# mfouda/epsilon

Hardware: AMD Instinct MI355X
Metric: ADMM iters/sec, dense Lasso 1e4x5e4 (higher is better)
Workload: dtype f32

## Files before the change

### epsilon_amd/csrc/admm.cc

```cpp
#include "admm.h"

#include <algorithm>
#include <chrono>
#include <cmath>
#include <cstdio>
#include <cstdlib>
#include <map>

#include "comm.h"
#include "fused_route.h"
#include "options.h"

namespace eps {

double Now() {
  using clock = std::chrono::steady_clock;
  return std::chrono::duration<double>(clock::now().time_since_epoch()).count();
}

namespace {

std::set<std::string> InferShardedArgs(const BlockMatrix& H) {
  std::set<std::string> out;
  const ShardSpec& sh = ShardSpec::Get();
// ... 44 lines not shown
}

}

Solver::Solver(pb::Problem problem, std::shared_ptr<DataMap> data, pb::SolverParams params)
    : problem_(std::move(problem)), data_(std::move(data)), params_(params) {}
Solver::~Solver() {}

FusedRoute* Solver::batch_route() const { return initialized_ && !finished_ && iter_ == 0 ? route_.get() : nullptr; }
void Solver::BatchLaunchCheck(int iter) {
  iter_ = iter;
  if (route_->HasCheck()) route_->LaunchNorms();
}
bool Solver::BatchFinishCheck() {
  if (route_->HasCheck()) FinishRouteCheck();
  else ComputeResiduals();
  finished_ = status_.state == pb::SolverStatus::OPTIMAL;
  return finished_;
}
void Solver::BatchFinishMaxIterations(int iter) {
  iter_ = iter;
  ComputeResiduals();
  status_.state = pb::SolverStatus::MAX_ITERATIONS_REACHED;
  finished_ = true;
}
void Solver::BatchAddLoopTime(double seconds) {
  loop_seconds_ += seconds;
  status_.init_time = init_seconds_;
  status_.total_time = init_seconds_ + loop_seconds_;
}

void Solver::LogStatus() {
  if (!params_.verbose || !log_) return;
  char buf[256];
  std::snprintf(buf, sizeof(buf), "iter=%d residuals primal=%.2e [%.2e] dual=%.2e [%.2e]",
                status_.num_iterations, status_.r_norm, status_.epsilon_primal, status_.s_norm,
                status_.epsilon_dual);
  log_(buf);
}

void Solver::FinishResiduals(double r, double s, double eps_pri, double eps_dual) {
  status_.r_norm = r;
  status_.s_norm = s;
  status_.epsilon_primal = eps_pri;
  status_.epsilon_dual = eps_dual;
  if (r <= eps_pri && s <= eps_dual && !params_.ignore_stopping_criteria)
    status_.state = pb::SolverStatus::OPTIMAL;
  else
    status_.state = pb::SolverStatus::RUNNING;
  status_.num_iterations = iter_;
}

int Solver::Run(int max_sweeps) {
  EPS_CHECK_MSG(initialized_, "Solver::Run before Init");
  SetCurrentDType(data_->dtype());
  const double t0 = Now();
  int done = 0;
  const int epoch = params_.epoch_iterations > 0 ? params_.epoch_iterations : 1;
  const int log_every = params_.log_iterations > 0 ? params_.log_iterations : 1;
  auto batch_size = [&](int it, int done_so_far) {
    if (it >= params_.max_iterations || (max_sweeps >= 0 && done_so_far >= max_sweeps)) return 0;
    int batch = 1;
    while ((it + batch - 1) % epoch != 0 && !(params_.verbose && (it + batch - 1) % log_every == 0))
      ++batch;
    if (batch > params_.max_iterations - it) batch = params_.max_iterations - it;
    if (max_sweeps >= 0 && batch > max_sweeps - done_so_far) batch = max_sweeps - done_so_far;
    return batch;
  };
  int speculated = 0;
  auto far_from_optimal = [&] {
    if (status_.epsilon_primal <= 0 || status_.epsilon_dual <= 0) return true;
    return status_.r_norm > 4 * status_.epsilon_primal || status_.s_norm > 4 * status_.epsilon_dual;
  };
  while (!finished_ && iter_ < params_.max_iterations && (max_sweeps < 0 || done < max_sweeps)) {
    int batch = speculated;
    if (batch == 0) {
      batch = batch_size(iter_, done);
      SweepBatch(batch);
    }
    speculated = 0;
    done += batch;
    iter_ += batch - 1;
    if (iter_ % epoch == 0) {
      const int next = (PipelinedChecks() && (params_.ignore_stopping_criteria || far_from_optimal()))
                           ? batch_size(iter_ + 1, done)
                           : 0;
      if (next > 0) {
        BeginResiduals();
        SaveSnapshot();
        SweepBatch(next);
        speculated = next;
        EndResiduals();
        if (status_.state == pb::SolverStatus::OPTIMAL) {
          RestoreSnapshot();
          finished_ = true;
          break;
        }
      } else {
        ComputeResiduals();
        if (status_.state == pb::SolverStatus::OPTIMAL) {
          finished_ = true;
          break;
        }
      }
    }
    if (iter_ % log_every == 0) LogStatus();
    ++iter_;
  }
  if (!finished_ && iter_ == params_.max_iterations) {
    ComputeResiduals();
    status_.state = pb::SolverStatus::MAX_ITERATIONS_REACHED;
    finished_ = true;
  }
  Runtime::Get().Sync();
  if (Runtime::Get().peer()) Runtime::Get().peer()->CheckError();
  loop_seconds_ += Now() - t0;
  if (finished_) LogStatus();
  status_.init_time = init_seconds_;
  status_.total_time = init_seconds_ + loop_seconds_;
  return done;
}

void Solver::Solve() {
  const double t0 = Now();
  Init();
  Runtime::Get().Sync();
  init_seconds_ = Now() - t0;
  Run(-1);
}


class ProxADMMSolver final : public Solver {
 public:
  using Solver::Solver;
  ~ProxADMMSolver() override { ResetGraph(); }

  void Init() override {
    SetCurrentDType(data_->dtype());
    const double t0 = Now();
    if (op_cache_.size() > 64) op_cache_.Clear();
    OpCacheScope cache_scope(InitCache());
    static const bool trace = opt::IsSet(opt::kInitTrace);
    auto mark = [&](const char* what) {
      if (!trace) return;
      const double th = Now();
      Runtime::Get().Sync();
      std::fprintf(stderr, "[init] %-16s host %.2f ms  drained %.2f ms\n", what, 1e3 * (th - t0),
                   1e3 * (Now() - t0));
    };
    InitConstraints();
    mark("constraints");
    InitProxOperators();
    mark("prox operators");
    if (!params_.warm_start || !vars_initialized_) {
      InitVariables();
      vars_initialized_ = true;
    }
    iter_ = 0;
    finished_ = false;
    status_ = pb::SolverStatus();
    initialized_ = true;
    ResetGraph();
    route_.reset();
    route_ = RecogniseMultiBlockRoute({static_cast<int>(problem_.constraint.size()), A_, b_, prox_, data_.get(),
                                       shared_cache_, u_, x_, y_, y_prev_});
    mark("fused state");
    if (params_.verbose && log_) {
      char buf[128];
      std::snprintf(buf, sizeof(buf), "constraints, m = %lld, variables, n = %lld",
                    static_cast<long long>(m_), static_cast<long long>(n_));
      log_(buf);
    }
    Runtime::Get().Sync();
    init_seconds_ = Now() - t0;
  }

  BlockVector GetSolution() override {
    BlockVector r;
    for (int i = 0; i < N_; ++i) r += x_[i];
    return r;
  }

 protected:
  void InitConstraints() {
    A_ = BlockMatrix();
    b_ = BlockVector();
    for (size_t i = 0; i < problem_.constraint.size(); ++i) {
      const pb::Expression& constr = problem_.constraint[i];
      EPS_CHECK_MSG(constr.expression_type == pb::Expression::INDICATOR, "constraint is not an indicator");
      EPS_CHECK_MSG(constr.cone_type == 1, "constraint cone is not ZERO");
      EPS_CHECK(constr.arg.size() == 1);
      affine::BuildAffineOperator(constr.arg[0], data_.get(), affine::constraint_key(i), &A_, &b_);
    }
    AT_ = A_.Transpose();
    GlobalDims(A_, &m_, &n_);
  }

  void InitProxOperators() {
    EPS_CHECK_MSG(problem_.objective.expression_type == pb::Expression::ADD, "objective is not ADD");
    N_ = static_cast<int>(problem_.objective.arg.size());
    EPS_CHECK_MSG(params_.rho == 1, "rho != 1 is not supported (reference prox_admm.cc:50)");
    const double sqrt_rho = std::sqrt(params_.rho);
    prox_.clear();
    AiT_.clear();
    arg_shards_.clear();
    term_per_rank_.clear();
    std::set<std::string> constr_vars = A_.col_keys();
    for (int i = 0; i < N_; ++i) {
      const pb::Expression& f_expr = problem_.objective.arg[i];
      EPS_CHECK_MSG(f_expr.expression_type == pb::Expression::PROX_FUNCTION,
                    "objective term " << i << " is not a PROX_FUNCTION");
      AffineOperator H;
      for (size_t k = 0; k < f_expr.arg.size(); ++k)
        affine::BuildAffineOperator(f_expr.arg[k], data_.get(), affine::arg_key(k), &H.A, &H.b);
      AffineOperator A;
      std::map<std::string, const pb::Expression*> vars;
      GetVariables(f_expr, &vars);
      for (const auto& var : vars) {
        if (constr_vars.find(var.first) == constr_vars.end()) continue;
        for (const auto& it : A_.col(var.first)) A.A(it.first, var.first) = sqrt_rho * it.second;
      }
      prox_.emplace_back(CreateProxOperator(f_expr.prox_function.prox_function_type,
                                            f_expr.prox_function.epigraph));
      arg_shards_.push_back(InferShardedArgs(H.A));
      {
        const ShardSpec& sh = ShardSpec::Get();
        bool own = sh.active() && sh.consensus_terms() && !vars.empty();
        for (const auto& var : vars) own = own && sh.IsSharded(var.first);
        term_per_rank_.push_back(own);
      }
      {
        LocalShardScope scope(arg_shards_.back());
        prox_.back()->Init(ProxOperatorArg(f_expr.prox_function, data_.get(), H, A));
      }
      AiT_.push_back(A.A.Transpose());
    }
  }

  void InitVariables() {
    x_.assign(N_, BlockVector());
    y_.assign(N_, BlockVector());
    u_ = BlockVector();
    for (size_t i = 0; i < problem_.constraint.size(); ++i) {
      u_.Set(affine::constraint_key(i),
             DVec::Zeros(GetDimension(problem_.constraint[i].arg[0]), data_->dtype()));
    }
  }

  void ResetGraph() {
    if (graph_exec_) (void)hipGraphExecDestroy(graph_exec_);
    if (graph_) (void)hipGraphDestroy(graph_);
    graph_exec_ = nullptr;
    graph_ = nullptr;
    graph_len_ = 0;
  }

  void SweepBatch(int count) override {
    static const int mode = opt::Int(opt::kGraph, -1);
    Runtime& rt = Runtime::Get();
    const bool want = route_ && route_->Capturable() && (mode == 1 || (mode != 0 && route_->CaptureByDefault()));
    if (!want || count < 2 || rt.profiling()) {
      for (int i = 0; i < count; ++i) Sweep();
      return;
    }
    if (graph_exec_ == nullptr || graph_len_ != count) {
      ResetGraph();
      hipStream_t s = rt.stream();
      EPS_HIP(hipStreamBeginCapture(s, hipStreamCaptureModeThreadLocal));
      rt.set_capturing(true);
      try {
        for (int i = 0; i < count; ++i) route_->Sweep();
      } catch (...) {
        rt.set_capturing(false);
        hipGraph_t dead = nullptr;
        (void)hipStreamEndCapture(s, &dead);
        if (dead) (void)hipGraphDestroy(dead);
        throw;
      }
      rt.set_capturing(false);
      EPS_HIP(hipStreamEndCapture(s, &graph_));
      EPS_HIP(hipGraphInstantiate(&graph_exec_, graph_, nullptr, nullptr, 0));
      graph_len_ = count;
    }
    EPS_HIP(hipGraphLaunch(graph_exec_, rt.stream()));
  }

  void Sweep() override {
    if (route_) {
      route_->Sweep();
      return;
    }
    y_prev_ = y_;
    u_ -= b_;
    for (int i = 0; i < N_; ++i) u_ -= y_[i];
    for (int i = 0; i < N_; ++i) {
      u_ += y_[i];
      {
        LocalShardScope scope(arg_shards_[i]);
        x_[i] = prox_[i]->Apply(u_);
      }
      y_[i] = A_ * x_[i];
      u_ -= y_[i];
    }
  }

  bool PipelinedChecks() const override { return route_ && route_->PipelineChecks(); }
  void BeginResiduals() override {
    Runtime& rt = Runtime::Get();
    rt.ResetSlots();
    route_->LaunchNorms();
    rt.FetchSlotsAsync();
  }
  void EndResiduals() override {
    Runtime::Get().WaitSlots();
    FinishRouteCheck();
  }
  void FinishRouteCheck() override {
    const FusedRoute::Check c = route_->FinishCheck();
// ... 227 lines not shown
```

### epsilon_amd/csrc/capi.cc

```cpp
#include "../../include/epsilon_hip.h"

#include <algorithm>
#include <cmath>
#include <cstdio>
#include <cstdlib>
#include <cstring>
#include <map>
#include <memory>
#include <set>
#include <string>
#include <vector>

#include "admm.h"
#include "block.h"
#include "comm.h"
#include "kernels.h"
#include "linear_map.h"
#include "options.h"
#include "wire.h"

using namespace eps;

struct eps_result {
  std::string status;
// ... 1162 lines not shown
            PutValues(r.get(), "trace\t" + std::to_string(s) + "\t" + f.first, {FillValue(f.second)});
          PutValues(r.get(), "pivot\t" + std::to_string(s) + "\t" + trace[s].pivot, {static_cast<double>(s)});
        }
        for (size_t i = 0; i < chol.order().size(); ++i)
          PutValues(r.get(), "order\t" + std::to_string(i) + "\t" + chol.order()[i], {static_cast<double>(i)});
        if (args.mode == BlockSolveArgs::FACTOR) {
          PutBlocks(r.get(), "L", chol.L());
          PutBlocks(r.get(), "D_inv", chol.D_inv());
        }
        PutValues(r.get(), "condition_estimate", {chol.condition_estimate()});
        PutValues(r.get(), "refine_steps", {static_cast<double>(chol.refine_steps())});
        if (nrhs > 0) {
          PutVector(r.get(), "x", chol.Solve(b));
          PutVector(r.get(), "x_again", chol.Solve(b));
        }
        break;
      }
    }
    *out = r.release();
  });
}

int eps_test_dense_op(const eps_dense_op* g, double* out, double* out2) {
  return Guard([&] {
    const DenseOpArgs args = CheckDenseOpArgs(g, out, out2);
    const DType dt = ConfiguredDType();
    constexpr int64_t G = EPS_DENSE_OP_GUARD;
    const int64_t n = g->rows;
    DVec a_all, x_all, y_all, add_all, a, x, y, add, work;
    if (args.use_a) a = PlaceOperand(g->a, g->a_len, g->a_off, 0, dt, &a_all);
    if (args.use_x) x = PlaceOperand(g->x, g->x_len, g->x_off, 0, dt, &x_all);
    if (args.use_add) add = PlaceOperand(g->add, g->add_len, g->add_off, 0, dt, &add_all);
    if (args.reduction) {
      if (args.use_y) y = PlaceOperand(g->y, g->y_len, g->y_off, 0, dt, &y_all);
      Runtime& rt = Runtime::Get();
      rt.ResetSlots();
      const int slot = rt.NewSlot();
      EPS_HIP(hipMemcpyAsync(rt.SlotPtr(slot), &g->preset, sizeof(double), hipMemcpyHostToDevice, rt.stream()));
      rt.Sync();
      const bool acc = g->accumulate != 0;
      if (args.op == DenseOpArgs::SUMSQ) k::SumSq(x, rt.SlotPtr(slot), acc);
      else if (args.op == DenseOpArgs::SUMSQ_DIFF) k::SumSqDiff(x, y, rt.SlotPtr(slot), acc);
      else k::Dot(x, y, rt.SlotPtr(slot), acc);
      EPS_HIP(hipGetLastError());
      rt.FetchSlots();
      out[0] = rt.SlotValue(slot);
      rt.ResetSlots();
      return;
    }
    static_assert(EPS_DENSE_OP_GUARD % 4 == 0, "the guard keeps offset 0 aligned");
    auto place_y = [&] { y = PlaceOperand(g->y, g->y_len, g->y_off, G, dt, &y_all); };
    auto fetch_y = [&](double* dst) { y_all.Slice(g->y_off, g->y_len + 2 * G).ToHost(dst); };
    place_y();
    const bool symv = args.op == DenseOpArgs::SYMV || args.op == DenseOpArgs::SYMV_PACKED;
    if (symv && g->use_work) work = DVec::Empty(k::SymvWorkspace(n), dt);
    const DVec* wp = (symv && g->use_work) ? &work : nullptr;
    switch (args.op) {
      case DenseOpArgs::GEMV_N:
      case DenseOpArgs::GEMV_T:
        k::Gemv(args.op == DenseOpArgs::GEMV_T, n, g->cols, g->alpha, a, g->lda, x, g->beta, y);
        break;
      case DenseOpArgs::SYMV:
        k::Symv(n, g->alpha, a, g->lda, x, g->beta, y, wp);
        break;
      case DenseOpArgs::SYMV_PACKED: {
        const DVec P = k::SymvPack(n, a, g->lda);
        k::SymvPacked(n, g->alpha, P, x, g->beta, y, wp);
        EPS_HIP(hipGetLastError());
        fetch_y(out);
        place_y();
        k::Symv(n, g->alpha, a, g->lda, x, g->beta, y, wp);
        EPS_HIP(hipGetLastError());
        fetch_y(out2);
        return;
      }
      case DenseOpArgs::REDUCE_PARTIALS:
        k::ReducePartials(n, g->nparts, a, g->alpha, g->beta, y, args.use_add ? &add : nullptr);
        break;
      case DenseOpArgs::AXPBY:
        k::Axpby(y, g->alpha, g->alias_xy ? y : x, g->beta);
        break;
      case DenseOpArgs::DIAG_MUL:
        k::DiagMul(y, g->alpha, a, x, g->beta);
        break;
      default:
        EPS_FATAL("eps_test_dense_op: unreachable");
    }
    EPS_HIP(hipGetLastError());
    fetch_y(out);
  });
}

int eps_test_gemm_op(const eps_gemm_op* g, double* out, char* route, size_t route_cap) {
  return Guard([&] {
    const GemmOpArgs args = CheckGemmOpArgs(g, out, route, route_cap);
    route[0] = '\0';
    const DType dt = ConfiguredDType();
    constexpr int64_t G = EPS_DENSE_OP_GUARD;
    const int64_t M = g->M, N = g->N, K = g->K;
    DVec a_all, b_all, c_all, d_all, a, b, c, d;
    if (args.use_a) a = PlaceOperand(g->a, g->a_len, g->a_off, G, dt, &a_all);
    if (args.use_b) b = PlaceOperand(g->b, g->b_len, g->b_off, G, dt, &b_all);
    if (args.use_c) c = PlaceOperand(g->c, g->c_len, g->c_off, G, dt, &c_all);
    if (args.use_d) d = PlaceOperand(g->d, g->d_len, 0, G, dt, &d_all);
    k::GemmClearRoute();
    switch (args.op) {
      case GemmOpArgs::GEMM:
        k::Gemm(g->trans_a != 0, g->trans_b != 0, M, N, K, g->alpha, a, g->lda, b, g->ldb, g->beta, c, g->ldc,
                g->lower_only != 0);
        break;
      case GemmOpArgs::GEMM_BATCHED:
        k::GemmBatched(g->trans_a != 0, g->trans_b != 0, M, N, K, g->alpha, a, g->lda, g->sA, b, g->ldb, g->sB,
                       g->beta, c, g->ldc, g->sC, g->batch, g->lower_only != 0, g->outer, g->sA2, g->sB2);
        break;
      case GemmOpArgs::MAT_COPY:
        k::MatCopy(g->trans_a != 0, M, N, g->alpha, a, g->lda, c);
        break;
      case GemmOpArgs::ADD_DIAG:
        k::AddDiag(c, M, g->ldc, g->alpha, args.use_d ? &d : nullptr);
        break;
      case GemmOpArgs::SYMMETRIZE:
        k::SymmetrizeFromLower(c, M, g->ldc);
        break;
      case GemmOpArgs::COL_ABS_SUMS: {
        std::vector<double> h(static_cast<size_t>(N + 2 * G), EPS_DENSE_OP_SENTINEL);
        c_all = DVec::FromHost(h.data(), N + 2 * G, F64);
        k::ColAbsSums(a, M, N, g->lda, c_all.as<double>() + G);
        EPS_HIP(hipGetLastError());
        c_all.ToHost(out);
        return;
      }
      case GemmOpArgs::KRON:
        k::KronDense(c, a, M, N, b, K, g->batch);
        break;
    }
    EPS_HIP(hipGetLastError());
    std::snprintf(route, route_cap, "%s", k::GemmLastRoute());
    c_all.Slice(g->c_off, g->c_len + 2 * G).ToHost(out);
  });
}

int eps_test_factor_op(const eps_factor_op* g, double* out, double* out2) {
  return Guard([&] {
    const FactorOpArgs args = CheckFactorOpArgs(g, out);
    const DType dt = ConfiguredDType();
    constexpr int64_t G = EPS_DENSE_OP_GUARD;
    const int64_t n = g->n;
    DVec w_all;
    DVec W = PlaceOperand(g->a, g->a_len, g->a_off, G, dt, &w_all);
    struct Restore { ~Restore() { k::SetPotrfForm(-1); } } restore;
    k::SetPotrfForm(g->form);
    if (args.op == FactorOpArgs::SPD_INVERSE) {
      DVec X;
      k::SpdInverseInPlace(W, n, out2 != nullptr ? &X : nullptr);
      EPS_HIP(hipGetLastError());
      w_all.Slice(g->a_off, n * n + 2 * G).ToHost(out);
      if (out2 != nullptr && n > 0) X.Slice(0, n * n).ToHost(out2);
      return;
    }
    const int64_t len = n * g->out_cols;
    std::vector<double> h(static_cast<size_t>(g->a_off + 2 * G + len), EPS_DENSE_OP_SENTINEL);
    DVec o_all = DVec::FromHost(h.data(), static_cast<int64_t>(h.size()), dt);
    k::SpdInverseColumns(W, n, g->lo, g->cnt, o_all.Slice(g->a_off + G, len));
    EPS_HIP(hipGetLastError());
    o_all.Slice(g->a_off, len + 2 * G).ToHost(out);
    if (out2 != nullptr && n > 0) W.ToHost(out2);
  });
}

int eps_bench_spd_inverse_columns(int64_t n, int64_t cnt, int iters, double* ms_avg) {
  return Guard([&] {
    const DType dt = ConfiguredDType();
    DVec G = Synthetic(n * n, dt, 1.0);
    DVec W0 = DVec::Zeros(n * n, dt);
    k::Gemm(false, true, n, n, n, 1.0 / n, G, n, G, n, 0.0, W0, n, false);
    k::AddDiag(W0, n, n, 1.0, nullptr);
    DVec W = DVec::Empty(n * n, dt);
    DVec Out = DVec::Empty(n * cnt, dt);
    Runtime& rt = Runtime::Get();
    double total = 0;
    for (int i = 0; i < iters + 1; ++i) {
      k::Copy(W, W0);
      rt.Sync();
      hipEvent_t a, b;
      EPS_HIP(hipEventCreate(&a));
      EPS_HIP(hipEventCreate(&b));
      EPS_HIP(hipEventRecord(a, rt.stream()));
      k::SpdInverseColumns(W, n, 0, cnt, Out);
      EPS_HIP(hipEventRecord(b, rt.stream()));
      EPS_HIP(hipEventSynchronize(b));
      float e = 0;
      EPS_HIP(hipEventElapsedTime(&e, a, b));
      (void)hipEventDestroy(a);
      (void)hipEventDestroy(b);
      if (i > 0) total += e;
    }
    *ms_avg = total / iters;
  });
}

int eps_bench_prox(int kind, int64_t n, int iters, double* ms_avg) {
  return Guard([&] {
    EPS_CHECK(n > 0 && iters > 0 && ms_avg != nullptr);
    const DType dt = ConfiguredDType();
    DVec v = Synthetic(n, dt, 4.0);
    DVec x = DVec::Empty(n, dt);
    k::ScaledZoneArgs a;
    a.lam = 0.7;
    DVec lamv;
    if (kind == 1) {
      lamv = Synthetic(n, dt, 1.0);
      k::Axpby(lamv, 0.0, lamv, 1.0);
      k::Fill(lamv, 0.7);
      a.lam_vec = &lamv;
    }
    *ms_avg = TimeLaunches(iters, [&] {
      if (kind == 2) k::MaxZero(x, v);
      else k::ScaledZone(x, v, a);
    });
  });
}

int eps_bench_svd(int64_t m, int64_t n, int rank, int max_sweeps, double perturb, double* ms_cold,
                  int* sweeps_cold, double* ms_warm, int* sweeps_warm, double* defects) {
  return Guard([&] {
    EPS_CHECK(m > 0 && n > 0 && ms_cold != nullptr);
    const DType dt = ConfiguredDType();
    Runtime& rt = Runtime::Get();
    uint64_t st = 0x9E3779B97F4A7C15ull;
    auto uni = [&] {
      st ^= st << 13;
      st ^= st >> 7;
      st ^= st << 17;
      return static_cast<double>(st >> 11) * (1.0 / 9007199254740992.0);
    };
    auto gauss = [&] { return (uni() + uni() + uni() + uni() - 2.0) * 1.7320508075688772; };
    std::vector<double> h(static_cast<size_t>(m) * std::max<int64_t>(rank, 1));
    for (auto& v : h) v = gauss();
    DVec A = DVec::FromHost(h.data(), m * std::max<int64_t>(rank, 1), dt);
    h.resize(static_cast<size_t>(n) * std::max<int64_t>(rank, 1));
    for (auto& v : h) v = gauss();
    DVec B = DVec::FromHost(h.data(), n * std::max<int64_t>(rank, 1), dt);
    DVec Y = DVec::Empty(m * n, dt);
    {
      std::vector<float> sp(static_cast<size_t>(m) * n);
      for (auto& v : sp) v = uni() < 0.1 ? static_cast<float>(10.0 * gauss()) : 0.0f;
      std::vector<double> col(m);
      std::vector<double> all(sp.begin(), sp.end());
      sp.clear();
      sp.shrink_to_fit();
      Y = DVec::FromHost(all.data(), m * n, dt);
    }
    if (rank > 0) k::Gemm(false, true, m, n, rank, 1.0, A, m, B, n, 1.0, Y, m);
    auto timed = [&](const DVec& W, const DVec& V, bool warm, double* ms, int* sweeps) {
      rt.Sync();
      hipEvent_t a, b;
      EPS_HIP(hipEventCreate(&a));
      EPS_HIP(hipEventCreate(&b));
      EPS_HIP(hipEventRecord(a, rt.stream()));
      const int sw = k::JacobiSvd(W, m, n, V, max_sweeps, warm, false);
      EPS_HIP(hipEventRecord(b, rt.stream()));
      EPS_HIP(hipEventSynchronize(b));
      float e = 0;
      EPS_HIP(hipEventElapsedTime(&e, a, b));
      (void)hipEventDestroy(a);
      (void)hipEventDestroy(b);
      *ms = e;
      if (sweeps) *sweeps = sw;
    };
    auto measure = [&](const DVec& Y0, const DVec& W, const DVec& V, double* out) {
      DVec T = DVec::Empty(n * n, dt);
      k::Gemm(true, false, n, n, n, 1.0, V, n, V, n, 0.0, T, n);
      k::AddDiag(T, n, n, -1.0, nullptr);
      rt.ResetSlots();
      const int s0 = rt.NewSlot(), s1 = rt.NewSlot(), s2 = rt.NewSlot(), s3 = rt.NewSlot(), s4 = rt.NewSlot();
      k::SumSq(T, rt.SlotPtr(s0), false);
      DVec R = Y0.Clone();
      k::Gemm(false, true, m, n, n, 1.0, W, m, V, n, -1.0, R, m);
      k::SumSq(R, rt.SlotPtr(s1), false);
      k::SumSq(Y0, rt.SlotPtr(s2), false);
      k::Gemm(true, false, n, n, m, 1.0, W, m, W, m, 0.0, T, n);
      k::SumSq(T, rt.SlotPtr(s3), false);
      DVec sig = DVec::Empty(n, dt);
      k::ColNorms(W, m, n, sig, false);
      DVec sq = DVec::Empty(n, dt);
      k::DiagMul(sq, 1.0, sig, sig, 0.0);
      k::SumSq(sq, rt.SlotPtr(s4), false);
      rt.FetchSlots();
      out[0] = std::sqrt(rt.SlotValue(s0) / static_cast<double>(n));
      out[1] = std::sqrt(rt.SlotValue(s1) / rt.SlotValue(s2));
      const double all = rt.SlotValue(s3), diag = rt.SlotValue(s4);
      out[2] = std::sqrt(std::max(0.0, all - diag) / diag);
    };
    DVec W = Y.Clone();
    DVec V = DVec::Empty(n * n, dt);
    timed(W, V, false, ms_cold, sweeps_cold);
    if (defects) measure(Y, W, V, defects);
    if (ms_warm != nullptr && perturb >= 0) {
      DVec Y2 = Y.Clone();
      DVec N = Synthetic(m * n, dt, 1.0);
      k::Axpby(Y2, perturb, N, 1.0);
      DVec W2 = DVec::Empty(m * n, dt);
      k::Gemm(false, false, m, n, n, 1.0, Y2, m, V, n, 0.0, W2, m);
      timed(W2, V, true, ms_warm, sweeps_warm);
      if (defects) measure(Y2, W2, V, defects + 3);
    }
  });
// ... 60 lines not shown
```

### epsilon_amd/csrc/fused_route.cc

```cpp
#include "fused_route.h"

#include <algorithm>
#include <cmath>
#include <cstring>
#include <map>

#include "admm.h"
#include "comm.h"
#include "kernels.h"
#include "options.h"

namespace eps {
namespace {


k::ZoneParams ZoneOf(const ScaledZoneDesc& z, double a1) {
  k::ZoneParams s;
  s.alpha_vec = z.alpha_vec;
  s.beta_vec = z.beta_vec;
  s.Bs = z.Bs;
  s.Cs = z.Cs;
  s.a1 = a1;
  s.lam = z.lam;
  s.alpha = z.alpha;
// ... 33 lines not shown
    if (shared != nullptr) {
      key = HashCombine(HashCombine(reinterpret_cast<uintptr_t>(D->data().data()), 0x9ac4ed), m);
      if (auto hit = shared->Find(key)) {
        packed = hit->data();
        return;
      }
    }
    packed = k::SymvPack(m, D->data(), m);
    if (key) shared->Put(key, std::make_shared<DenseMatrixImpl>(packed, packed.n, 1, false, 1.0, key));
  }
  InverseApply Column(int64_t c) const {
    InverseApply a = *this;
    a.p = p.Slice(c * m, m);
    a.w = w.Slice(c * m, m);
    if (work.n > 0) a.work = work.Slice(c * k::SymvWorkspace(m), k::SymvWorkspace(m));
    return a;
  }
  void Apply() const {
    if (packed.n > 0) k::SymvPacked(m, D->scale(), packed, p, 0.0, w, &work);
    else if (work.n > 0) k::Symv(m, D->scale(), D->data(), m, p, 0.0, w, &work);
    else D->Apply(1.0, p, 0.0, w);
  }
};

struct StateSlice {
  BlockVector* home;
  std::string key;
  DVec v;
  bool take = true;
};
void AdoptState(const std::vector<StateSlice>& table, const std::vector<BlockVector*>& homes) {
  for (const StateSlice& s : table) {
    if (!s.take || !s.home->has_key(s.key)) continue;
    EPS_CHECK((*s.home)(s.key).n == s.v.n);
    k::Copy(s.v, (*s.home)(s.key));
  }
  for (BlockVector* h : homes) *h = BlockVector();
  for (const StateSlice& s : table) s.home->Set(s.key, s.v);
}
std::vector<BlockVector*> Homes(const MultiBlockParts& a) {
  std::vector<BlockVector*> h = {&a.u};
  for (auto* c : {&a.x, &a.y, &a.y_prev})
    for (BlockVector& v : *c) h.push_back(&v);
  return h;
}

int BatchWideMin();

enum ZeroTallMode { kZeroTallOff, kZeroTallOn, kZeroTallAuto };
enum MatrixRoute { kMatrixOff, kMatrixPass, kMatrixWide, kMatrixAuto };

constexpr int64_t kResidentLimitBytes = int64_t(224) << 20;

k::FusedResidency ResidentShare(int64_t m, int64_t n, DType dt, int64_t touched, bool auto_on,
                                k::LassoFusedArgs* pass = nullptr) {
  int64_t budget = opt::FusedResident();
  if (budget < 0) budget = auto_on ? std::max<int64_t>(0, kResidentLimitBytes - touched * (dt == F32 ? 4 : 8)) : 0;
  const k::FusedResidency res = k::LassoFusedResidency(m, n, dt, budget);
  if (pass != nullptr) {
    pass->qfull = res.qfull;
    pass->jcut = res.jcut;
  }
  return res;
}

constexpr int64_t kMatrixFusedMinRows = 256;

constexpr int64_t kZeroFusedMinRows = 256;

constexpr int64_t kZeroTallMinCols = 256;
constexpr int64_t kZeroTallAutoMinCols = 256;
constexpr int64_t kZeroTallSmoothAutoMinCols = 512;

uint64_t Bits(double v) {
  uint64_t b;
  std::memcpy(&b, &v, 8);
  return b;
}

bool RhsAligned(const std::vector<const k::LassoInstance*>& members) {
  bool aligned = true;
  for (const k::LassoInstance* s : members)
    if (s->rhs.n > 0) aligned = aligned && reinterpret_cast<uintptr_t>(s->rhs.data()) % 16 == 0;
  return aligned;
}

struct WideSweep {
  static constexpr int PW = k::kLassoWidePanel;
  int64_t m = 0, n = 0, lda = 0, ldv = 0, panel_len = 0;
  DVec A;
  bool whiten = false;
  const DenseMatrixImpl* D = nullptr;
  DVec V, T, apart;
  int64_t akc = 0, afull = 0, arem = 0, aparts = 0;

  void Init(int64_t m_, int64_t n_, const DVec& A_, int64_t lda_, bool whiten_, const DenseMatrixImpl* D_) {
    m = m_;
    n = n_;
    A = A_;
    lda = lda_;
    whiten = whiten_;
    D = D_;
    ldv = (n + 63) / 64 * 64;
    panel_len = static_cast<int64_t>(PW) * m;
    V = DVec::Zeros(static_cast<int64_t>(PW) * ldv, F32);
    T = DVec::Empty(static_cast<int64_t>(k::LassoWideSlabs(m, n)) * panel_len, F32);
    akc = std::max<int64_t>(32, ((m + 63) / 64 + 31) / 32 * 32);
    afull = m / akc;
    arem = m - afull * akc;
    aparts = afull + (arem > 0 ? 1 : 0);
    apart = whiten ? DVec() : DVec::Empty(aparts * panel_len, F32);
  }

  void ApplyInverse(const DVec& Pp, const DVec& Wp) const {
    const int64_t sA = D->trans() ? akc : akc * D->rows();
    k::GemmBatched(D->trans(), false, m, PW, akc, D->scale(), D->data(), D->rows(), sA, Pp, m, akc, 0.0, apart, m,
                   panel_len, afull);
    if (arem > 0) {
      const int64_t oA = afull * sA, oB = afull * akc;
      k::GemmBatched(D->trans(), false, m, PW, arem, D->scale(), D->data().Slice(oA, D->data().n - oA), D->rows(),
                     0, Pp.Slice(oB, Pp.n - oB), m, 0, 0.0, apart.Slice(afull * panel_len, panel_len), m, 0, 1);
    }
    k::ReducePartials(panel_len, static_cast<int>(aparts), apart, 1.0, 0.0, Wp);
  }

  void Run(const DVec& table, int first, int nk, uint64_t live, const DVec& Wp, const DVec& Pp,
           const double* group_lam = nullptr) const {
    k::LassoWideBack(m, n, lda, A, table, first, nk, live, Wp, m, V, ldv, group_lam);
    k::LassoWideForward(m, n, lda, A, nk, V, ldv, T, m);
    k::LassoWideReduce(m, n, table, first, nk, live, T, m);
    if (!whiten) ApplyInverse(Pp, Wp);
  }
};

struct BatchRoute : FusedRoute {
  DType dt = F32;
  int64_t m = 0, n = 0;
  int grid = 0;
  DVec w, p, tpart;
  InverseApply inv;
  bool whiten = false;
  k::LassoFusedArgs pass;
  k::FusedResidency res;

  virtual bool BatchKey(const pb::SolverParams& params, bool tall_groups, std::vector<uint64_t>* key) const = 0;
  virtual const k::ZeroRowsArgs* Rows() const { return nullptr; }
  virtual const k::ZeroTallSamplesArgs* Samples() const { return nullptr; }
  virtual k::FusedResidency Residency(int64_t count) const { return res; }

  std::vector<uint64_t> KeyHead(const DenseMatrixImpl& L, const DenseMatrixImpl& D,
                                const pb::SolverParams& params) const {
    return {static_cast<uint64_t>(pass.chain), reinterpret_cast<uintptr_t>(L.data().data()),
            static_cast<uint64_t>(L.rows()), static_cast<uint64_t>(m), static_cast<uint64_t>(n),
            static_cast<uint64_t>(dt), Bits(L.scale()), reinterpret_cast<uintptr_t>(D.data().data()),
            Bits(D.scale()), reinterpret_cast<uintptr_t>(inv.packed.data()), inv.work.n > 0 ? 1u : 0u,
            static_cast<uint64_t>(params.max_iterations), static_cast<uint64_t>(params.epoch_iterations)};
  }

  template <class Applies>
  void BatchSweep(const DVec& table, const DVec& row_table, const DVec& sample_table, int count,
                  const double* group_lam, const k::FusedResidency& share, bool rhs_aligned, const DVec& work,
                  Applies own_applies) const {
    const int64_t pm = pass.m, pn = pass.n;
    auto passes = [&](int chain) {
      const int width = k::LassoBatchWidth(pm, pn, dt, chain);
      for (int first = 0; first < count; first += width)
        k::LassoBatchPass(pm, pn, pass.lda, pass.A, table, first, std::min(width, count - first), group_lam, share,
                          chain);
    };
    passes(pass.chain);
    if (Samples() != nullptr) {
      k::ZeroTallSamplesBatch(pn, dt, sample_table, count);
      passes(5);
    }
    if (Rows() != nullptr) k::ZeroFusedRowsBatch(pm, grid, Rows()->smooth, dt, row_table, count, Rows()->tall);
    else k::ReducePartialsBatch(pm, grid, table, count, dt, rhs_aligned);
    if (whiten) return;
    if (inv.packed.n > 0) k::SymvPackedBatch(pm, inv.D->scale(), inv.packed, table, count, work);
    else own_applies();
  }
};

struct LassoRoute final : BatchRoute {
  LeastSquaresDesc ls;
  ScaledZoneDesc sz;
  double a1 = 0;
  int64_t slab = 0;
  bool sharded = false;
  bool use_peer = false;
  bool peer_slab = false;
  bool replicated_apply = false;
  DVec wpad, wslice;
  DVec state_all, snapshot;
  DVec norm_work;
  int norm_slot = 0;
  double wscale = 1;
  DVec X, Ahat, rhat;
  int64_t cols = 1;
  bool group = false;
  int64_t group_rows = 0;
  bool wide = false;
  bool rhs_aligned = true;
  std::vector<k::LassoInstance> members;
  DVec table;
  WideSweep ws;

  k::FusedResidency Residency(int64_t count, k::LassoFusedArgs* into) const {
    if (sharded || use_peer || wide || ShardSpec::Get().active()) return k::FusedResidency();
    return ResidentShare(m, n, dt, count * (static_cast<int64_t>(grid) * m + 6 * n + 2 * m) + (whiten ? 0 : m * m),
                         count == 1 && cols == 1, into);
  }
  k::FusedResidency Residency(int64_t count) const override { return Residency(count, nullptr); }

  bool Enable(const MultiBlockParts& a) {
    if (opt::Is0(opt::kFused) || a.prox.size() != 2 || a.num_constraints != 1 || !a.b.data().empty()) return false;
    const ShardSpec& sh = ShardSpec::Get();
    if (sh.active() && sh.consensus_terms()) return false;
    if (!a.prox[0]->DescribeLeastSquares(&ls)) return false;
    cols = ls.cols;
    const int matrix_mode = cols > 1 ? opt::Word(opt::kFusedMatrix) : kMatrixAuto;
    if (cols > 1 && (matrix_mode == kMatrixOff || sh.active())) return false;
    if (!a.prox[1]->DescribeScaledZone(&sz)) {
      GroupNorm2Desc gn;
      if (cols == 1 || !a.prox[1]->DescribeGroupNorm2(&gn) || gn.cols != cols) return false;
      group = true;
      group_rows = gn.rows;
      sz = ScaledZoneDesc();
      sz.var_key = gn.var_key;
      sz.constraint_key = gn.constraint_key;
      sz.Bs = gn.Bs;
      sz.Cs = gn.Cs;
      sz.lam = gn.lam;
    }
    dt = a.data->dtype();
    if ((sz.alpha_vec.n > 0 && sz.alpha_vec.dt != dt) || (sz.beta_vec.n > 0 && sz.beta_vec.dt != dt)) return false;
    const std::string ck = affine::constraint_key(0);
    if (ls.constraint_key != ck || sz.constraint_key != ck || a.A.data().size() != 2) return false;
    const DenseMatrixImpl& L = *ls.L_arg_var;
    if (L.trans()) return false;
    m = L.rows();
    n = L.cols();
    const int64_t nx = n * cols;
    double a0 = 0;
    if (!ConsensusTie(a.A, ck, ls.var_key, sz.var_key, nx, &a0, &a1) || a0 != 1.0) return false;
    if (!k::LassoFusedSupported(m, n, L.data(), L.rows())) return false;
    if (ls.rhs_arg.n != 0 && ls.rhs_arg.n != m * cols) return false;
    if (cols > 1 && !ChooseMatrixRoute(matrix_mode)) return false;
    const int64_t npad = (nx + 63) / 64 * 64;
    state_all = DVec::Zeros(6 * npad, dt);
    snapshot = DVec::Empty(6 * npad, dt);
    norm_work = DVec::Zeros(64 * 5 + 1, F64);
    a.y_prev.resize(2);
    std::vector<StateSlice> views = {{&a.x[0], ls.var_key}, {&a.x[1], sz.var_key}, {&a.y[0], ck},
                                     {&a.y[1], ck},         {&a.u, ck},            {&a.y_prev[1], ck}};
    views[5].take = false;
    for (size_t q = 0; q < views.size(); ++q) views[q].v = state_all.Slice(static_cast<int64_t>(q) * npad, nx);
    k::ConsensusState& s = pass.inst.state;
    s.copy = views[0].v, s.var = views[1].v, s.y_zero = views[2].v, s.y_term = views[3].v, s.u = views[4].v;
    s.y_term_prev = views[5].v;
    grid = k::LassoFusedGrid(m, n, dt);
    const int64_t wlen = wide ? (cols + WideSweep::PW - 1) / WideSweep::PW * WideSweep::PW * m : cols * m;
    p = DVec::Zeros(wlen, dt);
    if (!wide) tpart = DVec::Empty(static_cast<int64_t>(grid) * m * cols, dt);
    if (cols > 1) {
      w = DVec::Zeros(wlen, dt);
    } else {
      Comm* comm = Runtime::Get().comm();
      PeerExchange* px = Runtime::Get().peer();
      sharded = sh.active() && sh.IsSharded(ls.var_key);
      use_peer = sharded && px != nullptr && m * (dt == F64 ? 2 : 1) <= px->slot() && ls.Dinv_arg != nullptr &&
                 !ls.Dinv_arg->trans() && ls.Dinv_arg->rows() == m;
      const int G = use_peer ? px->view().G : (comm ? comm->size() : 1);
      slab = ((m + G - 1) / G + 3) / 4 * 4;
      wpad = DVec::Zeros(slab * G, dt);
      wslice = DVec::Zeros(slab, dt);
      w = wpad.Slice(0, m);
      const char* e = opt::Raw(opt::kShardedApply);
      replicated_apply = e && e[0] == 'r';
      const bool want_slab = e ? !replicated_apply : G >= 3;
      peer_slab = use_peer && want_slab && k::PeerSlabApplySupported(px->view(), m, slab, ls.Dinv_arg->data(), m);
    }
    if (!use_peer && !sh.active() && EnableWhiten()) {
    } else if (wide) {
    } else {
      inv.Init(ls.Dinv_arg, m, p, w, a.shared_cache, cols);
    }
    if (wide) ws.Init(m, n, whiten ? Ahat : L.data(), whiten ? m : L.rows(), whiten, ls.Dinv_arg.get());
    BuildPass();
    AdoptState(views, Homes(a));
    ForwardFromState();
    return true;
  }

  bool ChooseMatrixRoute(int mode) {
    const DenseMatrixImpl& L = *ls.L_arg_var;
    const DenseMatrixImpl& D = *ls.Dinv_arg;
    if (m < kMatrixFusedMinRows || L.dtype() != dt || D.dtype() != dt) return false;
    if (group && group_rows != n) return false;
    if (sz.alpha_vec.n > 0 && sz.alpha_vec.n != n * cols) return false;
    if (sz.beta_vec.n > 0 && sz.beta_vec.n != n * cols) return false;
    if (D.rows() != m || D.cols() != m) return false;
    const int width = k::LassoBatchWidth(m, n, dt);
    const bool pass_ok = width > 0 && (!group || cols <= width);
    const bool wide_ok = dt == F32 && k::LassoWideSupported(m, n, L.data(), L.rows()) &&
                         (!group || cols <= WideSweep::PW);
    if (mode == kMatrixPass) wide = false;
    else if (mode == kMatrixWide) wide = true;
    else wide = wide_ok && (cols >= BatchWideMin() || !pass_ok);
    return wide ? wide_ok : pass_ok;
  }

  bool EnableWhiten() {
    const DenseMatrixImpl& L = *ls.L_arg_var;
    const DenseMatrixImpl& D = *ls.Dinv_arg;
    OpCache* cache = CurrentOpCache();
    if (!FusedWhitenEnabled() || cache == nullptr || dt != F32 || L.dtype() != F32 || m < kWhitenMinRows)
      return false;
    if (n < 2 * m) return false;
    if (D.id() == 0 || D.trans() || D.rows() != m || D.cols() != m || L.rows() != m) return false;
    const auto cached = cache->Find(D.id());
    const auto Xm = cache->Find(FactorInverseKey(D.id()));
    if (!cached || !Xm || cached->data().data() != D.data().data() || Xm->rows() != m || Xm->cols() != m)
      return false;
    const uint64_t key = HashCombine(HashCombine(HashCombine(HashCombine(Xm->id(), 0x3a7),
                                                             reinterpret_cast<uintptr_t>(L.data().data())),
                                                 L.id()),
                                     static_cast<uint64_t>(n));
    DVec Ah;
    if (auto hit = cache->Find(key)) {
      Ah = hit->data();
    } else {
      Ah = DVec::Empty(m * n, F32);
      if (!k::GemmSplitF16KRange(4, m, n, m, 1.0, Xm->data(), m, L.data(), m, Ah, m))
        k::Gemm(false, false, m, n, m, 1.0, Xm->data(), m, L.data(), m, 0.0, Ah, m);
      cache->Put(key, std::make_shared<DenseMatrixImpl>(Ah, m, n, false, 1.0, key));
    }
    if (!k::LassoFusedSupported(m, n, Ah, m)) return false;
    if (ls.rhs_arg.n != 0 && cols > 1) {
      rhat = DVec::Empty(m * cols, F32);
      k::Gemm(false, false, m, cols, m, 1.0, Xm->data(), m, ls.rhs_arg, m, 0.0, rhat, m);
    } else if (ls.rhs_arg.n != 0) {
      rhat = DVec::Empty(m, F32);
      k::Gemv(false, m, m, 1.0, Xm->data(), m, ls.rhs_arg, 0.0, rhat);
    }
    X = Xm->data();
    Ahat = Ah;
    wscale = D.scale();
    whiten = true;
    return true;
  }

  void ForwardFromState() {
    const DenseMatrixImpl& L = *ls.L_arg_var;
    const k::ConsensusState& s = pass.inst.state;
    DVec v0 = s.u.Clone();
    k::Axpby(v0, -1.0, s.y_zero, 1.0);
    k::Axpby(v0, -1.0, s.y_term, 1.0);
    k::Axpby(v0, 1.0, s.y_zero, 1.0);
    if (cols == 1 && !whiten) {
      L.Apply(-1.0, v0, 0.0, p);
      ForwardTail(false);
      return;
    }
    const int64_t mk = m * cols;
    DVec pp = whiten && cols > 1 ? DVec::Empty(mk, v0.dt) : p.Slice(0, mk);
    for (int64_t c = 0; c < cols; ++c) L.Apply(-1.0, v0.Slice(c * n, n), 0.0, pp.Slice(c * m, m));
    if (ls.rhs_arg.n != 0) k::Axpby(pp, 1.0, ls.rhs_arg, 1.0);
    for (int64_t c = 0; whiten && c < cols; ++c)
      k::Gemv(false, m, m, 1.0, X, m, pp.Slice(c * m, m), 0.0, w.Slice(c * m, m));
    if (!whiten) ApplyInverseFixed();
  }

  void ForwardTail(bool reduced) {
    const DenseMatrixImpl& L = *ls.L_arg_var;
    if (whiten) {
      k::ReducePartials(m, grid, tpart, -L.scale(), 0.0, w, rhat.n != 0 ? &rhat : nullptr);
      return;
    }
    bool rhs_added = false;
    if (reduced) {
      const bool have_rhs = ls.rhs_arg.n != 0;
      const bool fold = have_rhs && (!sharded || Runtime::Get().comm()->rank() == 0);
      k::ReducePartials(m, grid, tpart, -L.scale(), 0.0, p, fold ? &ls.rhs_arg : nullptr);
      rhs_added = have_rhs;
    }
    if (sharded) Runtime::Get().comm()->AllReduceSum(p);
    if (ls.rhs_arg.n != 0 && !rhs_added) k::Axpby(p, 1.0, ls.rhs_arg, 1.0);
    const DenseMatrixImpl& D = *ls.Dinv_arg;
    Comm* comm = Runtime::Get().comm();
    if (sharded && comm->size() > 1 && !D.trans() && D.rows() == m && !replicated_apply) {
      const int64_t per = slab;
      const int64_t lo = std::min<int64_t>(m, comm->rank() * per);
      const int64_t cnt = std::min<int64_t>(m, lo + per) - lo;
      DVec mine = wslice;
      if (cnt < per) k::Fill(mine, 0.0);
      if (cnt > 0) {
        DVec rows = D.data().Slice(lo * m, cnt * m);
        k::Gemv(true, m, cnt, D.scale(), rows, m, p, 0.0, mine.Slice(0, cnt));
      }
      comm->AllGather(mine.data(), wpad.data(), static_cast<size_t>(per), wpad.dt);
    } else {
      ApplyInverseFixed();
    }
  }

  void ForwardTailPeer() {
    const DenseMatrixImpl& L = *ls.L_arg_var;
    const DenseMatrixImpl& D = *ls.Dinv_arg;
    const PeerView& pv = Runtime::Get().peer()->view();
    k::PeerReduceExchange(pv, m, grid, tpart, -L.scale(), ls.rhs_arg.n != 0 ? &ls.rhs_arg : nullptr, p);
    if (peer_slab) {
      const int64_t lo = std::min<int64_t>(m, static_cast<int64_t>(pv.rank) * slab);
      k::PeerSlabApplyExchange(pv, m, slab, lo, D.data(), m, D.scale(), p, wpad);
    } else {
      ApplyInverseFixed();
    }
  }

  void ApplyInverseFixed() {
    if (wide) {
      for (int64_t q = 0; q * ws.panel_len < w.n; ++q)
        ws.ApplyInverse(p.Slice(q * ws.panel_len, ws.panel_len), w.Slice(q * ws.panel_len, ws.panel_len));
    } else if (cols == 1) {
      inv.Apply();
    } else if (inv.packed.n > 0) {
      k::SymvPackedBatch(m, inv.D->scale(), inv.packed, table, static_cast<int>(cols), inv.work);
    } else {
      for (int64_t c = 0; c < cols; ++c) inv.Column(c).Apply();
    }
  }

  void BuildPass() {
    const DenseMatrixImpl& L = *ls.L_arg_var;
    pass.m = m;
    pass.n = n;
    pass.lda = whiten ? m : L.rows();
    pass.A = whiten ? Ahat : L.data();
    res = Residency(cols, &pass);
    k::LassoInstance& s = pass.inst;
    s.w = w;
    s.tpart = tpart;
    s.p = whiten ? w : p;
    s.rhs = whiten ? rhat : ls.rhs_arg;
    s.kappa = -L.scale() * (whiten ? wscale : 1.0);
    s.pkappa = -L.scale();
    s.zone = ZoneOf(sz, a1);
    if (cols == 1) return;
    members.assign(static_cast<size_t>(cols), s);
    for (int64_t c = 0; c < cols; ++c) {
      k::LassoInstance& mb = members[static_cast<size_t>(c)];
      auto col = [&](const DVec& v, int64_t len) { return v.n > 0 ? v.Slice(c * len, len) : v; };
      mb.w = col(s.w, m);
      mb.p = col(s.p, m);
      mb.rhs = col(s.rhs, m);
      if (!wide) mb.tpart = col(s.tpart, static_cast<int64_t>(grid) * m);
      else mb.tpart = mb.w;
      k::ConsensusState& ms = mb.state;
      for (DVec* v : {&ms.u, &ms.var, &ms.copy, &ms.y_term, &ms.y_zero, &ms.y_term_prev, &mb.zone.alpha_vec,
                      &mb.zone.beta_vec})
        *v = col(*v, n);
    }
    std::vector<const k::LassoInstance*> v;
    for (const auto& mb : members) v.push_back(&mb);
    rhs_aligned = RhsAligned(v);
    k::LassoBatchUpload(v, dt, &table);
  }

  void MatrixSweep() {
    const int K = static_cast<int>(cols);
    const double* group_lam = group ? &sz.lam : nullptr;
    if (wide) {
      constexpr int PW = WideSweep::PW;
      for (int first = 0; first < K; first += PW) {
        const int nk = std::min(PW, K - first);
        const uint64_t live = nk == 64 ? ~uint64_t(0) : (uint64_t(1) << nk) - 1;
        const int64_t off = static_cast<int64_t>(first) * m;
        ws.Run(table, first, nk, live, w.Slice(off, ws.panel_len), whiten ? DVec() : p.Slice(off, ws.panel_len),
               group_lam);
      }
      return;
    }
    BatchSweep(table, DVec(), DVec(), K, group_lam, res, rhs_aligned, inv.work, [&] {
      for (int64_t c = 0; c < cols; ++c) inv.Column(c).Apply();
    });
  }

  void Sweep() override {
    if (cols > 1) {
      MatrixSweep();
    } else if (use_peer) {
      pass.epoch = Runtime::Get().peer()->view().epoch;
      k::LassoFusedPass(pass);
      ForwardTailPeer();
    } else {
      k::LassoFusedPass(pass);
      ForwardTail(true);
    }
  }

  bool HasCheck() const override { return true; }
  bool PipelineChecks() const override {
    static const bool off = opt::Is0(opt::kPipelineChecks);
    return !off;
  }
  void LaunchNorms() override {
    Runtime& rt = Runtime::Get();
    norm_slot = rt.NewSlot();
// ... 598 lines not shown
```

### epsilon_amd/csrc/fused_route.h

```cpp
#pragma once

#include <memory>
#include <vector>

#include "block.h"
#include "prox.h"

namespace eps {

class FusedRoute {
 public:
  virtual ~FusedRoute() {}
  virtual void Sweep() = 0;

  virtual bool HasCheck() const { return false; }
  virtual bool PipelineChecks() const { return false; }
  virtual void LaunchNorms() {}
  struct Check {
    double r = 0, s = 0;
    double max_norm = 0;
    double atu = 0;
  };
  virtual Check FinishCheck() { return Check(); }
  virtual void SaveSnapshot() {}
  virtual void RestoreSnapshot() {}

  virtual bool Capturable() const { return false; }
  virtual bool CaptureByDefault() const { return false; }
};

struct MultiBlockParts {
  int num_constraints;
  const BlockMatrix& A;
  const BlockVector& b;
  const std::vector<std::unique_ptr<ProxOperator>>& prox;
  DataMap* data;
  OpCache* shared_cache;
  BlockVector& u;
  std::vector<BlockVector>&x, &y, &y_prev;
};
struct TwoBlockParts {
  int num_constraints;
  const AffineOperator& constr_H;
  const std::vector<std::unique_ptr<ProxOperator>>& prox;
  DataMap* data;
  BlockVector &x, &z, &u, &z_prev;
};

std::unique_ptr<FusedRoute> RecogniseMultiBlockRoute(const MultiBlockParts& parts);
std::unique_ptr<FusedRoute> RecogniseTwoBlockRoute(const TwoBlockParts& parts);

}
```

### epsilon_amd/csrc/kernels.h

```cpp
#pragma once

#include "device.h"

namespace eps {
struct PeerView;
namespace k {

void Fill(const DVec& y, double v);
void Copy(const DVec& dst, const DVec& src);
void FillHash(const DVec& y, uint64_t seed);
void Axpby(const DVec& y, double a, const DVec& x, double b);
void DiagMul(const DVec& y, double a, const DVec& d, const DVec& x, double b);
void ConvertFromF64(const DVec& dst, const double* src_dev);
void ConvertToF64(double* dst_dev, const DVec& src);
void ConvertFromF32(const DVec& dst, const float* src_dev);

void SumSq(const DVec& x, double* slot, bool accumulate);
void SumSqDiff(const DVec& x, const DVec& y, double* slot, bool accumulate);
void Dot(const DVec& x, const DVec& y, double* slot, bool accumulate);

void Gemv(bool trans, int64_t rows, int64_t cols, double alpha, const DVec& A, int64_t lda,
          const DVec& x, double beta, const DVec& y);

void Symv(int64_t n, double alpha, const DVec& S, int64_t lds, const DVec& x, double beta,
// ... 17 lines not shown
  double Bs = 0, Cs = 0, a1 = 0, lam = 0, alpha = 1, beta = 1, M = 0;
};
struct LassoInstance {
  DVec w;
  DVec tpart;
  ConsensusState state;
  ZoneParams zone;
  DVec p, rhs;
  double kappa = 0;
  double pkappa = 0;
  DVec zg, zrhs;
  DVec zd, zfarg;
  double ke = 0, dinv = 0;
};
struct LassoFusedArgs {
  int64_t m = 0, n = 0, lda = 0;
  DVec A;
  LassoInstance inst;
  unsigned* epoch = nullptr;
  int chain = 0;
  double a0 = 1;
  DVec e1;
  int qfull = 0;
  int64_t jcut = 0;
};

enum SmoothFn { SMOOTH_EXP, SMOOTH_LOGISTIC, SMOOTH_NEG_ENTR, SMOOTH_INV_POS, SMOOTH_NEG_LOG };

struct ZeroRowsArgs {
  int64_t m = 0;
  int nparts = 0;
  DVec w, tpart, r, rhs, g;
  ConsensusState state;
  ZoneParams zone;
  double e = 0, pkappa = 0;
  bool smooth = false;
  SmoothFn fn = SMOOTH_LOGISTIC;
  DVec hs, hys, hv;
  bool tall = false;
};
struct ZeroTallSamplesArgs {
  int64_t m = 0;
  DVec d, farg;
  DVec rhs, g;
  ConsensusState state;
  ZoneParams zone;
  DVec hs, hys, hv;
  double kappa = 0, ke = 0, dinv = 0;
  SmoothFn fn = SMOOTH_LOGISTIC;
};
void ZeroTallSamples(const ZeroTallSamplesArgs& args);
void ZeroTallSamplesHead(const ZeroTallSamplesArgs& args);
void ZeroFusedRows(const ZeroRowsArgs& args);
void ZeroSmoothHead(const ZeroRowsArgs& args);
void ZeroRowsBatchUpload(const std::vector<const ZeroRowsArgs*>& members, DVec* table);
void ZeroFusedRowsBatch(int64_t m, int nparts, bool smooth, DType dt, const DVec& table, int count,
                        bool tall = false);
void ZeroTallSamplesBatchUpload(const std::vector<const ZeroTallSamplesArgs*>& members, DVec* table);
void ZeroTallSamplesBatch(int64_t m, DType dt, const DVec& table, int count);
bool LassoFusedSupported(int64_t m, int64_t n, const DVec& A, int64_t lda);
int LassoFusedGrid(int64_t m, int64_t n, DType dt = F32);
int LassoFusedBlock(int64_t m, int64_t n, DType dt);
struct FusedResidency {
  int qfull = 0;
  int64_t jcut = 0;
  int64_t bytes = 0;
};
FusedResidency LassoFusedResidency(int64_t m, int64_t n, DType dt, int64_t budget);
FusedResidency LastFusedResidency();
void NoteFusedResidency(int qfull, int64_t jcut);
void LassoFusedPass(const LassoFusedArgs& args);
void LassoFusedNorms(const DVec& u, const DVec& y0, const DVec& y1, const DVec& y1prev, double* out6,
                     const DVec& work, const unsigned* peer_err = nullptr);

template <class T> struct LassoBatchInst {
  const T* w;
  T* tpart;
  T* u; T* x0; T* x1; T* y0; T* y1; T* y1prev;
  const T* alpha_v;
  const T* beta_v;
  T* p;
  const T* rhs;
  T kappa, Bs, Cs, a1, lam, alpha, beta, M;
  T pkappa;
  T* e0;
  const T* zg;
  const T* zrhs;
  T* zd;
  const T* zfarg;
  T ke, dinv;
};
int LassoBatchWidth(int64_t m, int64_t n, DType dt, int chain = 0);
void LassoBatchUpload(const std::vector<const LassoInstance*>& members, DType dt, DVec* table);
void LassoBatchPass(int64_t m, int64_t n, int64_t lda, const DVec& A, const DVec& table, int first,
                    int count, const double* group_lam = nullptr, const FusedResidency& res = FusedResidency(),
                    int chain = 0);
void ReducePartialsBatch(int64_t m, int nparts, const DVec& table, int count, DType dt,
                         bool rhs_aligned);
void SymvPackedBatch(int64_t m, double alpha, const DVec& P, const DVec& table, int count,
                     const DVec& work);

constexpr int kLassoWidePanel = 64;
bool LassoWideSupported(int64_t m, int64_t n, const DVec& A, int64_t lda);
int LassoWideSlabs(int64_t m, int64_t n);
void LassoWideBack(int64_t m, int64_t n, int64_t lda, const DVec& A, const DVec& table, int first, int nk,
                   uint64_t active, const DVec& W, int64_t ldw, const DVec& V, int64_t ldv,
                   const double* group_lam = nullptr);
void LassoWideForward(int64_t m, int64_t n, int64_t lda, const DVec& A, int nk, const DVec& V, int64_t ldv,
                      const DVec& T, int64_t ldt);
void LassoWideReduce(int64_t m, int64_t n, const DVec& table, int first, int nk, uint64_t active, const DVec& T,
                     int64_t ldt);

void PeerBumpEpoch(const PeerView& pv);
void PeerReduceExchange(const PeerView& pv, int64_t rows, int nparts, const DVec& partial,
                        double alpha, const DVec* add, const DVec& y);
bool PeerSlabApplySupported(const PeerView& pv, int64_t m, int64_t slab, const DVec& D, int64_t ldd);
void PeerSlabApplyExchange(const PeerView& pv, int64_t m, int64_t slab, int64_t lo, const DVec& D,
                           int64_t ldd, double scale, const DVec& p, const DVec& wpad);

void Gemm(bool transA, bool transB, int64_t M, int64_t N, int64_t K, double alpha,
          const DVec& A, int64_t lda, const DVec& B, int64_t ldb, double beta, const DVec& C,
          int64_t ldc, bool lower_only = false);
void GemmBatched(bool transA, bool transB, int64_t M, int64_t N, int64_t K, double alpha,
                 const DVec& A, int64_t lda, int64_t sA, const DVec& B, int64_t ldb, int64_t sB,
                 double beta, const DVec& C, int64_t ldc, int64_t sC, int64_t batch,
                 bool lower_only = false, int64_t outer = 1, int64_t sA2 = 0, int64_t sB2 = 0);
void SymmetrizeFromLower(const DVec& C, int64_t n, int64_t ldc);
const char* GemmLastRoute();
void GemmClearRoute();
bool GemmSplitF16(bool transA, bool transB, int64_t M, int64_t N, int64_t K, double alpha, const DVec& A,
                  int64_t lda, const DVec& B, int64_t ldb, double beta, const DVec& C, int64_t ldc,
                  bool lower_only);
bool GemmF64Pipe(bool transA, bool transB, int64_t M, int64_t N, int64_t K, double alpha, const DVec& A,
                 int64_t lda, int64_t sA, const DVec& B, int64_t ldb, int64_t sB, double beta,
                 const DVec& C, int64_t ldc, int64_t sC, int64_t n1, int64_t batch, bool lower_only,
                 int64_t sA2, int64_t sB2);
bool GemmSplitF16KRange(int kmode, int64_t M, int64_t N, int64_t K, double alpha, const DVec& A, int64_t lda,
                        const DVec& B, int64_t ldb, const DVec& C, int64_t ldc);
bool SyrkSplitF16LowerTriangular(int64_t n, const DVec& X, int64_t ldx, const DVec& C, int64_t ldc);
bool MultiGemv(bool transA, int64_t M, int64_t N, int64_t K, double alpha, const DVec& A, int64_t lda,
               const DVec& B, int64_t ldb, double beta, const DVec& C, int64_t ldc);
void StreamProbe(int mode, const void* src, void* dst, int64_t bytes, float* scratch, int grid);
void StreamResidentProbe(const void* src, int64_t bytes, int64_t resident_per_column, float* scratch, int grid);

void MatCopy(bool trans, int64_t rows, int64_t cols, double alpha, const DVec& src,
             int64_t lds, const DVec& dst);
void AddDiag(const DVec& W, int64_t n, int64_t ld, double alpha, const DVec* d);
void ColAbsSums(const DVec& A, int64_t rows, int64_t cols, int64_t lda, double* colsum_dev);
void ScaleByInvNorm(const DVec& y, const DVec& x, const double* normsq_dev);
void KronDense(const DVec& dst, const DVec& A, int64_t mA, int64_t nA, const DVec& B,
               int64_t mB, int64_t nB);

void SpdInverseInPlace(const DVec& W, int64_t n, DVec* factor_inverse = nullptr);
void SetPotrfForm(int form);
void SpdInverseColumns(const DVec& W, int64_t n, int64_t lo, int64_t cnt, const DVec& Out);

struct ScaledZoneArgs {
  double lam = 0, alpha = 1, beta = 1, M = 0, C = 0;
  const DVec* lam_vec = nullptr;
  const DVec* alpha_vec = nullptr;
  const DVec* beta_vec = nullptr;
  int64_t period = 0;
};
void ScaledZone(const DVec& x, const DVec& v, const ScaledZoneArgs& args);
void MaxZero(const DVec& x, const DVec& v);
void Norm2Shrink(const DVec& x, const DVec& v, double lam, const double* normsq);

void SumSquareEpigraph(const DVec& x, const DVec& t, const DVec& u, const DVec& s,
                       const double* normsq, double* lam_scratch);
void ZoneEpigraphKeys(const DVec& v, double alpha, double beta, const DVec* alpha_vec,
                      const DVec* beta_vec, double M, double C, double* key, double* w2,
                      double* fval);
void ZoneEpigraphSums(int64_t n, const double* key, const double* w2, double lam, double* sums);

int JacobiSvd(const DVec& W, int64_t m, int64_t n, const DVec& V, int max_sweeps = 40,
              bool warm = false, bool row_sharded = false);
int BlockJacobiSvd(const DVec& W, int64_t m, int64_t n, const DVec& V, int max_sweeps = 40,
                   bool warm = false, bool row_sharded = false);
bool JacobiSvdCanSkipV(int64_t m, int64_t n, DType dt);
int JacobiSvdNoV(const DVec& W, int64_t m, int64_t n, int max_sweeps = 40);
void ColNorms(const DVec& W, int64_t m, int64_t n, const DVec& sigma, bool row_sharded = false);
void ColScaleByRatio(const DVec& W, int64_t m, int64_t n, const DVec& sigma, const DVec& xt);

struct Segs {
  int64_t count = 1, len = 0, seg_stride = 0, elem_stride = 1;
};
void SegNorm2Shrink(const DVec& x, const DVec& v, double lam, const Segs& S);
void SegMaxProx(const DVec& x, const DVec& v, double lam, const Segs& S);
void SegMaxEpigraph(const DVec& x, const DVec& t, const DVec& v, const DVec& s, const Segs& S);
void SegSumLargestProx(const DVec& x, const DVec& v, double lam, int k, const Segs& S);
void SegSumLargestEpigraph(const DVec& x, const DVec& t, const DVec& v, const DVec& s, int k,
                           const Segs& S);
void SegZoneEpigraph(const DVec& x, const DVec& t, const DVec& v, const DVec& s, double alpha,
                     double beta, const DVec* alpha_vec, const DVec* beta_vec, double M,
                     const Segs& S);
void SegSocProject(const DVec& x, const DVec& t, const DVec& v, const DVec& tin, double beta,
                   const Segs& S);
void SegLogSumExpProx(const DVec& x, const DVec& v, double lam, const Segs& S);
void SegLogSumExpEpigraph(const DVec& x, const DVec& t, const DVec& v, const DVec& s,
                          const Segs& S);
void SmoothProx(SmoothFn fn, const DVec& x, const DVec& v, double lam, const DVec* lam_vec);
void SegSmoothEpigraph(SmoothFn fn, const DVec& x, const DVec& t, const DVec& v, const DVec& s,
                       const Segs& S);
void KlDivProx(const DVec& x, const DVec& y, const DVec& u, const DVec& v, double lam,
               const DVec* lam_vec);
void SegKlDivEpigraph(const DVec& x, const DVec& y, const DVec& t, const DVec& u, const DVec& v,
                      const DVec& s, const Segs& S);
void ExpEpigraph(const DVec& x, const DVec& t, const DVec& v, const DVec& s);

int Tv1dSeg(const DVec& x, const DVec& v, double lam, const Segs& S);

}
}
```

### epsilon_amd/csrc/kernels_factor.hip

```cpp
#include <hip/hip_runtime.h>

#include <algorithm>
#include <cstdlib>
#include <type_traits>

#include "kernels.h"
#include "options.h"

namespace eps {
namespace k {

namespace {

constexpr int NB = 64;

template <int L> __device__ inline float ReadLane(float v) {
  return __builtin_bit_cast(float, __builtin_amdgcn_readlane(__builtin_bit_cast(int, v), L));
}
template <int L> __device__ inline double ReadLane(double v) {
  const long long b = __builtin_bit_cast(long long, v);
  const int lo = __builtin_amdgcn_readlane(static_cast<int>(b), L);
  const int hi = __builtin_amdgcn_readlane(static_cast<int>(b >> 32), L);
  return __builtin_bit_cast(double, (static_cast<long long>(hi) << 32) |
                                        static_cast<unsigned int>(lo));
// ... 230 lines not shown
      if (col < kb) W[row + (k0 + col) * ld] = Tt[col][r];
    }
  }
}

__global__ __launch_bounds__(256) void PotrfFusedStepKernel(float* W, int64_t ld, int64_t n, int64_t K0,
                                                            int64_t k0, int kb, int* flag,
                                                            float* __restrict__ dfac) {
  using T = float;
  __shared__ T Tt[NB][NB];
  __shared__ T Dd[NB][NB];
  __shared__ T buf[2 * KC * NB];
  T* Lr = buf;
  T* Pc = buf + KC * NB;
  const int t = threadIdx.x, r = t & 63, q = t >> 6;
  const int64_t row0 = k0 + kb + static_cast<int64_t>(blockIdx.x) * NB;
  const int64_t row = row0 + r;
  const bool live = row < n;
  T acc[16], dac[16];
#pragma unroll
  for (int c = 0; c < 16; ++c) {
    const int col = q * 16 + c;
    acc[c] = (live && col < kb) ? W[row + (k0 + col) * ld] : T(0);
    T v = (r == col) ? T(1) : T(0);
    if (r < kb && col < kb && r >= col) v = W[(k0 + r) + (k0 + col) * ld];
    dac[c] = v;
  }
  constexpr int PF = KC * NB / 256;
  T pfl[PF], pfp[PF];
  auto fetch = [&](int64_t kk) {
#pragma unroll
    for (int i = 0; i < PF; ++i) {
      const int idx = t + i * 256, rr = idx & 63, k = idx >> 6;
      pfl[i] = (row0 + rr < n) ? W[(row0 + rr) + (kk + k) * ld] : T(0);
      pfp[i] = rr < kb ? W[(k0 + rr) + (kk + k) * ld] : T(0);
    }
  };
  if (K0 < k0) fetch(K0);
  for (int64_t kk = K0; kk < k0; kk += KC) {
    __syncthreads();
#pragma unroll
    for (int i = 0; i < PF; ++i) {
      const int idx = t + i * 256;
      Lr[idx] = pfl[i];
      Pc[idx] = pfp[i];
    }
    __syncthreads();
    if (kk + KC < k0) fetch(kk + KC);
#pragma unroll 4
    for (int k = 0; k < KC; ++k) {
      const T a = Lr[k * NB + r], d = Pc[k * NB + r];
#pragma unroll
      for (int c = 0; c < 16; ++c) {
        const T pc = Pc[k * NB + q * 16 + c];
        acc[c] -= a * pc;
        dac[c] -= d * pc;
      }
    }
  }
  __syncthreads();
#pragma unroll
  for (int c = 0; c < 16; ++c) {
    Tt[q * 16 + c][r] = acc[c];
    Dd[q * 16 + c][r] = dac[c];
  }
  __syncthreads();
  if (q == 0) {
    T rowv[NB], tv[NB];
    StaticFor<0, NB>::Run([&](auto cc) {
      constexpr int c = decltype(cc)::value;
      rowv[c] = r >= c ? Dd[c][r] : T(0);
      tv[c] = Tt[c][r];
    });
    const bool bad = CholRowsSolve(rowv, tv, r);
    if (bad && r == 0) *flag = 1;
    StaticFor<0, NB>::Run([&](auto cc) {
      constexpr int c = decltype(cc)::value;
      Tt[c][r] = tv[c];
      if (blockIdx.x == 0) dfac[c * NB + r] = rowv[c];
    });
  }
  __syncthreads();
  if (live) {
#pragma unroll
    for (int c = 0; c < 16; ++c) {
      const int col = q * 16 + c;
      if (col < kb) W[row + (k0 + col) * ld] = Tt[col][r];
    }
  }
}

template <class T>
__global__ __launch_bounds__(64) void TrtriDiagBlocksKernel(const T* W, int64_t ld, int64_t n, T* Dinv) {
  const int lane = threadIdx.x;
  const int64_t k0 = static_cast<int64_t>(blockIdx.x) * NB;
  const int kb = static_cast<int>(n - k0 < NB ? n - k0 : NB);
  T r[NB];
  StaticFor<0, NB>::Run([&](auto cc) {
    constexpr int c = decltype(cc)::value;
    T v = (lane == c) ? T(1) : T(0);
    if (lane < kb && c < kb && lane >= c) v = W[(k0 + lane) + (k0 + c) * ld];
    r[c] = v;
  });
  T x[NB];
  StaticFor<0, NB>::Run([&](auto ii) {
    constexpr int j = NB - 1 - decltype(ii)::value;
    const T ajj = T(1) / ReadLane<j>(r[j]);
    T acc = T(0);
    StaticFor<0, (NB - 1 - j + 3) / 4>::Run([&](auto gg) {
      constexpr int c0 = j + 1 + 4 * decltype(gg)::value;
      T b[4];
      StaticFor<0, 4>::Run([&](auto ii) {
        constexpr int kk = c0 + decltype(ii)::value;
        if constexpr (kk < NB) b[decltype(ii)::value] = ReadLane<kk>(r[j]);
      });
      StaticFor<0, 4>::Run([&](auto ii) {
        constexpr int kk = c0 + decltype(ii)::value;
        if constexpr (kk < NB) acc += x[kk] * b[decltype(ii)::value];
      });
      Pin(acc);
    });
    x[j] = lane > j ? -acc * ajj : (lane == j ? ajj : T(0));
  });
  T* out = Dinv + static_cast<int64_t>(blockIdx.x) * NB * NB;
  StaticFor<0, NB>::Run([&](auto cc) {
    constexpr int c = decltype(cc)::value;
    out[lane + c * NB] = (lane < kb && c < kb && lane >= c) ? x[c] : T(0);
  });
}

template <class T>
__global__ __launch_bounds__(256) void ScatterDiagBlocksKernel(const T* Dinv, T* X, int64_t ld, int64_t n) {
  const int64_t k0 = static_cast<int64_t>(blockIdx.x) * NB;
  const T* src = Dinv + static_cast<int64_t>(blockIdx.x) * NB * NB;
  for (int idx = threadIdx.x; idx < NB * NB; idx += 256) {
    const int r = idx & 63, c = idx >> 6;
    if (k0 + r < n && k0 + c < n) X[(k0 + r) + (k0 + c) * ld] = src[idx];
  }
}

DVec Sub(const DVec& W, int64_t i, int64_t j, int64_t ld) {
  const int64_t off = i + j * ld;
  return W.Slice(off, W.n - off);
}

}

namespace {
void PotrfBlocked(const DVec& W, int64_t n, const DVec& dinv, int* flag);
void CheckFlag(int* flag);
void DoublingInverse(const DVec& W, const DVec& X, int64_t n, const DVec& dinv, int64_t cap);
}

void SpdInverseInPlace(const DVec& W, int64_t n, DVec* factor_inverse) {
  EPS_CHECK(W.n >= n * n);
  if (n == 0) return;
  Runtime& rt = Runtime::Get();
  hipStream_t s = rt.stream();
  ProfScope prof("spd_inverse", n);
  const DType dt = W.dt;
  const int64_t ld = n;
  const int64_t nb = (n + NB - 1) / NB;

  DVec dinv = DVec::Empty(nb * NB * NB, dt);
  auto flag_buf = rt.Alloc(sizeof(int));
  int* flag = static_cast<int*>(flag_buf->p);
  EPS_HIP(hipMemsetAsync(flag, 0, sizeof(int), s));
  {
    ProfScope p1("potrf", n);
    PotrfBlocked(W, n, dinv, flag);
  }

  DVec X = DVec::Zeros(n * n, dt);
  {
    ProfScope p2("trtri", n);
    DoublingInverse(W, X, n, dinv, n);
  }
  ProfScope p3("lauum", n);

  if (!SyrkSplitF16LowerTriangular(n, X, ld, W, ld)) {
    const int64_t B = 1024;
    Fill(W.Slice(0, n * n), 0.0);
    for (int64_t p0 = 0; p0 < n; p0 += B) {
      const int64_t pb = std::min<int64_t>(B, n - p0);
      const int64_t cp = p0 + pb;
      DVec Xp = Sub(X, p0, 0, ld);
      Gemm(true, false, cp, cp, pb, 1.0, Xp, ld, Xp, ld, 1.0, W, ld, true);
    }
  }
  SymmetrizeFromLower(W, n, ld);

  CheckFlag(flag);
  if (factor_inverse) *factor_inverse = X;
}

namespace {

void CheckFlag(int* flag) {
  hipStream_t s = Runtime::Get().stream();
  int host_flag = 0;
  EPS_HIP(hipMemcpyAsync(&host_flag, flag, sizeof(int), hipMemcpyDeviceToHost, s));
  EPS_HIP(hipStreamSynchronize(s));
  EPS_CHECK_MSG(host_flag == 0, "dense inverse: matrix is not positive definite");
}

void DoublingInverse(const DVec& W, const DVec& X, int64_t n, const DVec& dinv, int64_t cap) {
  hipStream_t s = Runtime::Get().stream();
  const DType dt = W.dt;
  const int64_t ld = n;
  const int64_t nb = (n + NB - 1) / NB;
  if (dt == F32)
    hipLaunchKernelGGL(ScatterDiagBlocksKernel<float>, dim3(static_cast<unsigned>(nb)), dim3(256), 0, s,
                       dinv.as<float>(), X.as<float>(), ld, n);
  else
    hipLaunchKernelGGL(ScatterDiagBlocksKernel<double>, dim3(static_cast<unsigned>(nb)), dim3(256), 0, s,
                       dinv.as<double>(), X.as<double>(), ld, n);
  const int64_t half = std::min<int64_t>(cap, n) / 2 + NB;
  const int64_t kBatchBelow = 4096;
  DVec tmp2 = DVec::Empty(std::max<int64_t>({1, half * half, n * std::min(cap, kBatchBelow) / 4}), dt);
  for (int64_t sz = NB; sz < cap; sz *= 2) {
    int64_t r_first = 0;
    if (sz < kBatchBelow) {
      const int64_t P = n / (2 * sz);
      if (P > 0) {
        const int64_t stride = 2 * sz * (ld + 1);
        EPS_CHECK(tmp2.n >= P * sz * sz);
        GemmBatched(false, false, sz, sz, sz, 1.0, Sub(W, sz, 0, ld), ld, stride, X, ld, stride, 0.0,
                    tmp2, sz, sz * sz, P);
        GemmBatched(false, false, sz, sz, sz, -1.0, Sub(X, sz, sz, ld), ld, stride, tmp2, sz, sz * sz,
                    0.0, Sub(X, sz, 0, ld), ld, stride, P);
      }
      r_first = P * 2 * sz;
    }
    for (int64_t r0 = r_first; r0 + sz < n; r0 += 2 * sz) {
      const int64_t s1 = sz;
      const int64_t s2 = std::min<int64_t>(sz, n - (r0 + sz));
      DVec L21 = Sub(W, r0 + s1, r0, ld);
      DVec X11 = Sub(X, r0, r0, ld);
      DVec X22 = Sub(X, r0 + s1, r0 + s1, ld);
      DVec X21 = Sub(X, r0 + s1, r0, ld);
      EPS_CHECK(tmp2.n >= s2 * s1);
      DVec T = tmp2.Slice(0, s2 * s1);
      const int64_t tiles = ((s1 + 127) / 128) * ((s2 + 127) / 128);
      const int64_t nsplit = std::max<int64_t>(1, std::min<int64_t>(4, tiles / 400));
      const int64_t cb = (s1 + nsplit - 1) / nsplit;
      const bool t_done = GemmSplitF16KRange(3, s2, s1, s1, 1.0, L21, ld, X11, ld, T, s2);
      for (int64_t c0 = 0; c0 < s1 && !t_done; c0 += cb) {
        const int64_t cw = std::min<int64_t>(cb, s1 - c0);
        Gemm(false, false, s2, cw, s1 - c0, 1.0, Sub(L21, 0, c0, ld), ld, Sub(X11, c0, c0, ld), ld,
             0.0, T.Slice(c0 * s2, cw * s2), s2);
      }
      const int64_t rb = (s2 + nsplit - 1) / nsplit;
      const bool x_done = GemmSplitF16KRange(4, s2, s1, s2, -1.0, X22, ld, T, s2, X21, ld);
      for (int64_t r1 = 0; r1 < s2 && !x_done; r1 += rb) {
        const int64_t rw = std::min<int64_t>(rb, s2 - r1);
        Gemm(false, false, rw, s1, r1 + rw, -1.0, Sub(X22, r1, 0, ld), ld, T, s2, 0.0,
             Sub(X21, r1, 0, ld), ld);
      }
    }
  }

}

int g_potrf_form = -1;

void PotrfBlocked(const DVec& W, int64_t n, const DVec& dinv, int* flag) {
  Runtime& rt = Runtime::Get();
  hipStream_t s = rt.stream();
  const DType dt = W.dt;
  const int64_t ld = n;
  const int64_t OB = 4 * NB;
  {
    const bool two_kernels = g_potrf_form == 1 ||
                             (g_potrf_form < 0 && opt::IsSet(opt::kPotrfTwoKernels));
    const unsigned nblk = static_cast<unsigned>((n + NB - 1) / NB);
    const bool fused = dt == F32 && !two_kernels;
    std::shared_ptr<Buffer> dfac_buf;
    if (fused) dfac_buf = rt.Alloc(static_cast<size_t>(nblk) * NB * NB * sizeof(float));
    float* dfac = fused ? static_cast<float*>(dfac_buf->p) : nullptr;
    for (int64_t K0 = 0; K0 < n; K0 += OB) {
      const int64_t KB = std::min<int64_t>(OB, n - K0);
      for (int64_t k0 = K0; k0 < K0 + KB; k0 += NB) {
        const int kb = static_cast<int>(std::min<int64_t>(NB, n - k0));
        const int64_t rem = n - (k0 + kb);
        const unsigned blocks = static_cast<unsigned>((rem + NB - 1) / NB);
        if (dt == F32) {
          if (fused) {
            hipLaunchKernelGGL(PotrfFusedStepKernel, dim3(blocks ? blocks : 1), dim3(256), 0, s,
                               W.as<float>(), ld, n, K0, k0, kb, flag, dfac + (k0 / NB) * NB * NB);
          } else {
            hipLaunchKernelGGL(PotrfDiagStepKernel<float>, dim3(1), dim3(256), 0, s, W.as<float>(), ld,
                               K0, k0, kb, flag);
            if (blocks)
              hipLaunchKernelGGL(PotrfPanelStepKernel<float>, dim3(blocks), dim3(256), 0, s,
                                 W.as<float>(), ld, n, K0, k0, kb);
          }
        } else {
          hipLaunchKernelGGL(PotrfDiagStepKernel<double>, dim3(1), dim3(256), 0, s, W.as<double>(),
                             ld, K0, k0, kb, flag);
          if (blocks)
            hipLaunchKernelGGL(PotrfPanelStepKernel<double>, dim3(blocks), dim3(256), 0, s,
                               W.as<double>(), ld, n, K0, k0, kb);
        }
      }
      const int64_t rem2 = n - (K0 + KB);
      if (rem2 > 0) {
        DVec L21 = Sub(W, K0 + KB, K0, ld);
        DVec W22 = Sub(W, K0 + KB, K0 + KB, ld);
        Gemm(false, true, rem2, rem2, KB, -1.0, L21, ld, L21, ld, 1.0, W22, ld, true);
      }
    }
    if (fused)
      hipLaunchKernelGGL(ScatterDiagBlocksKernel<float>, dim3(nblk), dim3(256), 0, s, dfac, W.as<float>(), ld, n);
    if (dt == F32)
      hipLaunchKernelGGL(TrtriDiagBlocksKernel<float>, dim3(nblk), dim3(64), 0, s, W.as<float>(), ld, n,
                         dinv.as<float>());
    else
      hipLaunchKernelGGL(TrtriDiagBlocksKernel<double>, dim3(nblk), dim3(64), 0, s, W.as<double>(), ld,
                         n, dinv.as<double>());
  }
}

}

void SetPotrfForm(int form) { g_potrf_form = form; }

void SpdInverseColumns(const DVec& W, int64_t n, int64_t lo, int64_t cnt, const DVec& Out) {
  EPS_CHECK(W.n >= n * n && Out.n >= n * cnt && Out.dt == W.dt && lo >= 0 && lo + cnt <= n);
  if (n == 0) return;
  Runtime& rt = Runtime::Get();
  hipStream_t s = rt.stream();
  ProfScope prof("spd_inverse_columns", n, cnt);
  const DType dt = W.dt;
  const int64_t ld = n;
  const int64_t nb = (n + NB - 1) / NB;
  DVec dinv = DVec::Empty(nb * NB * NB, dt);
  auto flag_buf = rt.Alloc(sizeof(int));
  int* flag = static_cast<int*>(flag_buf->p);
  EPS_HIP(hipMemsetAsync(flag, 0, sizeof(int), s));
  PotrfBlocked(W, n, dinv, flag);
  if (cnt == 0) {
    CheckFlag(flag);
    return;
  }
  Fill(Out.Slice(0, n * cnt), 0.0);
// ... 37 lines not shown
```

### epsilon_amd/csrc/kernels_vec.hip

```cpp
#include <hip/hip_runtime.h>

#include "kernels.h"

namespace eps {
namespace k {

namespace {

constexpr int kBlock = 256;
constexpr int kMaxGrid = 2048;

template <class T> struct Pack;
template <> struct Pack<float> { using type = float4; static constexpr int V = 4; };
template <> struct Pack<double> { using type = double2; static constexpr int V = 2; };

inline bool Aligned16(const void* p) { return (reinterpret_cast<uintptr_t>(p) & 15) == 0; }

inline int GridFor(int64_t work_items) {
  int64_t g = (work_items + kBlock - 1) / kBlock;
  if (g < 1) g = 1;
  if (g > kMaxGrid) g = kMaxGrid;
  return static_cast<int>(g);
}

// ... 94 lines not shown
#pragma unroll
  for (int off = 32; off > 0; off >>= 1) v += __shfl_down(v, off, 64);
  return v;
}

__device__ inline double BlockSum(double v) {
  __shared__ double wsum[kBlock / 64];
  v = WaveSum(v);
  const int lane = threadIdx.x & 63, wave = threadIdx.x >> 6;
  if (lane == 0) wsum[wave] = v;
  __syncthreads();
  double total = 0;
  if (threadIdx.x == 0) {
#pragma unroll
    for (int w = 0; w < kBlock / 64; ++w) total += wsum[w];
  }
  __syncthreads();
  return total;
}

enum RedOp { RED_SUMSQ = 0, RED_SUMSQ_DIFF = 1, RED_DOT = 2 };

template <class T, int OP>
__device__ inline double RedTerm(const T* x, const T* y, int64_t i) {
  if (OP == RED_SUMSQ) {
    double a = static_cast<double>(x[i]);
    return a * a;
  } else if (OP == RED_SUMSQ_DIFF) {
    double a = static_cast<double>(x[i]) - static_cast<double>(y[i]);
    return a * a;
  } else {
    return static_cast<double>(x[i]) * static_cast<double>(y[i]);
  }
}

template <class T, int OP>
__global__ __launch_bounds__(kBlock) void RedKernel(const T* __restrict__ x,
                                                    const T* __restrict__ y, int64_t n,
                                                    double* partial, double* slot,
                                                    int accumulate) {
  const int64_t tid = blockIdx.x * static_cast<int64_t>(blockDim.x) + threadIdx.x;
  const int64_t stride = static_cast<int64_t>(gridDim.x) * blockDim.x;
  double a0 = 0, a1 = 0, a2 = 0, a3 = 0;
  int64_t i = tid;
  for (; i + 3 * stride < n; i += 4 * stride) {
    a0 += RedTerm<T, OP>(x, y, i);
    a1 += RedTerm<T, OP>(x, y, i + stride);
    a2 += RedTerm<T, OP>(x, y, i + 2 * stride);
    a3 += RedTerm<T, OP>(x, y, i + 3 * stride);
  }
  for (; i < n; i += stride) a0 += RedTerm<T, OP>(x, y, i);
  double total = BlockSum((a0 + a1) + (a2 + a3));
  if (threadIdx.x == 0) {
    if (gridDim.x == 1) {
      *slot = (accumulate ? *slot : 0.0) + total;
    } else {
      partial[blockIdx.x] = total;
    }
  }
}

__global__ __launch_bounds__(kBlock) void RedFinalKernel(const double* partial, int nparts,
                                                         double* slot, int accumulate) {
  double acc = 0;
  for (int i = threadIdx.x; i < nparts; i += kBlock) acc += partial[i];
  double total = BlockSum(acc);
  if (threadIdx.x == 0) *slot = (accumulate ? *slot : 0.0) + total;
}

template <class T, int OP>
void LaunchRed(const T* x, const T* y, int64_t n, double* slot, bool accumulate) {
  Runtime& rt = Runtime::Get();
  hipStream_t s = rt.stream();
  if (n <= (int64_t(1) << 13)) {
    hipLaunchKernelGGL((RedKernel<T, OP>), dim3(1), dim3(kBlock), 0, s, x, y, n,
                       static_cast<double*>(nullptr), slot, accumulate ? 1 : 0);
    return;
  }
  int grid = GridFor(n / 8);
  if (grid > 1024) grid = 1024;
  double* partial = static_cast<double*>(rt.Scratch(1024 * sizeof(double)));
  hipLaunchKernelGGL((RedKernel<T, OP>), dim3(grid), dim3(kBlock), 0, s, x, y, n, partial, slot,
                     0);
  hipLaunchKernelGGL(RedFinalKernel, dim3(1), dim3(kBlock), 0, s, partial, grid, slot,
                     accumulate ? 1 : 0);
}


template <class T>
__global__ __launch_bounds__(kBlock) void AddDiagKernel(T* W, int64_t n, int64_t ld, T alpha,
                                                        const T* d) {
  const int64_t i = blockIdx.x * static_cast<int64_t>(blockDim.x) + threadIdx.x;
  if (i < n) W[i + i * ld] += d ? alpha * d[i] : alpha;
}

template <class T>
__global__ __launch_bounds__(kBlock) void MatCopyKernel(int trans, int64_t rows, int64_t cols,
                                                        T alpha, const T* __restrict__ src,
                                                        int64_t lds, T* __restrict__ dst) {
  __shared__ T tile[32][33];
  const int tx = threadIdx.x & 31, ty = threadIdx.x >> 5;
  const int64_t i0 = static_cast<int64_t>(blockIdx.x) * 32, j0 = static_cast<int64_t>(blockIdx.y) * 32;
  if (!trans) {
    for (int r = ty; r < 32; r += 8) {
      int64_t i = i0 + tx, j = j0 + r;
      if (i < rows && j < cols) dst[i + j * rows] = alpha * src[i + j * lds];
    }
    return;
  }
  for (int r = ty; r < 32; r += 8) {
    int64_t j = j0 + tx, i = i0 + r;
    if (i < rows && j < cols) tile[r][tx] = src[j + i * lds];
  }
  __syncthreads();
  for (int r = ty; r < 32; r += 8) {
    int64_t i = i0 + tx, j = j0 + r;
    if (i < rows && j < cols) dst[i + j * rows] = alpha * tile[tx][r];
  }
}

template <class T>
__global__ __launch_bounds__(kBlock) void SymmetrizeKernel(T* C, int64_t n, int64_t ldc) {
  __shared__ T tile[32][33];
  const int tx = threadIdx.x & 31, ty = threadIdx.x >> 5;
  const int64_t bi = blockIdx.x, bj = blockIdx.y;
  if (bi > bj) return;
  for (int r = ty; r < 32; r += 8) {
    int64_t jj = bj * 32 + tx, ii = bi * 32 + r;
    if (jj < n && ii < n) tile[r][tx] = C[jj + ii * ldc];
  }
  __syncthreads();
  for (int r = ty; r < 32; r += 8) {
    int64_t ii = bi * 32 + tx, jj = bj * 32 + r;
    if (ii < n && jj < n && ii < jj) C[ii + jj * ldc] = tile[tx][r];
  }
}

template <class T>
__global__ __launch_bounds__(kBlock) void ColAbsSumKernel(const T* __restrict__ A, int64_t rows,
                                                          int64_t lda, double* __restrict__ colsum) {
  const T* col = A + static_cast<int64_t>(blockIdx.x) * lda;
  double a0 = 0, a1 = 0;
  int64_t i = threadIdx.x;
  for (; i + kBlock < rows; i += 2 * kBlock) {
    a0 += fabs(static_cast<double>(col[i]));
    a1 += fabs(static_cast<double>(col[i + kBlock]));
  }
  if (i < rows) a0 += fabs(static_cast<double>(col[i]));
  const double total = BlockSum(a0 + a1);
  if (threadIdx.x == 0) colsum[blockIdx.x] = total;
}

template <class T>
__global__ __launch_bounds__(kBlock) void ScaleByInvNormKernel(T* __restrict__ y, const T* __restrict__ x,
                                                               int64_t n, const double* normsq) {
  const double nn = *normsq;
  const T sc = nn > 0.0 ? static_cast<T>(1.0 / sqrt(nn)) : T(1);
  const int64_t stride = static_cast<int64_t>(gridDim.x) * blockDim.x;
  for (int64_t i = blockIdx.x * static_cast<int64_t>(blockDim.x) + threadIdx.x; i < n; i += stride) y[i] = sc * x[i];
}

template <class T>
__global__ __launch_bounds__(kBlock) void KronKernel(T* __restrict__ dst, const T* __restrict__ A,
                                                     int64_t mA, int64_t nA,
                                                     const T* __restrict__ B, int64_t mB,
                                                     int64_t nB) {
  const int64_t M = mA * mB, N = nA * nB;
  const int64_t total = M * N;
  const int64_t tid = blockIdx.x * static_cast<int64_t>(blockDim.x) + threadIdx.x;
  const int64_t stride = static_cast<int64_t>(gridDim.x) * blockDim.x;
  for (int64_t idx = tid; idx < total; idx += stride) {
    int64_t r = idx % M, c = idx / M;
    int64_t ia = r / mB, ib = r % mB, ja = c / nB, jb = c % nB;
    dst[idx] = A[ia + ja * mA] * B[ib + jb * mB];
  }
}

}

#define EPS_DISPATCH(dt, ...)                      \
  do {                                             \
    if ((dt) == F32) {                             \
      using T = float;                             \
      __VA_ARGS__;                                 \
    } else {                                       \
      using T = double;                            \
      __VA_ARGS__;                                 \
    }                                              \
  } while (0)

void Fill(const DVec& y, double v) {
  EPS_DISPATCH(y.dt, LaunchEw<T>(y.as<T>(), nullptr, nullptr, nullptr, y.n, FillF<T>{T(v)}));
}

namespace {
template <class T> __global__ __launch_bounds__(256) void FillHashKernel(T* y, int64_t n, uint64_t seed) {
  const int64_t i = blockIdx.x * static_cast<int64_t>(256) + threadIdx.x;
  if (i >= n) return;
  uint64_t z = seed + 0x9E3779B97F4A7C15ull * static_cast<uint64_t>(i + 1);
  z = (z ^ (z >> 30)) * 0xBF58476D1CE4E5B9ull;
  z = (z ^ (z >> 27)) * 0x94D049BB133111EBull;
  z ^= z >> 31;
  y[i] = static_cast<T>(static_cast<double>(z >> 11) * (2.0 / 9007199254740992.0) - 1.0);
}
}

void FillHash(const DVec& y, uint64_t seed) {
  if (y.n == 0) return;
  hipStream_t s = Runtime::Get().stream();
  const unsigned grid = static_cast<unsigned>((y.n + 255) / 256);
  if (y.dt == F32) hipLaunchKernelGGL(FillHashKernel<float>, dim3(grid), dim3(256), 0, s, y.as<float>(), y.n, seed);
  else hipLaunchKernelGGL(FillHashKernel<double>, dim3(grid), dim3(256), 0, s, y.as<double>(), y.n, seed);
}

void Copy(const DVec& dst, const DVec& src) {
  CheckSame(dst, src);
  if (dst.n == 0 || dst.data() == src.data()) return;
  EPS_HIP(hipMemcpyAsync(dst.data(), src.data(), dst.bytes(), hipMemcpyDeviceToDevice,
                         Runtime::Get().stream()));
}

void Axpby(const DVec& y, double a, const DVec& x, double b) {
  CheckSame(y, x);
  if (b == 0) {
    EPS_DISPATCH(y.dt, LaunchEw<T>(y.as<T>(), x.as<T>(), nullptr, nullptr, y.n, ScaleF<T>{T(a)}));
  } else if (b == 1 && (a == 1 || a == -1)) {
    EPS_DISPATCH(y.dt,
                 LaunchEw<T>(y.as<T>(), x.as<T>(), y.as<T>(), nullptr, y.n, AddF<T>{T(a)}));
  } else {
    EPS_DISPATCH(y.dt, LaunchEw<T>(y.as<T>(), x.as<T>(), y.as<T>(), nullptr, y.n,
                                   AxpbyF<T>{T(a), T(b)}));
  }
}

void DiagMul(const DVec& y, double a, const DVec& d, const DVec& x, double b) {
  CheckSame(y, x);
  CheckSame(y, d);
  if (b == 0) {
    EPS_DISPATCH(y.dt,
                 LaunchEw<T>(y.as<T>(), d.as<T>(), x.as<T>(), nullptr, y.n, DiagMul0F<T>{T(a)}));
  } else {
    EPS_DISPATCH(y.dt, LaunchEw<T>(y.as<T>(), d.as<T>(), x.as<T>(), y.as<T>(), y.n,
                                   DiagMulF<T>{T(a), T(b)}));
  }
}

void ConvertFromF64(const DVec& dst, const double* src_dev) {
  EPS_DISPATCH(dst.dt, LaunchCvt<T, double>(dst.as<T>(), src_dev, dst.n));
}

void ConvertFromF32(const DVec& dst, const float* src_dev) {
  EPS_DISPATCH(dst.dt, LaunchCvt<T, float>(dst.as<T>(), src_dev, dst.n));
}

void ConvertToF64(double* dst_dev, const DVec& src) {
  EPS_DISPATCH(src.dt, LaunchCvt<double, T>(dst_dev, src.as<T>(), src.n));
}

void SumSq(const DVec& x, double* slot, bool accumulate) {
  EPS_DISPATCH(x.dt, (LaunchRed<T, RED_SUMSQ>(x.as<T>(), nullptr, x.n, slot, accumulate)));
}

void SumSqDiff(const DVec& x, const DVec& y, double* slot, bool accumulate) {
  CheckSame(x, y);
  EPS_DISPATCH(x.dt, (LaunchRed<T, RED_SUMSQ_DIFF>(x.as<T>(), y.as<T>(), x.n, slot, accumulate)));
}

void Dot(const DVec& x, const DVec& y, double* slot, bool accumulate) {
  CheckSame(x, y);
  EPS_DISPATCH(x.dt, (LaunchRed<T, RED_DOT>(x.as<T>(), y.as<T>(), x.n, slot, accumulate)));
}

void AddDiag(const DVec& W, int64_t n, int64_t ld, double alpha, const DVec* d) {
  if (n <= 0) return;
  EPS_CHECK(W.n >= (n - 1) * ld + n);
  if (d) EPS_CHECK(d->n == n && d->dt == W.dt);
  int grid = static_cast<int>((n + kBlock - 1) / kBlock);
  EPS_DISPATCH(W.dt, hipLaunchKernelGGL(AddDiagKernel<T>, dim3(grid), dim3(kBlock), 0,
                                        Runtime::Get().stream(), W.as<T>(), n, ld, T(alpha),
                                        d ? d->as<T>() : static_cast<const T*>(nullptr)));
}

void MatCopy(bool trans, int64_t rows, int64_t cols, double alpha, const DVec& src,
             int64_t lds, const DVec& dst) {
  if (rows <= 0 || cols <= 0) return;
  EPS_CHECK(dst.n >= rows * cols && src.dt == dst.dt);
  dim3 grid(static_cast<unsigned>((rows + 31) / 32), static_cast<unsigned>((cols + 31) / 32));
  EPS_DISPATCH(dst.dt, hipLaunchKernelGGL(MatCopyKernel<T>, grid, dim3(kBlock), 0,
                                          Runtime::Get().stream(), trans ? 1 : 0, rows, cols,
                                          T(alpha), src.as<T>(), lds, dst.as<T>()));
}

void SymmetrizeFromLower(const DVec& C, int64_t n, int64_t ldc) {
  if (n <= 1) return;
  unsigned nb = static_cast<unsigned>((n + 31) / 32);
  EPS_DISPATCH(C.dt, hipLaunchKernelGGL(SymmetrizeKernel<T>, dim3(nb, nb), dim3(kBlock), 0,
                                        Runtime::Get().stream(), C.as<T>(), n, ldc));
}

void ColAbsSums(const DVec& A, int64_t rows, int64_t cols, int64_t lda, double* colsum_dev) {
  if (rows <= 0 || cols <= 0) return;
  EPS_CHECK(A.n >= (cols - 1) * lda + rows);
  EPS_DISPATCH(A.dt, hipLaunchKernelGGL(ColAbsSumKernel<T>, dim3(static_cast<unsigned>(cols)), dim3(kBlock), 0,
                                        Runtime::Get().stream(), A.as<T>(), rows, lda, colsum_dev));
}

void ScaleByInvNorm(const DVec& y, const DVec& x, const double* normsq_dev) {
  CheckSame(y, x);
  if (y.n == 0) return;
  EPS_DISPATCH(y.dt, hipLaunchKernelGGL(ScaleByInvNormKernel<T>, dim3(GridFor(y.n)), dim3(kBlock), 0,
                                        Runtime::Get().stream(), y.as<T>(), x.as<T>(), y.n, normsq_dev));
}

void KronDense(const DVec& dst, const DVec& A, int64_t mA, int64_t nA, const DVec& B,
               int64_t mB, int64_t nB) {
  int64_t total = mA * mB * nA * nB;
  EPS_CHECK(dst.n == total && A.n >= mA * nA && B.n >= mB * nB);
  EPS_CHECK(dst.dt == A.dt && dst.dt == B.dt);
  if (total == 0) return;
  EPS_DISPATCH(dst.dt, hipLaunchKernelGGL(KronKernel<T>, dim3(GridFor(total)), dim3(kBlock), 0,
                                          Runtime::Get().stream(), dst.as<T>(), A.as<T>(), mA,
                                          nA, B.as<T>(), mB, nB));
}


namespace {
typedef float f32x4_probe __attribute__((ext_vector_type(4)));

template <bool NT>
__global__ __launch_bounds__(256) void StreamReadKernel(const f32x4_probe* __restrict__ p, int64_t n4,
                                                        float* __restrict__ out) {
  const int64_t stride = static_cast<int64_t>(gridDim.x) * 256;
  int64_t i = static_cast<int64_t>(blockIdx.x) * 256 + threadIdx.x;
  float acc = 0.f;
  for (; i + 3 * stride < n4; i += 4 * stride) {
    f32x4_probe v0, v1, v2, v3;
    if (NT) {
      v0 = __builtin_nontemporal_load(p + i);
      v1 = __builtin_nontemporal_load(p + i + stride);
      v2 = __builtin_nontemporal_load(p + i + 2 * stride);
      v3 = __builtin_nontemporal_load(p + i + 3 * stride);
    } else {
      v0 = p[i];
      v1 = p[i + stride];
      v2 = p[i + 2 * stride];
      v3 = p[i + 3 * stride];
    }
    acc += (v0.x + v0.y + v0.z + v0.w) + (v1.x + v1.y + v1.z + v1.w) + (v2.x + v2.y + v2.z + v2.w) +
           (v3.x + v3.y + v3.z + v3.w);
  }
  for (; i < n4; i += stride) {
    const f32x4_probe v = p[i];
    acc += v.x + v.y + v.z + v.w;
  }
  __shared__ float red[256];
  red[threadIdx.x] = acc;
  __syncthreads();
  for (int off = 128; off > 0; off >>= 1) {
    if (static_cast<int>(threadIdx.x) < off) red[threadIdx.x] += red[threadIdx.x + off];
    __syncthreads();
  }
  if (threadIdx.x == 0) out[blockIdx.x] = red[0];
}

constexpr int kProbeColumn = 2500;

__global__ __launch_bounds__(256) void StreamResidentKernel(const f32x4_probe* __restrict__ p, int64_t ncols,
                                                            int rv, float* __restrict__ out) {
  typedef const f32x4_probe __attribute__((address_space(4))) * ConstV;
  constexpr int kPer = (kProbeColumn + 255) / 256;
  const int tid = threadIdx.x;
  float acc = 0.f;
  for (int64_t c = blockIdx.x; c < ncols; c += gridDim.x) {
    const f32x4_probe* cp = p + c * kProbeColumn;
    f32x4_probe v[kPer];
#pragma unroll
    for (int q = 0; q < kPer; ++q) {
      const int i = q * 256 + tid;
      if (i >= kProbeColumn) v[q] = 0.f;
      else if (i < rv) v[q] = *(ConstV)(cp + i);
      else v[q] = __builtin_nontemporal_load(cp + i);
    }
#pragma unroll
    for (int q = 0; q < kPer; ++q) acc += (v[q].x + v[q].y) + (v[q].z + v[q].w);
  }
  __shared__ float red[256];
  red[tid] = acc;
  __syncthreads();
  for (int off = 128; off > 0; off >>= 1) {
    if (tid < off) red[tid] += red[tid + off];
    __syncthreads();
  }
  if (tid == 0) out[blockIdx.x] = red[0];
}

__global__ __launch_bounds__(256) void StreamCopyKernel(const f32x4_probe* __restrict__ src,
                                                        f32x4_probe* __restrict__ dst, int64_t n4) {
  const int64_t stride = static_cast<int64_t>(gridDim.x) * 256;
  for (int64_t i = static_cast<int64_t>(blockIdx.x) * 256 + threadIdx.x; i < n4; i += stride)
    dst[i] = src[i];
}
}

void StreamProbe(int mode, const void* src, void* dst, int64_t bytes, float* scratch, int grid) {
  hipStream_t s = Runtime::Get().stream();
  const int64_t n4 = bytes / 16;
  const auto* p = static_cast<const f32x4_probe*>(src);
  if (mode == 0)
    hipLaunchKernelGGL(StreamReadKernel<true>, dim3(grid), dim3(256), 0, s, p, n4, scratch);
  else if (mode == 1)
    hipLaunchKernelGGL(StreamReadKernel<false>, dim3(grid), dim3(256), 0, s, p, n4, scratch);
  else
    hipLaunchKernelGGL(StreamCopyKernel, dim3(grid), dim3(256), 0, s, p, static_cast<f32x4_probe*>(dst), n4);
}

void StreamResidentProbe(const void* src, int64_t bytes, int64_t resident_per_column, float* scratch, int grid) {
  const int64_t ncols = bytes / (16 * kProbeColumn);
  int64_t rv = resident_per_column / 16;
  if (rv < 0) rv = 0;
  if (rv > kProbeColumn) rv = kProbeColumn;
  if (ncols < 1) return;
  hipLaunchKernelGGL(StreamResidentKernel, dim3(grid), dim3(256), 0, Runtime::Get().stream(),
                     static_cast<const f32x4_probe*>(src), ncols, static_cast<int>(rv), scratch);
}

}
}
```

### epsilon_amd/csrc/linear_map.cc

```cpp
#include "linear_map.h"

#include <chrono>
#include <cstdio>
#include <cstdlib>

#include <algorithm>
#include <cmath>
#include <cstdlib>
#include <cstring>
#include <limits>
#include <sstream>

#include "comm.h"
#include "kernels.h"
#include "options.h"
#include "sparse.h"

namespace eps {

const char* ImplTypeName(ImplType t) {
  switch (t) {
    case DENSE_MATRIX: return "DENSE_MATRIX";
    case SPARSE_MATRIX: return "SPARSE_MATRIX";
    case DIAGONAL_MATRIX: return "DIAGONAL_MATRIX";
// ... 87 lines not shown
                                  << " elements, expected " << count);
    DVec src = DVec::Borrow(const_cast<void*>(b.ptr), count, bdt);
    if (bdt == dtype_) {
      v = src;
    } else {
      v = DVec::Empty(count, dtype_);
      if (bdt == F32) k::ConvertFromF32(v, src.as<float>());
      else k::ConvertFromF64(v, src.as<double>());
    }
  }
  uploaded_[c.data_location] = v;
  return v;
}

uint64_t DataMap::DenseId(const pb::Constant& c_in) const {
  const pb::Constant& c = Resolve(c_in);
  if (c.data_location.empty()) return 0;
  const Blob& b = Get(c.data_location);
  uint64_t h = HashBytes(c.data_location.data(), c.data_location.size(), 0x5eed);
  if (b.kind != 0) h = HashCombine(h, reinterpret_cast<uintptr_t>(b.ptr));
  auto g = generation_.find(c.data_location);
  h = HashCombine(h, g == generation_.end() ? 0 : g->second);
  h = HashCombine(h, b.len);
  h = HashCombine(h, static_cast<uint64_t>(c.m) << 32 | static_cast<uint32_t>(c.n));
  return h ? h : 1;
}

std::vector<double> DataMap::DenseHost(const pb::Constant& c_in) {
  const pb::Constant& c = Resolve(c_in);
  EPS_CHECK_MSG(c.constant_type == pb::Constant::DENSE_MATRIX, "constant is not a dense matrix");
  const int64_t count = static_cast<int64_t>(c.m) * c.n;
  const Blob& b = Get(c.data_location);
  if (b.kind == 0 && b.ptr != nullptr) {
    EPS_CHECK(b.len == static_cast<size_t>(count) * sizeof(double));
    std::vector<double> out(count);
    std::memcpy(out.data(), b.ptr, b.len);
    return out;
  }
  return DenseDevice(c).ToHost();
}


LinearMap::LinearMap() : impl_(std::make_shared<ScalarMatrixImpl>(0, 0.0)) {}

LinearMap& LinearMap::operator+=(const LinearMap& rhs) {
  *this = *this + rhs;
  return *this;
}
LinearMap& LinearMap::operator*=(const LinearMap& rhs) {
  *this = *this * rhs;
  return *this;
}

LinearMap LinearMap::Identity(int64_t n) { return Scalar(1.0, n); }
LinearMap LinearMap::Scalar(double alpha, int64_t n) {
  return LinearMap(std::make_shared<ScalarMatrixImpl>(n, alpha));
}
LinearMap LinearMap::Diagonal(std::vector<double> d, DType dt) {
  return LinearMap(std::make_shared<DiagonalMatrixImpl>(std::move(d), dt));
}
LinearMap LinearMap::Dense(DVec data, int64_t rows, int64_t cols, uint64_t id) {
  EPS_CHECK(data.n == rows * cols);
  return LinearMap(std::make_shared<DenseMatrixImpl>(std::move(data), rows, cols, false, 1.0, id));
}
LinearMap LinearMap::Kronecker(LinearMap A, LinearMap B) {
  return LinearMap(std::make_shared<KroneckerProductImpl>(std::move(A), std::move(B)));
}

bool operator==(const LinearMap& lhs, const LinearMap& rhs) { return lhs.impl().Equals(rhs.impl()); }

LinearMap operator*(double alpha, const LinearMap& A) {
  return LinearMap::Scalar(alpha, A.impl().m()) * A;
}

DType MapDType(const LinearMapImpl& A, DType fallback) {
  switch (A.type()) {
    case DENSE_MATRIX: return static_cast<const DenseMatrixImpl&>(A).dtype();
    case DIAGONAL_MATRIX: return static_cast<const DiagonalMatrixImpl&>(A).dtype();
    case SPARSE_MATRIX: return static_cast<const SparseMatrixImpl&>(A).dtype();
    case KRONECKER_PRODUCT: {
      const auto& K = static_cast<const KroneckerProductImpl&>(A);
      return MapDType(K.A().impl(), MapDType(K.B().impl(), fallback));
    }
    default: return fallback;
  }
}


std::string ScalarMatrixImpl::DebugString() const {
  std::ostringstream os;
  os << "scalar matrix: n=" << n_ << " alpha=" << alpha_;
  return os.str();
}
std::shared_ptr<const LinearMapImpl> ScalarMatrixImpl::Transpose() const {
  return std::make_shared<ScalarMatrixImpl>(n_, alpha_);
}
std::shared_ptr<const LinearMapImpl> ScalarMatrixImpl::Inverse() const {
  return std::make_shared<ScalarMatrixImpl>(n_, 1 / alpha_);
}
bool ScalarMatrixImpl::Equals(const LinearMapImpl& o) const {
  if (o.type() != SCALAR_MATRIX || o.m() != m() || o.n() != n()) return false;
  return static_cast<const ScalarMatrixImpl&>(o).alpha() == alpha_;
}
void ScalarMatrixImpl::Apply(double alpha, const DVec& x, double beta, const DVec& y) const {
  EPS_CHECK_MSG(x.n == n_ && y.n == n_, "scalar map of size " << n_ << " applied to " << x.n);
  k::Axpby(y, alpha * alpha_, x, beta);
}
std::vector<double> ScalarMatrixImpl::AsDenseHost() const {
  std::vector<double> D(n_ * n_, 0.0);
  for (int64_t i = 0; i < n_; ++i) D[i + i * n_] = alpha_;
  return D;
}


DiagonalMatrixImpl::DiagonalMatrixImpl(std::vector<double> d, DType dt)
    : LinearMapImpl(DIAGONAL_MATRIX), d_(std::move(d)) {
  dev_ = DVec::FromHost(d_.data(), static_cast<int64_t>(d_.size()), dt);
}
std::string DiagonalMatrixImpl::DebugString() const {
  std::ostringstream os;
  os << "diagonal matrix: n=" << d_.size();
  return os.str();
}
std::shared_ptr<const LinearMapImpl> DiagonalMatrixImpl::Transpose() const {
  return std::make_shared<DiagonalMatrixImpl>(d_, dev_.dt);
}
std::shared_ptr<const LinearMapImpl> DiagonalMatrixImpl::Inverse() const {
  std::vector<double> inv(d_.size());
  for (size_t i = 0; i < d_.size(); ++i) inv[i] = d_[i] ? 1 / d_[i] : 0;
  return std::make_shared<DiagonalMatrixImpl>(std::move(inv), dev_.dt);
}
bool DiagonalMatrixImpl::Equals(const LinearMapImpl& o) const {
  if (o.type() != DIAGONAL_MATRIX || o.m() != m()) return false;
  return static_cast<const DiagonalMatrixImpl&>(o).d_ == d_;
}
void DiagonalMatrixImpl::Apply(double alpha, const DVec& x, double beta, const DVec& y) const {
  EPS_CHECK(x.n == n() && y.n == m());
  k::DiagMul(y, alpha, dev_, x, beta);
}
std::vector<double> DiagonalMatrixImpl::AsDenseHost() const {
  const int64_t n = m();
  std::vector<double> D(n * n, 0.0);
  for (int64_t i = 0; i < n; ++i) D[i + i * n] = d_[i];
  return D;
}


std::string DenseMatrixImpl::DebugString() const {
  std::ostringstream os;
  os << "dense matrix " << m() << " x " << n() << (trans_ ? " (T)" : "") << " scale=" << scale_;
  return os.str();
}
std::shared_ptr<const LinearMapImpl> DenseMatrixImpl::Transpose() const {
  return std::make_shared<DenseMatrixImpl>(data_, rows_, cols_, !trans_, scale_, id_, symmetric_);
}
DVec DenseMatrixImpl::Materialize(bool force_copy) const {
  if (!trans_ && scale_ == 1.0 && !force_copy) return data_;
  DVec out = DVec::Empty(m() * n(), data_.dt);
  k::MatCopy(trans_, m(), n(), scale_, data_, rows_, out);
  return out;
}
namespace {
DVec SymmetricInverseByEig(const DVec& S, int64_t n) {
  Runtime& rt = Runtime::Get();
  rt.ResetSlots();
  const int slot = rt.NewSlot();
  k::SumSq(S, rt.SlotPtr(slot), false);
  rt.FetchSlots();
  const double fro = std::sqrt(rt.SlotValue(slot));
  EPS_CHECK_MSG(fro > 0 && std::isfinite(fro), "dense inverse: the matrix is zero or not finite");
  const double shift = fro * 1.0625;
  DVec W = S.Clone();
  k::AddDiag(W, n, n, shift, nullptr);
  DVec V = DVec::Empty(n * n, S.dt);
  k::JacobiSvd(W, n, n, V, 60, false, false);
  DVec sigma = DVec::Empty(n, S.dt);
  k::ColNorms(W, n, n, sigma, false);
  std::vector<double> lam = sigma.ToHost();
  const double tiny = (S.dt == F32 ? 1e-5 : 1e-12) * fro;
  for (double& l : lam) {
    l -= shift;
    EPS_CHECK_MSG(std::fabs(l) > tiny, "dense inverse: the matrix is singular to working precision");
    l = 1.0 / l;
  }
  DVec linv = DVec::FromHost(lam.data(), n, S.dt);
  DVec ones = DVec::Full(n, 1.0, S.dt);
  DVec T = V.Clone();
  k::ColScaleByRatio(T, n, n, ones, linv);
  DVec out = DVec::Empty(n * n, S.dt);
  k::Gemm(false, true, n, n, n, 1.0, T, n, V, n, 0.0, out, n);
  k::SymmetrizeFromLower(out, n, n);
  return out;
}
}

std::shared_ptr<const LinearMapImpl> DenseMatrixImpl::Inverse() const {
  EPS_CHECK_MSG(m() == n(), "inverting non-square dense matrix");
  const int64_t nn = n();
  if (nn == 0) return std::make_shared<DenseMatrixImpl>(data_, 0, 0, false, 1.0);
  double d0;
  {
    DVec first = data_.Slice(0, 1);
    std::vector<double> h = first.ToHost();
    d0 = h[0] * scale_;
  }
  const double sign = d0 < 0 ? -1.0 : 1.0;
  uint64_t key = 0;
  OpCache* cache = CurrentOpCache();
  if (cache && id_) {
    key = HashDouble(HashCombine(HashCombine(id_, 0x1171), trans_ ? 2 : 1), scale_);
    if (auto hit = cache->Find(key)) {
      auto again = std::make_shared<DenseMatrixImpl>(hit->data(), nn, nn, false, sign, key, true);
      again->packed_ = hit->packed_;
      again->applies_ = hit->applies_;
      return again;
    }
  }
  DVec W = DVec::Empty(nn * nn, data_.dt);
  k::MatCopy(trans_, nn, nn, sign * scale_, data_, rows_, W);
  const bool keep_x = key != 0 && data_.dt == F32 && nn >= kWhitenMinRows && FusedWhitenEnabled();
  DVec X;
  try {
    k::SpdInverseInPlace(W, nn, keep_x ? &X : nullptr);
  } catch (const Error&) {
    (void)hipGetLastError();
    k::MatCopy(trans_, nn, nn, sign * scale_, data_, rows_, W);
    W = SymmetricInverseByEig(W, nn);
    X = DVec();
  }
  auto result = std::make_shared<DenseMatrixImpl>(W, nn, nn, false, sign, key, true);
  if (cache && key) cache->Put(key, result);
  if (cache && key && X.n > 0) {
    const uint64_t xkey = FactorInverseKey(key);
    cache->Put(xkey, std::make_shared<DenseMatrixImpl>(X, nn, nn, false, 1.0, xkey));
  }
  return result;
}

bool FusedWhitenEnabled() {
  static const bool on = !opt::Is0(opt::kFusedWhiten);
  return on;
}
std::shared_ptr<const LinearMapImpl> DenseMatrixImpl::InverseDistributed() const {
  Comm* comm = Runtime::Get().comm();
  const int64_t nn = n();
  const int min_ranks = opt::Int(opt::kDistInverse, 16);
  if (comm == nullptr || comm->size() < std::max(2, min_ranks) || m() != nn || nn < 1024)
    return Inverse();
  double d0;
  {
    std::vector<double> h = data_.Slice(0, 1).ToHost();
    d0 = h[0] * scale_;
  }
  const double sign = d0 < 0 ? -1.0 : 1.0;
  uint64_t key = 0;
  OpCache* cache = CurrentOpCache();
  if (cache && id_) {
    key = HashDouble(HashCombine(HashCombine(id_, 0x1171), trans_ ? 2 : 1), scale_);
    if (auto hit = cache->Find(key))
      return std::make_shared<DenseMatrixImpl>(hit->data(), nn, nn, false, sign, key, true);
  }
  const int G = comm->size();
  const int64_t per = (nn + G - 1) / G;
  const int64_t lo = std::min<int64_t>(nn, comm->rank() * per);
  const int64_t cnt = std::min<int64_t>(nn, lo + per) - lo;
  DVec W = DVec::Empty(nn * nn, data_.dt);
  k::MatCopy(trans_, nn, nn, sign * scale_, data_, rows_, W);
  DVec mine = DVec::Zeros(nn * per, data_.dt);
  k::SpdInverseColumns(W, nn, lo, cnt, mine);
  DVec full = DVec::Empty(nn * per * G, data_.dt);
  comm->AllGather(mine.data(), full.data(), static_cast<size_t>(nn * per), data_.dt);
  DVec inv = full.Slice(0, nn * nn);
  k::SymmetrizeFromLower(inv, nn, nn);
  auto result = std::make_shared<DenseMatrixImpl>(inv, nn, nn, false, sign, key, true);
  if (cache && key) cache->Put(key, result);
  return result;
}

bool DenseMatrixImpl::Equals(const LinearMapImpl& o) const {
  if (o.type() != DENSE_MATRIX || o.m() != m() || o.n() != n()) return false;
  const auto& A = static_cast<const DenseMatrixImpl&>(o);
  if (A.trans_ != trans_ || A.scale_ != scale_) return false;
  if (A.data_.data() == data_.data()) return true;
  if (A.data_.dt != data_.dt) return false;
  Runtime& rt = Runtime::Get();
  rt.ResetSlots();
  int s = rt.NewSlot();
  k::SumSqDiff(A.data_, data_, rt.SlotPtr(s), false);
  rt.FetchSlots();
  return rt.SlotValue(s) == 0.0;
}
void DenseMatrixImpl::Apply(double alpha, const DVec& x, double beta, const DVec& y) const {
  if (symmetric_ && rows_ >= 1024) {
    const opt::SymvPackedMode mode = opt::SymvPacked();
    const bool packed = mode != opt::kSymvPackedOff;
    const int first = mode == opt::kSymvPackedFirst ? 1 : 3;
    if (!packed) packed_ = DVec();
    if (packed && packed_.n == 0 && ++applies_ >= first && !Runtime::Get().capturing())
      packed_ = k::SymvPack(rows_, data_, rows_);
    if (packed_.n > 0) k::SymvPacked(rows_, alpha * scale_, packed_, x, beta, y);
    else k::Symv(rows_, alpha * scale_, data_, rows_, x, beta, y);
    return;
  }
  k::Gemv(trans_, rows_, cols_, alpha * scale_, data_, rows_, x, beta, y);
}
std::vector<double> DenseMatrixImpl::AsDenseHost() const { return Materialize(false).ToHost(); }


std::string KroneckerProductImpl::DebugString() const {
  return "kronecker product\nA: " + A_.impl().DebugString() + "\nB: " + B_.impl().DebugString();
}
std::shared_ptr<const LinearMapImpl> KroneckerProductImpl::Transpose() const {
  return std::make_shared<KroneckerProductImpl>(A_.Transpose(), B_.Transpose());
}
std::shared_ptr<const LinearMapImpl> KroneckerProductImpl::Inverse() const {
  return std::make_shared<KroneckerProductImpl>(A_.Inverse(), B_.Inverse());
}
bool KroneckerProductImpl::Equals(const LinearMapImpl& o) const {
  if (o.type() != KRONECKER_PRODUCT || o.m() != m() || o.n() != n()) return false;
  const auto& K = static_cast<const KroneckerProductImpl&>(o);
  return K.A() == A_ && K.B() == B_;
}

namespace {
void LeftMultiply(const LinearMapImpl& F, double alpha, const DVec& X, int64_t N, double beta,
                  const DVec& C) {
  const int64_t M = F.m(), K = F.n();
  if (F.type() == SCALAR_MATRIX) {
    k::Axpby(C, alpha * static_cast<const ScalarMatrixImpl&>(F).alpha(), X, beta);
  } else if (F.type() == DENSE_MATRIX) {
    const auto& D = static_cast<const DenseMatrixImpl&>(F);
    k::Gemm(D.trans(), false, M, N, K, alpha * D.scale(), D.data(), D.rows(), X, K, beta, C, M);
  } else {
    auto D = ToDense(F, X.dt);
    k::Gemm(false, false, M, N, K, alpha, D->data(), D->rows(), X, K, beta, C, M);
  }
}
void RightMultiplyT(const LinearMapImpl& F, double alpha, const DVec& X, int64_t M, double beta,
                    const DVec& C) {
  const int64_t N = F.m(), K = F.n();
  if (F.type() == SCALAR_MATRIX) {
    k::Axpby(C, alpha * static_cast<const ScalarMatrixImpl&>(F).alpha(), X, beta);
  } else if (F.type() == DENSE_MATRIX) {
    const auto& D = static_cast<const DenseMatrixImpl&>(F);
    k::Gemm(false, !D.trans(), M, N, K, alpha * D.scale(), X, M, D.data(), D.rows(), beta, C, M);
  } else {
    auto D = ToDense(F, X.dt);
    k::Gemm(false, true, M, N, K, alpha, X, M, D->data(), D->rows(), beta, C, M);
  }
}
}

void KroneckerProductImpl::Apply(double alpha, const DVec& x, double beta, const DVec& y) const {
  const LinearMapImpl& A = A_.impl();
  const LinearMapImpl& B = B_.impl();
  EPS_CHECK(x.n == n() && y.n == m());
  if (A.type() == SCALAR_MATRIX) {
    LeftMultiply(B, alpha * static_cast<const ScalarMatrixImpl&>(A).alpha(), x, A.n(), beta, y);
    return;
  }
  if (B.type() == SCALAR_MATRIX) {
    RightMultiplyT(A, alpha * static_cast<const ScalarMatrixImpl&>(B).alpha(), x, B.n(), beta, y);
    return;
  }
  DVec T = DVec::Empty(B.m() * A.n(), x.dt);
  LeftMultiply(B, 1.0, x, A.n(), 0.0, T);
  RightMultiplyT(A, alpha, T, B.m(), beta, y);
}

std::vector<double> KroneckerProductImpl::AsDenseHost() const {
  std::vector<double> A = A_.impl().AsDenseHost(), B = B_.impl().AsDenseHost();
  const int64_t mA = A_.impl().m(), nA = A_.impl().n(), mB = B_.impl().m(), nB = B_.impl().n();
  const int64_t M = mA * mB, N = nA * nB;
  std::vector<double> C(M * N);
  for (int64_t ja = 0; ja < nA; ++ja)
    for (int64_t jb = 0; jb < nB; ++jb)
      for (int64_t ia = 0; ia < mA; ++ia)
        for (int64_t ib = 0; ib < mB; ++ib)
          C[(ia * mB + ib) + (ja * nB + jb) * M] = A[ia + ja * mA] * B[ib + jb * mB];
  return C;
}


std::shared_ptr<const DenseMatrixImpl> ToDense(const LinearMapImpl& A, DType dt) {
  const int64_t m = A.m(), n = A.n();
  EPS_CHECK_MSG(m * n <= (int64_t(1) << 28), "refusing to densify a " << m << " x " << n << " "
                                                                     << ImplTypeName(A.type()));
  switch (A.type()) {
    case DENSE_MATRIX: {
      const auto& D = static_cast<const DenseMatrixImpl&>(A);
      return std::make_shared<DenseMatrixImpl>(D.Materialize(false), m, n, false, 1.0);
    }
    case SCALAR_MATRIX: {
      DVec W = DVec::Zeros(m * n, dt);
      k::AddDiag(W, n, n, static_cast<const ScalarMatrixImpl&>(A).alpha(), nullptr);
      return std::make_shared<DenseMatrixImpl>(W, m, n, false, 1.0);
    }
    case DIAGONAL_MATRIX: {
      const auto& D = static_cast<const DiagonalMatrixImpl&>(A);
      DVec W = DVec::Zeros(m * n, dt);
      k::AddDiag(W, n, n, 1.0, &D.device());
      return std::make_shared<DenseMatrixImpl>(W, m, n, false, 1.0);
    }
    case KRONECKER_PRODUCT: {
      const auto& K = static_cast<const KroneckerProductImpl&>(A);
      auto DA = ToDense(K.A().impl(), dt);
      auto DB = ToDense(K.B().impl(), dt);
      DVec W = DVec::Empty(m * n, dt);
      k::KronDense(W, DA->data(), DA->rows(), DA->cols(), DB->data(), DB->rows(), DB->cols());
      return std::make_shared<DenseMatrixImpl>(W, m, n, false, 1.0);
    }
    case SPARSE_MATRIX: {
      const auto& S = static_cast<const SparseMatrixImpl&>(A);
      DVec W = DVec::Zeros(m * n, S.dtype());
      k::ScatterAddCsc(S.csr_of_transpose(), S.scale(), W);
      return std::make_shared<DenseMatrixImpl>(W, m, n, false, 1.0);
    }
    default:
      EPS_FATAL("ToDense: unsupported type " << ImplTypeName(A.type()));
  }
}


namespace {

using ImplPtr = std::shared_ptr<const LinearMapImpl>;

DType PairDType(const LinearMapImpl& a, const LinearMapImpl& b) {
  return MapDType(a, MapDType(b, CurrentDType()));
}

ImplPtr MultiplyDenseDense(const DenseMatrixImpl& A, const DenseMatrixImpl& B) {
  const int64_t M = A.m(), K = A.n(), N = B.n();
  const double scale = A.scale() * B.scale();
  uint64_t key = 0;
  OpCache* cache = CurrentOpCache();
  if (cache && A.id() && B.id()) {
    key = HashCombine(HashCombine(HashCombine(A.id(), 0x6d756c), B.id()),
                      (A.trans() ? 2 : 0) + (B.trans() ? 1 : 0));
    if (auto hit = cache->Find(key))
      return std::make_shared<DenseMatrixImpl>(hit->data(), M, N, false, scale, key);
  }
  DVec C = DVec::Empty(M * N, A.dtype());
  const bool syrk = A.data().data() == B.data().data() && A.rows() == B.rows() &&
                    A.cols() == B.cols() && A.trans() != B.trans() && M == N;
  k::Gemm(A.trans(), B.trans(), M, N, K, 1.0, A.data(), A.rows(), B.data(), B.rows(), 0.0, C, M,
          syrk);
  if (syrk) k::SymmetrizeFromLower(C, M, M);
  auto unit = std::make_shared<DenseMatrixImpl>(C, M, N, false, 1.0, key);
  if (cache && key) cache->Put(key, unit);
  return std::make_shared<DenseMatrixImpl>(C, M, N, false, scale, key);
}

ImplPtr MultiplyViaDense(const LinearMapImpl& L, const LinearMapImpl& R) {
  DType dt = PairDType(L, R);
  return MultiplyDenseDense(*ToDense(L, dt), *ToDense(R, dt));
}

ImplPtr Multiply(const LinearMapImpl& L, const LinearMapImpl& R);

ImplPtr MultiplyScalarKron(const ScalarMatrixImpl& S, const KroneckerProductImpl& K) {
  ScalarMatrixImpl S1(K.A().impl().m(), S.alpha());
  ScalarMatrixImpl S2(K.B().impl().m(), 1);
  return std::make_shared<KroneckerProductImpl>(LinearMap(Multiply(S1, K.A().impl())),
                                                LinearMap(Multiply(S2, K.B().impl())));
}

ImplPtr MultiplyDenseSparse(const DenseMatrixImpl& A, const SparseMatrixImpl& S);

ImplPtr MultiplyViaSparse(const LinearMapImpl& L, const LinearMapImpl& R) {
  auto diag_of = [](const LinearMapImpl& D, std::vector<double>* d) {
    if (D.type() == SCALAR_MATRIX) {
      d->assign(1, static_cast<const ScalarMatrixImpl&>(D).alpha());
      return true;
    }
    if (D.type() == DIAGONAL_MATRIX) {
      *d = static_cast<const DiagonalMatrixImpl&>(D).diagonal();
      return true;
    }
    return false;
  };
  std::vector<double> d;
  if (R.type() == SPARSE_MATRIX && diag_of(L, &d)) {
    const auto& SR = static_cast<const SparseMatrixImpl&>(R);
    if (d.size() == 1) return SR.Scaled(d[0]);
    return std::make_shared<SparseMatrixImpl>(CscScaleRows(SR.csc(), d), SR.dtype());
  }
  if (L.type() == SPARSE_MATRIX && diag_of(R, &d)) {
    const auto& SL = static_cast<const SparseMatrixImpl&>(L);
    if (d.size() == 1) return SL.Scaled(d[0]);
    return std::make_shared<SparseMatrixImpl>(CscScaleCols(SL.csc(), d), SL.dtype());
  }
  if (L.type() == SPARSE_MATRIX && R.type() == SPARSE_MATRIX) {
    const auto& SL = static_cast<const SparseMatrixImpl&>(L);
    const auto& SR = static_cast<const SparseMatrixImpl&>(R);
    const HostCsc& A = SL.csc_unscaled();
    const HostCsc& B = SR.csc_unscaled();
    std::vector<int64_t> brow(static_cast<size_t>(B.m), 0);
    for (int32_t r : B.rowidx) ++brow[static_cast<size_t>(r)];
    double work = 0;
    for (int64_t k = 0; k < A.n; ++k)
      work += static_cast<double>(A.colptr[k + 1] - A.colptr[k]) * static_cast<double>(brow[k]);
    if (work > 5e7 && L.m() * L.n() <= (int64_t(1) << 28) && L.m() * R.n() <= (int64_t(1) << 25)) {
      const DType dt = PairDType(L, R);
      ImplPtr D = MultiplyDenseSparse(*ToDense(L, dt), SR);
      return std::make_shared<SparseMatrixImpl>(CscFromDense(D->AsDenseHost(), L.m(), R.n()), dt);
    }
  }
  return std::make_shared<SparseMatrixImpl>(CscMultiply(AsSparseHost(L), AsSparseHost(R)),
                                            PairDType(L, R));
}

ImplPtr MultiplyDenseSparse(const DenseMatrixImpl& A, const SparseMatrixImpl& S) {
  DVec Am = A.Materialize(false);
  DVec C = DVec::Empty(A.m() * S.n(), A.dtype());
  k::DenseSpmmCsc(S.csr_of_transpose(), S.scale(), Am, A.m(), A.m(), C);
  return std::make_shared<DenseMatrixImpl>(C, A.m(), S.n(), false, 1.0);
}

ImplPtr MultiplySparseDense(const SparseMatrixImpl& S, const DenseMatrixImpl& B) {
  DVec Bm = B.Materialize(false);
  DVec C = DVec::Empty(S.m() * B.n(), B.dtype());
  k::SpmmCsrDense(S.csr(), S.scale(), Bm, B.m(), B.n(), C);
  return std::make_shared<DenseMatrixImpl>(C, S.m(), B.n(), false, 1.0);
}

ImplPtr Multiply(const LinearMapImpl& L, const LinearMapImpl& R) {
  EPS_CHECK_MSG(L.n() == R.m(), "multiply: A: " << L.DebugString() << "\nB: " << R.DebugString());
  const ImplType a = L.type(), b = R.type();
  if (a == SPARSE_MATRIX || b == SPARSE_MATRIX) {
    if (a == DENSE_MATRIX)
      return MultiplyDenseSparse(static_cast<const DenseMatrixImpl&>(L),
                                 static_cast<const SparseMatrixImpl&>(R));
    if (b == DENSE_MATRIX)
      return MultiplySparseDense(static_cast<const SparseMatrixImpl&>(L),
                                 static_cast<const DenseMatrixImpl&>(R));
    return MultiplyViaSparse(L, R);
  }
  if (a == SCALAR_MATRIX) {
    const auto& S = static_cast<const ScalarMatrixImpl&>(L);
    switch (b) {
      case SCALAR_MATRIX:
        return std::make_shared<ScalarMatrixImpl>(
            S.n(), S.alpha() * static_cast<const ScalarMatrixImpl&>(R).alpha());
      case DIAGONAL_MATRIX: {
        const auto& D = static_cast<const DiagonalMatrixImpl&>(R);
        std::vector<double> d = D.diagonal();
        for (auto& v : d) v = S.alpha() * v;
        return std::make_shared<DiagonalMatrixImpl>(std::move(d), D.dtype());
      }
      case DENSE_MATRIX: {
        const auto& D = static_cast<const DenseMatrixImpl&>(R);
        return std::make_shared<DenseMatrixImpl>(D.data(), D.rows(), D.cols(), D.trans(),
                                                 S.alpha() * D.scale(), D.id(), D.symmetric());
      }
      case KRONECKER_PRODUCT:
        return MultiplyScalarKron(S, static_cast<const KroneckerProductImpl&>(R));
      default: break;
    }
  }
  if (b == SCALAR_MATRIX) {
    const auto& S = static_cast<const ScalarMatrixImpl&>(R);
    switch (a) {
      case DIAGONAL_MATRIX: {
        const auto& D = static_cast<const DiagonalMatrixImpl&>(L);
        std::vector<double> d = D.diagonal();
        for (auto& v : d) v = v * S.alpha();
        return std::make_shared<DiagonalMatrixImpl>(std::move(d), D.dtype());
      }
      case DENSE_MATRIX: {
        const auto& D = static_cast<const DenseMatrixImpl&>(L);
        return std::make_shared<DenseMatrixImpl>(D.data(), D.rows(), D.cols(), D.trans(),
                                                 D.scale() * S.alpha(), D.id(), D.symmetric());
      }
      case KRONECKER_PRODUCT:
        return MultiplyScalarKron(S, static_cast<const KroneckerProductImpl&>(L));
      default: break;
    }
  }
  if (a == DIAGONAL_MATRIX && b == DIAGONAL_MATRIX) {
    const auto& D = static_cast<const DiagonalMatrixImpl&>(L);
    const auto& E = static_cast<const DiagonalMatrixImpl&>(R);
    std::vector<double> d(D.diagonal().size());
    for (size_t i = 0; i < d.size(); ++i) d[i] = D.diagonal()[i] * E.diagonal()[i];
    return std::make_shared<DiagonalMatrixImpl>(std::move(d), D.dtype());
  }
  if (a == DENSE_MATRIX && b == DENSE_MATRIX)
    return MultiplyDenseDense(static_cast<const DenseMatrixImpl&>(L),
                              static_cast<const DenseMatrixImpl&>(R));
  if (a == KRONECKER_PRODUCT && b == KRONECKER_PRODUCT) {
    const auto& C = static_cast<const KroneckerProductImpl&>(L);
    const auto& D = static_cast<const KroneckerProductImpl&>(R);
    if (C.A().impl().n() == D.A().impl().m() && C.B().impl().n() == D.B().impl().m())
      return std::make_shared<KroneckerProductImpl>(C.A() * D.A(), C.B() * D.B());
  }
  if (a == DENSE_MATRIX || b == DENSE_MATRIX) return MultiplyViaDense(L, R);
  return MultiplyViaSparse(L, R);
}


ImplPtr Add(const LinearMapImpl& L, const LinearMapImpl& R);

ImplPtr AddViaDense(const LinearMapImpl& L, const LinearMapImpl& R) {
  DType dt = PairDType(L, R);
  auto A = ToDense(L, dt);
  auto B = ToDense(R, dt);
  DVec C = A->Materialize(true);
  k::Axpby(C, 1.0, B->Materialize(false), 1.0);
  return std::make_shared<DenseMatrixImpl>(C, L.m(), L.n(), false, 1.0);
}

ImplPtr AddViaSparse(const LinearMapImpl& L, const LinearMapImpl& R) {
  return std::make_shared<SparseMatrixImpl>(CscAdd(AsSparseHost(L), AsSparseHost(R)),
                                            PairDType(L, R));
}

ImplPtr AddScalarKron(const ScalarMatrixImpl& S, const KroneckerProductImpl& K) {
  if (K.A().impl().type() == SCALAR_MATRIX) {
    const auto& KS = static_cast<const ScalarMatrixImpl&>(K.A().impl());
    LinearMap S1 = LinearMap::Scalar(0, K.A().impl().n());
    LinearMap S2 = LinearMap::Scalar(S.alpha() / KS.alpha(), K.B().impl().n());
    return std::make_shared<KroneckerProductImpl>(S1 + K.A(), S2 + K.B());
  }
  if (K.B().impl().type() == SCALAR_MATRIX) {
    const auto& KS = static_cast<const ScalarMatrixImpl&>(K.B().impl());
    LinearMap S1 = LinearMap::Scalar(S.alpha() / KS.alpha(), K.A().impl().n());
    LinearMap S2 = LinearMap::Scalar(0, K.B().impl().n());
    return std::make_shared<KroneckerProductImpl>(S1 + K.A(), S2 + K.B());
  }
  return AddViaSparse(S, K);
}

ImplPtr Add(const LinearMapImpl& L, const LinearMapImpl& R) {
  EPS_CHECK_MSG(L.m() == R.m() && L.n() == R.n(),
                "add: A: " << L.DebugString() << "\nB: " << R.DebugString());
  const ImplType a = L.type(), b = R.type();
  if (a == SPARSE_MATRIX || b == SPARSE_MATRIX) {
    if (a == DENSE_MATRIX || b == DENSE_MATRIX) {
      const auto& D = static_cast<const DenseMatrixImpl&>(a == DENSE_MATRIX ? L : R);
      const auto& S = static_cast<const SparseMatrixImpl&>(a == DENSE_MATRIX ? R : L);
      DVec C = D.Materialize(true);
      k::ScatterAddCsc(S.csr_of_transpose(), S.scale(), C);
      return std::make_shared<DenseMatrixImpl>(C, D.m(), D.n(), false, 1.0);
    }
    return AddViaSparse(L, R);
  }
  if (a == SCALAR_MATRIX && b == SCALAR_MATRIX) {
    return std::make_shared<ScalarMatrixImpl>(
        L.n(), static_cast<const ScalarMatrixImpl&>(L).alpha() +
                   static_cast<const ScalarMatrixImpl&>(R).alpha());
  }
  if (a == DIAGONAL_MATRIX && b == DIAGONAL_MATRIX) {
    const auto& D = static_cast<const DiagonalMatrixImpl&>(L);
    const auto& E = static_cast<const DiagonalMatrixImpl&>(R);
    std::vector<double> d(D.diagonal().size());
    for (size_t i = 0; i < d.size(); ++i) d[i] = D.diagonal()[i] + E.diagonal()[i];
    return std::make_shared<DiagonalMatrixImpl>(std::move(d), D.dtype());
  }
  if ((a == DIAGONAL_MATRIX && b == SCALAR_MATRIX) || (a == SCALAR_MATRIX && b == DIAGONAL_MATRIX)) {
    const auto& D = static_cast<const DiagonalMatrixImpl&>(a == DIAGONAL_MATRIX ? L : R);
    const auto& S = static_cast<const ScalarMatrixImpl&>(a == DIAGONAL_MATRIX ? R : L);
    std::vector<double> d = D.diagonal();
    for (auto& v : d) v = v + S.alpha();
    return std::make_shared<DiagonalMatrixImpl>(std::move(d), D.dtype());
  }
  if (a == DENSE_MATRIX || b == DENSE_MATRIX) {
    const LinearMapImpl& Dm = (a == DENSE_MATRIX) ? L : R;
    const LinearMapImpl& O = (a == DENSE_MATRIX) ? R : L;
    const auto& D = static_cast<const DenseMatrixImpl&>(Dm);
    if (O.type() == DENSE_MATRIX) {
      const auto& E = static_cast<const DenseMatrixImpl&>(O);
      DVec C = static_cast<const DenseMatrixImpl&>(L).Materialize(true);
      k::Axpby(C, 1.0, static_cast<const DenseMatrixImpl&>(R).Materialize(false), 1.0);
      (void)E;
      return std::make_shared<DenseMatrixImpl>(C, L.m(), L.n(), false, 1.0);
    }
    if (O.type() == SCALAR_MATRIX) {
      const double a = static_cast<const ScalarMatrixImpl&>(O).alpha();
      uint64_t key = 0;
      OpCache* cache = CurrentOpCache();
      if (cache && D.id()) {
        key = HashDouble(HashDouble(HashCombine(HashCombine(D.id(), 0xadd5), D.trans() ? 2 : 1),
                                    D.scale()), a);
        if (auto hit = cache->Find(key)) return hit;
      }
      DVec C = D.Materialize(true);
      k::AddDiag(C, D.m(), D.m(), a, nullptr);
      auto result = std::make_shared<DenseMatrixImpl>(C, D.m(), D.n(), false, 1.0, key);
      if (cache && key) cache->Put(key, result);
      return result;
    }
    if (O.type() == DIAGONAL_MATRIX) {
      DVec C = D.Materialize(true);
      k::AddDiag(C, D.m(), D.m(), 1.0, &static_cast<const DiagonalMatrixImpl&>(O).device());
      return std::make_shared<DenseMatrixImpl>(C, D.m(), D.n(), false, 1.0);
    }
    return AddViaDense(L, R);
  }
  if (a == SCALAR_MATRIX && b == KRONECKER_PRODUCT)
    return AddScalarKron(static_cast<const ScalarMatrixImpl&>(L),
                         static_cast<const KroneckerProductImpl&>(R));
  if (a == KRONECKER_PRODUCT && b == SCALAR_MATRIX)
    return AddScalarKron(static_cast<const ScalarMatrixImpl&>(R),
                         static_cast<const KroneckerProductImpl&>(L));
  if (a == KRONECKER_PRODUCT && b == KRONECKER_PRODUCT) {
    const auto& K1 = static_cast<const KroneckerProductImpl&>(L);
    const auto& K2 = static_cast<const KroneckerProductImpl&>(R);
    if (K1.A() == K2.A()) return std::make_shared<KroneckerProductImpl>(K1.A(), K1.B() + K2.B());
    if (K1.B() == K2.B()) return std::make_shared<KroneckerProductImpl>(K1.A() + K2.A(), K1.B());
  }
  return AddViaSparse(L, R);
}

}

LinearMap operator*(const LinearMap& lhs, const LinearMap& rhs) {
  return LinearMap(Multiply(lhs.impl(), rhs.impl()));
}
LinearMap operator+(const LinearMap& lhs, const LinearMap& rhs) {
  return LinearMap(Add(lhs.impl(), rhs.impl()));
}


LinearMap BuildLinearMap(const pb::LinearMap& p, DataMap* data) {
  switch (p.linear_map_type) {
    case pb::LinearMap::DENSE_MATRIX: {
      const pb::Constant& c = data->Resolve(p.constant);
      return LinearMap::Dense(data->DenseDevice(c), c.m, c.n, data->DenseId(c));
    }
    case pb::LinearMap::DIAGONAL_MATRIX:
      return LinearMap::Diagonal(data->DenseHost(p.constant), data->dtype());
    case pb::LinearMap::SCALAR:
      return LinearMap::Scalar(p.scalar, p.n);
    case pb::LinearMap::KRONECKER_PRODUCT:
      EPS_CHECK(p.arg.size() == 2);
      return LinearMap::Kronecker(BuildLinearMap(p.arg[0], data), BuildLinearMap(p.arg[1], data));
    case pb::LinearMap::TRANSPOSE:
      EPS_CHECK(p.arg.size() == 1);
      return BuildLinearMap(p.arg[0], data).Transpose();
    case pb::LinearMap::SPARSE_MATRIX: {
      const pb::Constant& c = data->Resolve(p.constant);
      const Blob& b = data->Get(c.data_location);
      EPS_CHECK_MSG(b.kind == 0, "sparse constants must be host blobs");
      return LinearMap(std::make_shared<SparseMatrixImpl>(CscFromBlob(c, b.ptr, b.len),
                                                          data->dtype()));
    }
    default:
      EPS_FATAL("No linear map function for type " << p.linear_map_type);
  }
}

std::vector<double> GetDiagonal(const LinearMap& A) {
  const LinearMapImpl& impl = A.impl();
  if (impl.type() == SCALAR_MATRIX) {
    const auto& S = static_cast<const ScalarMatrixImpl&>(impl);
    return std::vector<double>(S.n(), S.alpha());
  }
  EPS_CHECK_MSG(impl.type() == DIAGONAL_MATRIX, "Non-diagonal linear map " << impl.DebugString());
  return static_cast<const DiagonalMatrixImpl&>(impl).diagonal();
}

double GetScalar(const LinearMap& A) {
  EPS_CHECK_MSG(A.impl().type() == SCALAR_MATRIX, "Non-scalar matrix " << A.impl().DebugString());
  return static_cast<const ScalarMatrixImpl&>(A.impl()).alpha();
}

double OneNorm(const LinearMapImpl& A) {
  switch (A.type()) {
    case SCALAR_MATRIX: return std::fabs(static_cast<const ScalarMatrixImpl&>(A).alpha());
    case DIAGONAL_MATRIX: {
      double mx = 0;
      for (double d : static_cast<const DiagonalMatrixImpl&>(A).diagonal()) mx = std::max(mx, std::fabs(d));
      return mx;
    }
    case DENSE_MATRIX: {
      const auto& D = static_cast<const DenseMatrixImpl&>(A);
      if (D.rows() == 0 || D.cols() == 0) return 0;
      auto buf = Runtime::Get().Alloc(static_cast<size_t>(D.cols()) * sizeof(double));
      k::ColAbsSums(D.data(), D.rows(), D.cols(), D.rows(), static_cast<double*>(buf->p));
      std::vector<double> h(static_cast<size_t>(D.cols()));
      EPS_HIP(hipMemcpyAsync(h.data(), buf->p, h.size() * sizeof(double), hipMemcpyDeviceToHost,
                             Runtime::Get().stream()));
      Runtime::Get().Sync();
      double mx = 0;
      for (double v : h) mx = std::max(mx, v);
      return mx * std::fabs(D.scale());
    }
    case SPARSE_MATRIX: {
      const auto& S = static_cast<const SparseMatrixImpl&>(A);
      const HostCsc& C = S.csc_unscaled();
      double mx = 0;
      for (int64_t j = 0; j < C.n; ++j) {
        double sum = 0;
        for (int32_t p = C.colptr[j]; p < C.colptr[j + 1]; ++p) sum += std::fabs(C.val[p]);
        mx = std::max(mx, sum);
      }
      return mx * std::fabs(S.scale());
    }
    case KRONECKER_PRODUCT: {
      const auto& K = static_cast<const KroneckerProductImpl&>(A);
      return OneNorm(K.A().impl()) * OneNorm(K.B().impl());
    }
    default: return 0;
  }
}

namespace {
double SpectralNormLowerBound(const LinearMapImpl& A, int steps) {
  const int64_t n = A.n();
  if (n == 0 || A.m() != n) return 0;
  const DType dt = MapDType(A, CurrentDType());
  Runtime& rt = Runtime::Get();
  DVec x = DVec::Empty(n, dt), y = DVec::Empty(n, dt);
  k::FillHash(x, 0x5eedu);
  rt.ResetSlots();
  int slot = rt.NewSlot();
  k::SumSq(x, rt.SlotPtr(slot), false);
  k::ScaleByInvNorm(x, x, rt.SlotPtr(slot));
  for (int it = 0; it < steps; ++it) {
    A.Apply(1.0, x, 0.0, y);
    slot = rt.NewSlot();
    k::SumSq(y, rt.SlotPtr(slot), false);
    k::ScaleByInvNorm(x, y, rt.SlotPtr(slot));
  }
  rt.FetchSlots();
  return std::sqrt(rt.SlotValue(slot));
}
}

double ConditionEstimate(const LinearMap& B, const LinearMap& Binv) {
  if (B.impl().type() == SCALAR_MATRIX) return 1.0;
  if (B.impl().type() == DIAGONAL_MATRIX) {
    double mx = 0, mn = std::numeric_limits<double>::infinity();
    for (double d : static_cast<const DiagonalMatrixImpl&>(B.impl()).diagonal()) {
      if (d == 0) continue;
      mx = std::max(mx, std::fabs(d));
      mn = std::min(mn, std::fabs(d));
    }
    return mx > 0 ? mx / mn : 1.0;
  }
  const double k1 = OneNorm(B.impl()) * OneNorm(Binv.impl());
  if (!(k1 > 1e3)) return k1;
  const double k2 = 1.5 * SpectralNormLowerBound(B.impl(), 6) * SpectralNormLowerBound(Binv.impl(), 6);
  return std::min(k1, k2);
}

ImplType ComputeType(ImplType A, ImplType B) {
  if (A <= SCALAR_MATRIX && B <= SCALAR_MATRIX) return A < B ? A : B;
  return DENSE_MATRIX;
}

uint64_t Nonzeros(ImplType type, uint64_t m, uint64_t n) {
  switch (type) {
    case DENSE_MATRIX:
    case SPARSE_MATRIX: return m * n;
    case DIAGONAL_MATRIX: EPS_CHECK(m == n); return n;
    case SCALAR_MATRIX: return 1;
    default: EPS_FATAL("Nonzeros: not implemented for " << ImplTypeName(type));
  }
}

}
```

### epsilon_amd/csrc/linear_map.h

```cpp
#pragma once

#include <map>
#include <memory>
#include <string>
#include <vector>

#include "device.h"
#include "wire.h"

namespace eps {

enum ImplType {
  DENSE_MATRIX = 0,
  SPARSE_MATRIX = 1,
  DIAGONAL_MATRIX = 2,
  SCALAR_MATRIX = 3,
  KRONECKER_PRODUCT = 4,
  NUM_IMPL_TYPES = 5,
};

const char* ImplTypeName(ImplType t);

class LinearMapImpl {
 public:
  explicit LinearMapImpl(ImplType type) : type_(type) {}
  virtual ~LinearMapImpl() {}
  ImplType type() const { return type_; }
  virtual int64_t m() const = 0;
  virtual int64_t n() const = 0;
  virtual std::string DebugString() const = 0;
  virtual std::shared_ptr<const LinearMapImpl> Transpose() const = 0;
  virtual std::shared_ptr<const LinearMapImpl> Inverse() const = 0;
  virtual bool Equals(const LinearMapImpl& other) const = 0;
  virtual void Apply(double alpha, const DVec& x, double beta, const DVec& y) const = 0;
  virtual std::vector<double> AsDenseHost() const = 0;

 private:
  ImplType type_;
};

struct Blob {
  const void* ptr = nullptr;
  size_t len = 0;
  int kind = 0;
  std::shared_ptr<char> owned;
};

class DataMap {
 public:
  explicit DataMap(DType dt) : dtype_(dt) {}
  DType dtype() const { return dtype_; }
  void Insert(const std::string& key, const Blob& b) {
    blobs_[key] = b;
    uploaded_.erase(key);
    ++generation_[key];
  }
  void InsertOwned(const std::string& key, Blob b);
  bool Has(const std::string& key) const { return blobs_.count(key) != 0; }
  const Blob& Get(const std::string& key) const;
  DVec DenseDevice(const pb::Constant& c);
  uint64_t DenseId(const pb::Constant& c) const;
  std::vector<double> DenseHost(const pb::Constant& c);
  void SetParameter(const std::string& id, const pb::Constant& c) { params_[id] = c; }
  void ClearParameters() { params_.clear(); }
  const pb::Constant& Resolve(const pb::Constant& c) const;

 private:
  DType dtype_;
  std::map<std::string, Blob> blobs_;
  std::map<std::string, DVec> uploaded_;
  std::map<std::string, uint64_t> generation_;
  std::map<std::string, pb::Constant> params_;
};

class LinearMap {
 public:
  LinearMap();
  explicit LinearMap(std::shared_ptr<const LinearMapImpl> impl) : impl_(std::move(impl)) {}
  const LinearMapImpl& impl() const { return *impl_; }
  const std::shared_ptr<const LinearMapImpl>& ptr() const { return impl_; }
  LinearMap Inverse() const { return LinearMap(impl_->Inverse()); }
  LinearMap Transpose() const { return LinearMap(impl_->Transpose()); }
  LinearMap& operator+=(const LinearMap& rhs);
  LinearMap& operator*=(const LinearMap& rhs);

  static LinearMap Identity(int64_t n);
  static LinearMap Scalar(double alpha, int64_t n);
  static LinearMap Diagonal(std::vector<double> d, DType dt);
  static LinearMap Dense(DVec data, int64_t rows, int64_t cols, uint64_t id = 0);
  static LinearMap Kronecker(LinearMap A, LinearMap B);

 private:
  std::shared_ptr<const LinearMapImpl> impl_;
};

LinearMap operator+(const LinearMap& lhs, const LinearMap& rhs);
LinearMap operator*(const LinearMap& lhs, const LinearMap& rhs);
LinearMap operator*(double alpha, const LinearMap& A);
bool operator==(const LinearMap& lhs, const LinearMap& rhs);

LinearMap BuildLinearMap(const pb::LinearMap& proto, DataMap* data);

std::vector<double> GetDiagonal(const LinearMap& A);
double GetScalar(const LinearMap& A);

double OneNorm(const LinearMapImpl& A);
double ConditionEstimate(const LinearMap& B, const LinearMap& Binv);

ImplType ComputeType(ImplType A, ImplType B);
uint64_t Nonzeros(ImplType type, uint64_t m, uint64_t n);


class ScalarMatrixImpl final : public LinearMapImpl {
 public:
  ScalarMatrixImpl(int64_t n, double alpha) : LinearMapImpl(SCALAR_MATRIX), n_(n), alpha_(alpha) {}
  int64_t m() const override { return n_; }
  int64_t n() const override { return n_; }
  std::string DebugString() const override;
  std::shared_ptr<const LinearMapImpl> Transpose() const override;
  std::shared_ptr<const LinearMapImpl> Inverse() const override;
  bool Equals(const LinearMapImpl& other) const override;
  void Apply(double alpha, const DVec& x, double beta, const DVec& y) const override;
  std::vector<double> AsDenseHost() const override;
  double alpha() const { return alpha_; }

 private:
  int64_t n_;
  double alpha_;
};

class DiagonalMatrixImpl final : public LinearMapImpl {
 public:
  DiagonalMatrixImpl(std::vector<double> d, DType dt);
  int64_t m() const override { return static_cast<int64_t>(d_.size()); }
  int64_t n() const override { return static_cast<int64_t>(d_.size()); }
  std::string DebugString() const override;
  std::shared_ptr<const LinearMapImpl> Transpose() const override;
  std::shared_ptr<const LinearMapImpl> Inverse() const override;
  bool Equals(const LinearMapImpl& other) const override;
  void Apply(double alpha, const DVec& x, double beta, const DVec& y) const override;
  std::vector<double> AsDenseHost() const override;
  const std::vector<double>& diagonal() const { return d_; }
  const DVec& device() const { return dev_; }
  DType dtype() const { return dev_.dt; }

 private:
  std::vector<double> d_;
  DVec dev_;
};

class DenseMatrixImpl final : public LinearMapImpl {
 public:
  DenseMatrixImpl(DVec data, int64_t rows, int64_t cols, bool trans, double scale,
                  uint64_t id = 0, bool symmetric = false)
      : LinearMapImpl(DENSE_MATRIX), data_(std::move(data)), rows_(rows), cols_(cols),
        trans_(trans), scale_(scale), id_(id), symmetric_(symmetric && rows == cols) {}
  int64_t m() const override { return trans_ ? cols_ : rows_; }
  int64_t n() const override { return trans_ ? rows_ : cols_; }
  std::string DebugString() const override;
  std::shared_ptr<const LinearMapImpl> Transpose() const override;
  std::shared_ptr<const LinearMapImpl> Inverse() const override;
  std::shared_ptr<const LinearMapImpl> InverseDistributed() const;
  bool Equals(const LinearMapImpl& other) const override;
  void Apply(double alpha, const DVec& x, double beta, const DVec& y) const override;
  std::vector<double> AsDenseHost() const override;

  const DVec& data() const { return data_; }
  int64_t rows() const { return rows_; }
  int64_t cols() const { return cols_; }
  bool trans() const { return trans_; }
  double scale() const { return scale_; }
  uint64_t id() const { return id_; }
  bool symmetric() const { return symmetric_; }
  DType dtype() const { return data_.dt; }
  DVec Materialize(bool force_copy) const;

 private:
  DVec data_;
  int64_t rows_, cols_;
  bool trans_;
  double scale_;
  uint64_t id_;
  bool symmetric_;
  mutable DVec packed_;
  mutable int applies_ = 0;
};

class OpCache {
 public:
  std::shared_ptr<const DenseMatrixImpl> Find(uint64_t key) const {
    auto it = map_.find(key);
    return it == map_.end() ? nullptr : it->second;
  }
  void Put(uint64_t key, std::shared_ptr<const DenseMatrixImpl> v) { map_[key] = std::move(v); }
  size_t size() const { return map_.size(); }
  void Clear() { map_.clear(); }

 private:
  std::map<uint64_t, std::shared_ptr<const DenseMatrixImpl>> map_;
};
OpCache* CurrentOpCache();
struct OpCacheScope {
  OpCache* saved;
  explicit OpCacheScope(OpCache* c);
  ~OpCacheScope();
};
uint64_t HashCombine(uint64_t h, uint64_t v);
uint64_t HashBytes(const void* p, size_t n, uint64_t seed);
inline uint64_t HashDouble(uint64_t h, double d) {
  uint64_t b;
  static_assert(sizeof(b) == sizeof(d), "");
  __builtin_memcpy(&b, &d, 8);
  return HashCombine(h, b);
}

constexpr int64_t kWhitenMinRows = 2048;
bool FusedWhitenEnabled();
inline uint64_t FactorInverseKey(uint64_t inverse_key) { return HashCombine(inverse_key, 0x77e1); }

class KroneckerProductImpl final : public LinearMapImpl {
 public:
  KroneckerProductImpl(LinearMap A, LinearMap B)
      : LinearMapImpl(KRONECKER_PRODUCT), A_(std::move(A)), B_(std::move(B)) {}
  int64_t m() const override { return A_.impl().m() * B_.impl().m(); }
  int64_t n() const override { return A_.impl().n() * B_.impl().n(); }
  std::string DebugString() const override;
  std::shared_ptr<const LinearMapImpl> Transpose() const override;
  std::shared_ptr<const LinearMapImpl> Inverse() const override;
  bool Equals(const LinearMapImpl& other) const override;
  void Apply(double alpha, const DVec& x, double beta, const DVec& y) const override;
  std::vector<double> AsDenseHost() const override;
  const LinearMap& A() const { return A_; }
  const LinearMap& B() const { return B_; }

 private:
  LinearMap A_, B_;
};

std::shared_ptr<const DenseMatrixImpl> ToDense(const LinearMapImpl& A, DType dt);
DType MapDType(const LinearMapImpl& A, DType fallback);

}
```

### epsilon_amd/csrc/options.cc

```cpp
#include "options.h"

#include <algorithm>
#include <cstdlib>
#include <cstring>
#include <string>

#include "common.h"

namespace eps {
namespace opt {
namespace {

const struct Option {
  Id id;
  const char *env, *key, *words[5], *unset;
} kOptions[] = {
    {kBatchWide, "EPSILON_HIP_BATCH_WIDE", "batch_wide", {"0", "1"}, "0"},
    {kBatchWideMin, "EPSILON_HIP_BATCH_WIDE_MIN"},
    {kBatchZeroTall, "EPSILON_HIP_BATCH_ZERO_TALL", "batch_zero_tall", {"0", "1"}, "0"},
    {kBenchRandom, "EPSILON_HIP_BENCH_RANDOM"},
    {kDevice, "EPSILON_HIP_DEVICE", "device"},
    {kDistInverse, "EPSILON_HIP_DIST_INVERSE"},
    {kDtype, "EPSILON_HIP_DTYPE"},
    {kForceSharded, "EPSILON_HIP_FORCE_SHARDED"},
    {kFused, "EPSILON_HIP_FUSED", "fused"},
    {kFusedBlock, "EPSILON_HIP_FUSED_BLOCK"},
    {kFusedGrid, "EPSILON_HIP_FUSED_GRID"},
    {kFusedMatrix, "EPSILON_HIP_FUSED_MATRIX", "fused_matrix", {"0", "pass", "wide", "auto"}, "auto"},
    {kFusedResident, "EPSILON_HIP_FUSED_RESIDENT_KB", "fused_resident"},
    {kFusedWhiten, "EPSILON_HIP_FUSED_WHITEN"},
    {kFusedZero, "EPSILON_HIP_FUSED_ZERO", "fused_zero", {"0", "auto"}, "auto"},
    {kFusedZeroTall, "EPSILON_HIP_FUSED_ZERO_TALL", "fused_zero_tall", {"0", "1", "auto"}, "auto"},
    {kFusedZeroTallSmooth, "EPSILON_HIP_FUSED_ZERO_TALL_SMOOTH", "fused_zero_tall_smooth", {"0", "1", "auto"}, "auto"},
    {kGemm, "EPSILON_HIP_GEMM", "gemm"},
    {kGemmOrder, "EPSILON_HIP_GEMM_ORDER"},
    {kGemmSmall, "EPSILON_HIP_GEMM_SMALL"},
    {kGemmStage, "EPSILON_HIP_GEMM_STAGE"},
    {kGramF16Split, "EPSILON_HIP_GRAM_F16SPLIT"},
    {kGraph, "EPSILON_HIP_GRAPH"},
    {kHostThreads, "EPSILON_HIP_HOST_THREADS"},
    {kInitTrace, "EPSILON_HIP_INIT_TRACE"},
    {kPeerWindowMemory, "EPSILON_HIP_PEER_WINDOW_MEMORY"},
    {kPinnedUpload, "EPSILON_HIP_PINNED_UPLOAD"},
    {kPipelineChecks, "EPSILON_HIP_PIPELINE_CHECKS"},
    {kPotrfTwoKernels, "EPSILON_HIP_POTRF_TWO_KERNELS"},
    {kRccl, "EPSILON_HIP_RCCL"},
    {kRefine, "EPSILON_HIP_REFINE", "refine"},
    {kSegGrid, "EPSILON_HIP_SEG_GRID"},
    {kShardedApply, "EPSILON_HIP_SHARDED_APPLY"},
    {kSvd, "EPSILON_HIP_SVD"},
    {kSvdConfirm, "EPSILON_HIP_SVD_CONFIRM"},
    {kSvdInner, "EPSILON_HIP_SVD_INNER"},
    {kSvdMfma, "EPSILON_HIP_SVD_MFMA"},
    {kSvdNoV, "EPSILON_HIP_SVD_NO_V"},
    {kSvdNsplit, "EPSILON_HIP_SVD_NSPLIT"},
    {kSvdPartial, "EPSILON_HIP_SVD_PARTIAL"},
    {kSvdPartialBackoff, "EPSILON_HIP_SVD_PARTIAL_BACKOFF"},
    {kSvdPolar, "EPSILON_HIP_SVD_POLAR"},
    {kSvdSmallFast, "EPSILON_HIP_SVD_SMALL_FAST"},
    {kSvdSort, "EPSILON_HIP_SVD_SORT"},
    {kSvdTrace, "EPSILON_HIP_SVD_TRACE"},
    {kSvdVerbose, "EPSILON_HIP_SVD_VERBOSE"},
    {kSvdWarm, "EPSILON_HIP_SVD_WARM"},
    {kSymvPacked, "EPSILON_HIP_SYMV_PACKED"},
    {kSyrk2d, "EPSILON_HIP_SYRK_2D"},
    {kSyrkTail, "EPSILON_HIP_SYRK_TAIL"},
};
static_assert(sizeof(kOptions) / sizeof(kOptions[0]) == kNumOptions, "one row per Id");

const Option& Row(Id id) {
  const Option& o = kOptions[id];
  EPS_CHECK(o.id == id);
  return o;
}

int WordIndex(const Option& o, const char* value) {
  std::string list;
  for (int i = 0; o.words[i] != nullptr; ++i) {
    if (std::strcmp(o.words[i], value) == 0) return i;
    if (i > 0) list += o.words[i + 1] != nullptr ? ", " : " or ";
    list += o.words[i];
  }
  EPS_FATAL(o.key << " must be " << list << ", got " << value);
}

int64_t ParseFusedResident(const char* value) {
  if (std::strcmp(value, "auto") == 0) return -1;
  const int64_t cap = int64_t(1) << 40;
  int64_t kb = 0;
  bool ok = value[0] != '\0';
  for (const char* c = value; ok && *c != '\0'; ++c) {
    ok = *c >= '0' && *c <= '9';
    if (ok) kb = std::min(cap, kb * 10 + (*c - '0'));
  }
  if (!ok) EPS_FATAL("fused_resident must be auto or a number of KiB, got " << value);
  return kb * 1024;
}

}

const char* Raw(Id id) { return std::getenv(Row(id).env); }

bool IsSet(Id id) { return Raw(id) != nullptr; }

bool Is0(Id id) {
  const char* e = Raw(id);
  return e != nullptr && e[0] == '0';
}

bool Is1(Id id) {
  const char* e = Raw(id);
  return e != nullptr && e[0] == '1';
}

int Int(Id id, int fallback) {
  const char* e = Raw(id);
  return e != nullptr ? std::atoi(e) : fallback;
}

int Word(Id id) {
  const Option& o = Row(id);
  EPS_CHECK(o.words[0] != nullptr);
  const char* e = std::getenv(o.env);
  return WordIndex(o, e != nullptr ? e : o.unset);
}

void Set(const char* key, const char* value) {
  for (const Option& o : kOptions) {
    if (o.key == nullptr || std::strcmp(o.key, key) != 0) continue;
    if (o.words[0] != nullptr) (void)WordIndex(o, value);
    if (o.id == kFusedResident) (void)ParseFusedResident(value);
    if (o.id == kRefine && std::strcmp(value, "auto") == 0) unsetenv(o.env);
    else setenv(o.env, value, 1);
    return;
  }
  EPS_FATAL("unknown option " << key);
}

int64_t FusedResident() {
  const char* e = Raw(kFusedResident);
  return e == nullptr ? -1 : ParseFusedResident(e);
}

int InitTraceLevel() { return Int(kInitTrace, 0); }

SymvPackedMode SymvPacked() {
  const char* e = Raw(kSymvPacked);
  if (e != nullptr && e[0] == '0') return kSymvPackedOff;
  if (e != nullptr && e[0] == '2') return kSymvPackedFirst;
  return kSymvPackedDefault;
}

int DeviceOrdinal(int fallback) {
  const char* e = Raw(kDevice);
  if (e == nullptr) e = std::getenv("LOCAL_RANK");
  return e != nullptr ? std::atoi(e) : fallback;
}

}
}
```

### epsilon_amd/csrc/options.h

```cpp
#pragma once

#include <cstdint>

namespace eps {
namespace opt {

enum Id {
  kBatchWide,
  kBatchWideMin,
  kBatchZeroTall,
  kBenchRandom,
  kDevice,
  kDistInverse,
  kDtype,
  kForceSharded,
  kFused,
  kFusedBlock,
  kFusedGrid,
  kFusedMatrix,
  kFusedResident,
  kFusedWhiten,
  kFusedZero,
  kFusedZeroTall,
  kFusedZeroTallSmooth,
  kGemm,
  kGemmOrder,
  kGemmSmall,
  kGemmStage,
  kGramF16Split,
  kGraph,
  kHostThreads,
  kInitTrace,
  kPeerWindowMemory,
  kPinnedUpload,
  kPipelineChecks,
  kPotrfTwoKernels,
  kRccl,
  kRefine,
  kSegGrid,
  kShardedApply,
  kSvd,
  kSvdConfirm,
  kSvdInner,
  kSvdMfma,
  kSvdNoV,
  kSvdNsplit,
  kSvdPartial,
  kSvdPartialBackoff,
  kSvdPolar,
  kSvdSmallFast,
  kSvdSort,
  kSvdTrace,
  kSvdVerbose,
  kSvdWarm,
  kSymvPacked,
  kSyrk2d,
  kSyrkTail,
  kNumOptions
};

const char* Raw(Id id);
bool IsSet(Id id);
bool Is0(Id id);
bool Is1(Id id);
int Int(Id id, int fallback);
int Word(Id id);

void Set(const char* key, const char* value);

int64_t FusedResident();
int InitTraceLevel();
enum SymvPackedMode { kSymvPackedOff, kSymvPackedFirst, kSymvPackedDefault };
SymvPackedMode SymvPacked();
int DeviceOrdinal(int fallback);

}
}
```

### epsilon_amd/csrc/prox.cc

```cpp
#include "prox.h"

#include <cmath>
#include <map>

#include "kernels.h"

namespace eps {


namespace {
using Factory = std::function<std::unique_ptr<ProxOperator>()>;
std::map<std::pair<int, bool>, Factory>* g_registry = nullptr;
}

bool RegisterProxOperatorFactory(int type, bool epigraph, Factory factory) {
  if (g_registry == nullptr) g_registry = new std::map<std::pair<int, bool>, Factory>();
  (*g_registry)[std::make_pair(type, epigraph)] = std::move(factory);
  return true;
}

std::unique_ptr<ProxOperator> CreateProxOperator(int type, bool epigraph) {
  EPS_CHECK_MSG(g_registry != nullptr, "No registered operators");
  auto it = g_registry->find(std::make_pair(type, epigraph));
  if (it == g_registry->end()) {
// ... 354 lines not shown
REGISTER_EPIGRAPH_OPERATOR(SUM_HINGE, ScaledZoneEpigraph);
REGISTER_EPIGRAPH_OPERATOR(SUM_QUANTILE, ScaledZoneEpigraph);


class Norm2Prox final : public VectorProx {
 public:

  void Init(const ProxOperatorArg& arg) override {
    VectorProx::Init(arg);
    const pb::ProxFunction& f = arg.prox_function();
    has_axis_ = f.has_axis;
    axis_ = f.axis;
    rows_ = cols_ = 0;
    if (!f.arg_size.empty() && f.arg_size[0].dim.size() == 2) {
      rows_ = f.arg_size[0].dim[0];
      cols_ = f.arg_size[0].dim[1];
    }
  }

  bool DescribeGroupNorm2(GroupNorm2Desc* d) const override {
    if (!has_axis_ || axis_ != 1 || rows_ < 1 || cols_ < 1) return false;
    if (!ScalarForm(&d->var_key, &d->constraint_key, &d->Bs, &d->Cs, &d->lam)) return false;
    d->rows = rows_;
    d->cols = cols_;
    return true;
  }

 protected:
  void ApplyVector(const VectorProxInput& input, VectorProxOutput* output) override {
    const DVec& v = input.value_vec(0);
    if (input.prox_function().has_axis) {
      DVec x = DVec::Empty(v.n, v.dt);
      k::SegNorm2Shrink(x, v, input.lambda(), SegsOf(input.prox_function(), 0, v.n));
      output->set_value(0, x);
      return;
    }
    if (!normsq_) normsq_ = Runtime::Get().Alloc(sizeof(double));
    double* slot = static_cast<double*>(normsq_->p);
    k::SumSq(v, slot, false);
    DVec x = DVec::Empty(v.n, v.dt);
    k::Norm2Shrink(x, v, input.lambda(), slot);
    output->set_value(0, x);
  }

 private:
  std::shared_ptr<Buffer> normsq_;
  bool has_axis_ = false;
  int axis_ = 0;
  int64_t rows_ = 0, cols_ = 0;
};
REGISTER_PROX_OPERATOR(NORM_2, Norm2Prox);


class NonNegativeProx final : public VectorProx {
 public:

 protected:
  void ApplyVector(const VectorProxInput& input, VectorProxOutput* output) override {
    const DVec& v = input.value_vec(0);
    DVec x = DVec::Empty(v.n, v.dt);
    k::MaxZero(x, v);
    output->set_value(0, x);
  }
};
REGISTER_PROX_OPERATOR(NON_NEGATIVE, NonNegativeProx);


class TotalVariation1DProx final : public VectorProx {
 protected:
  void ApplyVector(const VectorProxInput& input, VectorProxOutput* output) override {
    const DVec& v = input.value_vec(0);
    DVec x = DVec::Empty(v.n, v.dt);
    k::Tv1dSeg(x, v, input.lambda(), SegsOf(input.prox_function(), 0, v.n));
    output->set_value(0, x);
  }
};
REGISTER_PROX_OPERATOR(TOTAL_VARIATION_1D, TotalVariation1DProx);


class SumSquareProx final : public ProxOperator {
 public:

 public:
  void Init(const ProxOperatorArg& arg) override {
    const BlockMatrix& H = arg.affine_arg().A;
    const BlockVector& g = arg.affine_arg().b;
    const BlockMatrix& A = arg.affine_constraint().A;
    const double alpha = std::sqrt(2 * arg.prox_function().alpha);
    BlockMatrix M = alpha * (H + H.Transpose()) + (A + A.Transpose()) - H.LeftIdentity() -
                    A.LeftIdentity();
    chol_.Compute(M);
    b_ = (-alpha) * g;
    var_keys_ = H.col_keys();
  }
  BlockVector Apply(const BlockVector& v) override {
    return chol_.Solve(b_ + v).Select(var_keys_);
  }

  bool DescribeLeastSquares(LeastSquaresDesc* d) const override {
    const std::vector<std::string>& p = chol_.order();
    if (chol_.refine_steps() > 0) return false;
    if (p.size() == 2 && var_keys_.size() == 1) {
      const std::string &vk = p[0], &ak = p[1];
      if (vk != *var_keys_.begin()) return false;
      const BlockMatrix& L = chol_.L();
      const BlockMatrix& Di = chol_.D_inv();
      if (!L.has_key(ak, vk) || !Di.has_key(vk, vk) || !Di.has_key(ak, ak)) return false;
      if (Di(vk, vk).impl().type() != SCALAR_MATRIX || GetScalar(Di(vk, vk)) != 1.0) return false;
      if (L(ak, vk).impl().type() != DENSE_MATRIX || Di(ak, ak).impl().type() != DENSE_MATRIX)
        return false;
      for (const auto& kv : b_.data())
        if (kv.first != ak) return false;
      d->constraint_key = vk;
      d->var_key = vk;
      d->arg_key = ak;
      d->L_arg_var = std::static_pointer_cast<const DenseMatrixImpl>(L(ak, vk).ptr());
      d->Dinv_arg = std::static_pointer_cast<const DenseMatrixImpl>(Di(ak, ak).ptr());
      if (b_.has_key(ak)) d->rhs_arg = b_(ak);
      return true;
    }
    if (p.size() != 3 || var_keys_.size() != 1) return false;
    const std::string &ck = p[0], &vk = p[1], &ak = p[2];
    if (vk != *var_keys_.begin()) return false;
    const BlockMatrix& L = chol_.L();
    const BlockMatrix& Di = chol_.D_inv();
    if (!L.has_key(vk, ck) || !L.has_key(ak, vk) || L.has_key(ak, ck)) return false;
    if (!Di.has_key(ck, ck) || !Di.has_key(vk, vk) || !Di.has_key(ak, ak)) return false;
    if (!is_scalar(L(vk, ck), -1.0) || !is_scalar(Di(ck, ck), -1.0) || !is_scalar(Di(vk, vk), 1.0))
      return false;
    for (const auto& kv : b_.data())
      if (kv.first != ak) return false;
    int64_t cols = 1, dcols = 1;
    d->L_arg_var = DenseFactor(L(ak, vk), &cols);
    d->Dinv_arg = DenseFactor(Di(ak, ak), &dcols);
    if (!d->L_arg_var || !d->Dinv_arg || cols != dcols) return false;
    d->constraint_key = ck;
    d->var_key = vk;
    d->arg_key = ak;
    d->cols = cols;
    d->rhs_arg = b_.has_key(ak) ? b_(ak) : DVec();
    return true;
  }

 private:
  static std::shared_ptr<const DenseMatrixImpl> DenseFactor(const LinearMap& M, int64_t* cols) {
    *cols = 1;
    if (M.impl().type() == DENSE_MATRIX) return std::static_pointer_cast<const DenseMatrixImpl>(M.ptr());
    if (M.impl().type() != KRONECKER_PRODUCT) return nullptr;
    const auto& K = static_cast<const KroneckerProductImpl&>(M.impl());
    if (K.A().impl().type() != SCALAR_MATRIX || K.B().impl().type() != DENSE_MATRIX) return nullptr;
    const auto& D = static_cast<const DenseMatrixImpl&>(K.B().impl());
    *cols = K.A().impl().n();
    if (*cols < 1) return nullptr;
    return std::make_shared<DenseMatrixImpl>(D.data(), D.rows(), D.cols(), D.trans(),
                                             D.scale() * GetScalar(K.A()), D.id(), D.symmetric());
  }

 private:
  BlockCholesky chol_;
  BlockVector b_;
  std::set<std::string> var_keys_;
};
REGISTER_PROX_OPERATOR(SUM_SQUARE, SumSquareProx);


class SumSquareEpigraph final : public VectorProx {
 protected:
  void ApplyVector(const VectorProxInput& input, VectorProxOutput* output) override {
    const DVec& u = input.value_vec(0);
    const DVec& s = input.value_vec(1);
    if (!scratch_) scratch_ = Runtime::Get().Alloc(2 * sizeof(double));
    double* normsq = static_cast<double*>(scratch_->p);
    k::SumSq(u, normsq, false);
    DVec x = DVec::Empty(u.n, u.dt), t = DVec::Empty(1, u.dt);
    k::SumSquareEpigraph(x, t, u, s, normsq, normsq + 1);
    output->set_value(0, x);
    output->set_value(1, t);
  }

 private:
  std::shared_ptr<Buffer> scratch_;
};
REGISTER_EPIGRAPH_OPERATOR(SUM_SQUARE, SumSquareEpigraph);


class ZeroProx final : public ProxOperator {
 public:

 public:
  void Init(const ProxOperatorArg& arg) override {
    const BlockMatrix& H = arg.affine_arg().A;
    const BlockVector& g = arg.affine_arg().b;
    const BlockMatrix& A = arg.affine_constraint().A;
    BlockMatrix M = H + H.Transpose() + A + A.Transpose() - A.LeftIdentity();
    chol_.Compute(M);
    b_ = (-1.0) * g;
    var_keys_ = H.col_keys();
  }
  BlockVector Apply(const BlockVector& v) override {
    return chol_.Solve(b_ + v).Select(var_keys_);
  }

  bool DescribeZeroProjection(ZeroProjectionDesc* d) const override {
    return DescribeFat(d) || DescribeTall(d);
  }

 private:
  bool DescribeFat(ZeroProjectionDesc* d) const {
    const std::vector<std::string>& p = chol_.order();
    if (chol_.refine_steps() > 0) return false;
    const size_t nv = var_keys_.size();
    if ((nv != 1 && nv != 2) || p.size() != 2 * nv + 1) return false;
    const std::string& ak = p.back();
    if (var_keys_.count(ak) != 0) return false;
    const BlockMatrix& L = chol_.L();
    const BlockMatrix& Di = chol_.D_inv();
    if (!Di.has_key(ak, ak) || Di(ak, ak).impl().type() != DENSE_MATRIX) return false;
    *d = ZeroProjectionDesc();
    for (const std::string& vk : var_keys_) {
      std::string ck;
      for (size_t i = 0; i + 1 < p.size(); ++i) {
        if (var_keys_.count(p[i]) != 0 || !L.has_key(vk, p[i])) continue;
        if (!ck.empty()) return false;
        ck = p[i];
      }
      if (ck.empty() || L.has_key(ak, ck) || !L.has_key(ak, vk)) return false;
      if (!Di.has_key(ck, ck) || !Di.has_key(vk, vk)) return false;
      if (!is_scalar(L(vk, ck), -1.0) || !is_scalar(Di(ck, ck), -1.0) || !is_scalar(Di(vk, vk), 1.0))
        return false;
      for (const std::string& other : var_keys_)
        if (other != vk && (L.has_key(other, vk) || L.has_key(vk, other) || L.has_key(other, ck))) return false;
      const LinearMap& Lav = L(ak, vk);
      if (Lav.impl().type() == DENSE_MATRIX) {
        if (d->L) return false;
        d->L = std::static_pointer_cast<const DenseMatrixImpl>(Lav.ptr());
        d->x_key = vk;
        d->x_constraint_key = ck;
      } else if (Lav.impl().type() == SCALAR_MATRIX) {
        if (!d->z_key.empty()) return false;
        d->e = GetScalar(Lav);
        d->z_key = vk;
        d->z_constraint_key = ck;
      } else {
        return false;
      }
    }
    if (!d->L || d->L->trans() || (nv == 2 && d->z_key.empty())) return false;
    for (const auto& kv : b_.data())
      if (kv.first != ak) return false;
    d->arg_key = ak;
    d->Dinv = std::static_pointer_cast<const DenseMatrixImpl>(Di(ak, ak).ptr());
    d->rhs_arg = b_.has_key(ak) ? b_(ak) : DVec();
    return true;
  }

  bool DescribeTall(ZeroProjectionDesc* d) const {
    const std::vector<std::string>& p = chol_.order();
    if (chol_.refine_steps() > 0) return false;
    if (var_keys_.size() != 2 || p.size() != 5) return false;
    const std::string &zk = p[2], &ak = p[3], &xk = p[4];
    if (var_keys_.count(zk) == 0 || var_keys_.count(xk) == 0 || var_keys_.count(ak) != 0) return false;
    if (var_keys_.count(p[0]) != 0 || var_keys_.count(p[1]) != 0) return false;
    const BlockMatrix& L = chol_.L();
    const BlockMatrix& Di = chol_.D_inv();
    auto row_of = [&](const std::string& vk, std::string* ck) {
      const bool r0 = L.has_key(vk, p[0]), r1 = L.has_key(vk, p[1]);
      if (r0 == r1) return false;
      *ck = r0 ? p[0] : p[1];
      return Di.has_key(*ck, *ck) && is_scalar(L(vk, *ck), -1.0) && is_scalar(Di(*ck, *ck), -1.0);
    };
    std::string cx, cz;
    if (!row_of(xk, &cx) || !row_of(zk, &cz) || cx == cz) return false;
    size_t blocks = 0;
    for (const auto& col : L.data()) blocks += col.second.size();
    if (blocks != 4 || !L.has_key(ak, zk) || !L.has_key(xk, ak)) return false;
    if (!Di.has_key(zk, zk) || !Di.has_key(ak, ak) || !Di.has_key(xk, xk)) return false;
    if (!is_scalar(Di(zk, zk), 1.0)) return false;
    if (Di(ak, ak).impl().type() != SCALAR_MATRIX || L(ak, zk).impl().type() != SCALAR_MATRIX) return false;
    if (L(xk, ak).impl().type() != DENSE_MATRIX || Di(xk, xk).impl().type() != DENSE_MATRIX) return false;
    auto Lxa = std::static_pointer_cast<const DenseMatrixImpl>(L(xk, ak).ptr());
    auto Dx = std::static_pointer_cast<const DenseMatrixImpl>(Di(xk, xk).ptr());
    if (!Lxa->trans() || Dx->rows() != Lxa->m() || Dx->cols() != Lxa->m()) return false;
    for (const auto& kv : b_.data())
      if (kv.first != ak) return false;
    *d = ZeroProjectionDesc();
    d->tall = true;
    d->x_key = xk;
    d->z_key = zk;
    d->arg_key = ak;
    d->x_constraint_key = cx;
    d->z_constraint_key = cz;
    d->L = Lxa;
    d->Dinv = Dx;
    d->dinv_arg = GetScalar(Di(ak, ak));
    d->e = GetScalar(L(ak, zk));
    d->rhs_arg = b_.has_key(ak) ? b_(ak) : DVec();
    return true;
  }

  BlockCholesky chol_;
  BlockVector b_;
  std::set<std::string> var_keys_;
};
REGISTER_PROX_OPERATOR(ZERO, ZeroProx);


class AffineProx final : public ProxOperator {
 public:
// ... 35 lines not shown
```

Baseline: 3370.

## Defer explicit SPD inverse materialization and skip forward pass on zero start

New measurement: 3374, median of 4. No clear change (+0.1%).

```diff
diff --git a/epsilon_amd/csrc/admm.cc b/epsilon_amd/csrc/admm.cc
--- a/epsilon_amd/csrc/admm.cc
+++ b/epsilon_amd/csrc/admm.cc
@@ -220,7 +220,8 @@
     mark("constraints");
     InitProxOperators();
     mark("prox operators");
-    if (!params_.warm_start || !vars_initialized_) {
+    const bool zero_start = !params_.warm_start || !vars_initialized_;
+    if (zero_start) {
       InitVariables();
       vars_initialized_ = true;
     }
@@ -231,7 +232,7 @@
     ResetGraph();
     route_.reset();
     route_ = RecogniseMultiBlockRoute({static_cast<int>(problem_.constraint.size()), A_, b_, prox_, data_.get(),
-                                       shared_cache_, u_, x_, y_, y_prev_});
+                                       shared_cache_, u_, x_, y_, y_prev_, zero_start});
     mark("fused state");
     if (params_.verbose && log_) {
       char buf[128];
diff --git a/epsilon_amd/csrc/capi.cc b/epsilon_amd/csrc/capi.cc
--- a/epsilon_amd/csrc/capi.cc
+++ b/epsilon_amd/csrc/capi.cc
@@ -1338,7 +1338,12 @@
     k::SetPotrfForm(g->form);
     if (args.op == FactorOpArgs::SPD_INVERSE) {
       DVec X;
-      k::SpdInverseInPlace(W, n, out2 != nullptr ? &X : nullptr);
+      if (out2 != nullptr && n > 0) {
+        X = k::SpdFactorInverse(W, n);
+        k::SpdInverseFromFactor(X, n, W);
+      } else {
+        k::SpdInverseInPlace(W, n);
+      }
       EPS_HIP(hipGetLastError());
       w_all.Slice(g->a_off, n * n + 2 * G).ToHost(out);
       if (out2 != nullptr && n > 0) X.Slice(0, n * n).ToHost(out2);
diff --git a/epsilon_amd/csrc/fused_route.cc b/epsilon_amd/csrc/fused_route.cc
--- a/epsilon_amd/csrc/fused_route.cc
+++ b/epsilon_amd/csrc/fused_route.cc
@@ -209,7 +209,8 @@
                                 const pb::SolverParams& params) const {
     return {static_cast<uint64_t>(pass.chain), reinterpret_cast<uintptr_t>(L.data().data()),
             static_cast<uint64_t>(L.rows()), static_cast<uint64_t>(m), static_cast<uint64_t>(n),
-            static_cast<uint64_t>(dt), Bits(L.scale()), reinterpret_cast<uintptr_t>(D.data().data()),
+            static_cast<uint64_t>(dt), Bits(L.scale()),
+            D.deferred() != nullptr ? D.id() : reinterpret_cast<uintptr_t>(D.data().data()),
             Bits(D.scale()), reinterpret_cast<uintptr_t>(inv.packed.data()), inv.work.n > 0 ? 1u : 0u,
             static_cast<uint64_t>(params.max_iterations), static_cast<uint64_t>(params.epoch_iterations)};
   }
@@ -258,6 +259,7 @@
   int64_t group_rows = 0;
   bool wide = false;
   bool rhs_aligned = true;
+  bool zero_start = false;
   std::vector<k::LassoInstance> members;
   DVec table;
   WideSweep ws;
@@ -345,6 +347,7 @@
     if (wide) ws.Init(m, n, whiten ? Ahat : L.data(), whiten ? m : L.rows(), whiten, ls.Dinv_arg.get());
     BuildPass();
     AdoptState(views, Homes(a));
+    zero_start = a.zero_start;
     ForwardFromState();
     return true;
   }
@@ -377,7 +380,10 @@
     if (D.id() == 0 || D.trans() || D.rows() != m || D.cols() != m || L.rows() != m) return false;
     const auto cached = cache->Find(D.id());
     const auto Xm = cache->Find(FactorInverseKey(D.id()));
-    if (!cached || !Xm || cached->data().data() != D.data().data() || Xm->rows() != m || Xm->cols() != m)
+    if (!cached || !Xm || Xm->rows() != m || Xm->cols() != m) return false;
+    const bool deferred = cached->deferred() != nullptr || D.deferred() != nullptr;
+    if (deferred ? cached->deferred() != D.deferred() || Xm->data().data() != D.deferred()->X.data()
+                 : cached->data().data() != D.data().data())
       return false;
     const uint64_t key = HashCombine(HashCombine(HashCombine(HashCombine(Xm->id(), 0x3a7),
                                                              reinterpret_cast<uintptr_t>(L.data().data())),
@@ -410,6 +416,10 @@
   void ForwardFromState() {
     const DenseMatrixImpl& L = *ls.L_arg_var;
     const k::ConsensusState& s = pass.inst.state;
+    if (whiten && zero_start) {
+      if (rhat.n != 0) k::Copy(w.Slice(0, rhat.n), rhat);
+      return;
+    }
     DVec v0 = s.u.Clone();
     k::Axpby(v0, -1.0, s.y_zero, 1.0);
     k::Axpby(v0, -1.0, s.y_term, 1.0);
diff --git a/epsilon_amd/csrc/fused_route.h b/epsilon_amd/csrc/fused_route.h
--- a/epsilon_amd/csrc/fused_route.h
+++ b/epsilon_amd/csrc/fused_route.h
@@ -38,6 +38,7 @@
   OpCache* shared_cache;
   BlockVector& u;
   std::vector<BlockVector>&x, &y, &y_prev;
+  bool zero_start = false;
 };
 struct TwoBlockParts {
   int num_constraints;
diff --git a/epsilon_amd/csrc/kernels.h b/epsilon_amd/csrc/kernels.h
--- a/epsilon_amd/csrc/kernels.h
+++ b/epsilon_amd/csrc/kernels.h
@@ -193,6 +193,9 @@
                int64_t mB, int64_t nB);
 
 void SpdInverseInPlace(const DVec& W, int64_t n, DVec* factor_inverse = nullptr);
+DVec SpdFactorInverse(const DVec& W, int64_t n);
+void SpdInverseFromFactor(const DVec& X, int64_t n, const DVec& W);
+void RowAbsSums(const DVec& A, int64_t rows, int64_t cols, int64_t lda, double* rowsum_dev);
 void SetPotrfForm(int form);
 void SpdInverseColumns(const DVec& W, int64_t n, int64_t lo, int64_t cnt, const DVec& Out);
 
diff --git a/epsilon_amd/csrc/kernels_factor.hip b/epsilon_amd/csrc/kernels_factor.hip
--- a/epsilon_amd/csrc/kernels_factor.hip
+++ b/epsilon_amd/csrc/kernels_factor.hip
@@ -406,14 +406,13 @@
 void DoublingInverse(const DVec& W, const DVec& X, int64_t n, const DVec& dinv, int64_t cap);
 }
 
-void SpdInverseInPlace(const DVec& W, int64_t n, DVec* factor_inverse) {
+DVec SpdFactorInverse(const DVec& W, int64_t n) {
   EPS_CHECK(W.n >= n * n);
-  if (n == 0) return;
+  if (n == 0) return DVec();
   Runtime& rt = Runtime::Get();
   hipStream_t s = rt.stream();
   ProfScope prof("spd_inverse", n);
   const DType dt = W.dt;
-  const int64_t ld = n;
   const int64_t nb = (n + NB - 1) / NB;
 
   DVec dinv = DVec::Empty(nb * NB * NB, dt);
@@ -430,6 +429,14 @@
     ProfScope p2("trtri", n);
     DoublingInverse(W, X, n, dinv, n);
   }
+  CheckFlag(flag);
+  return X;
+}
+
+void SpdInverseFromFactor(const DVec& X, int64_t n, const DVec& W) {
+  EPS_CHECK(W.n >= n * n && X.n >= n * n && X.dt == W.dt);
+  if (n == 0) return;
+  const int64_t ld = n;
   ProfScope p3("lauum", n);
 
   if (!SyrkSplitF16LowerTriangular(n, X, ld, W, ld)) {
@@ -443,8 +450,13 @@
     }
   }
   SymmetrizeFromLower(W, n, ld);
-
-  CheckFlag(flag);
+}
+
+void SpdInverseInPlace(const DVec& W, int64_t n, DVec* factor_inverse) {
+  EPS_CHECK(W.n >= n * n);
+  if (n == 0) return;
+  DVec X = SpdFactorInverse(W, n);
+  SpdInverseFromFactor(X, n, W);
   if (factor_inverse) *factor_inverse = X;
 }
 
diff --git a/epsilon_amd/csrc/kernels_vec.hip b/epsilon_amd/csrc/kernels_vec.hip
--- a/epsilon_amd/csrc/kernels_vec.hip
+++ b/epsilon_amd/csrc/kernels_vec.hip
@@ -270,6 +270,18 @@
 }
 
 template <class T>
+__global__ __launch_bounds__(kBlock) void RowAbsSumPartKernel(const T* __restrict__ A, int64_t rows, int64_t cols,
+                                                              int64_t lda, int64_t per, double* __restrict__ part) {
+  const int64_t i = static_cast<int64_t>(blockIdx.x) * kBlock + threadIdx.x;
+  if (i >= rows) return;
+  const int64_t j0 = static_cast<int64_t>(blockIdx.y) * per;
+  const int64_t j1 = j0 + per < cols ? j0 + per : cols;
+  double a = 0;
+  for (int64_t j = j0; j < j1; ++j) a += fabs(static_cast<double>(A[i + j * lda]));
+  part[blockIdx.y + i * static_cast<int64_t>(gridDim.y)] = a;
+}
+
+template <class T>
 __global__ __launch_bounds__(kBlock) void ScaleByInvNormKernel(T* __restrict__ y, const T* __restrict__ x,
                                                                int64_t n, const double* normsq) {
   const double nn = *normsq;
@@ -421,6 +433,19 @@
   EPS_CHECK(A.n >= (cols - 1) * lda + rows);
   EPS_DISPATCH(A.dt, hipLaunchKernelGGL(ColAbsSumKernel<T>, dim3(static_cast<unsigned>(cols)), dim3(kBlock), 0,
                                         Runtime::Get().stream(), A.as<T>(), rows, lda, colsum_dev));
+}
+
+void RowAbsSums(const DVec& A, int64_t rows, int64_t cols, int64_t lda, double* rowsum_dev) {
+  if (rows <= 0 || cols <= 0) return;
+  EPS_CHECK(A.n >= (cols - 1) * lda + rows);
+  const int64_t rb = (rows + kBlock - 1) / kBlock;
+  const int64_t chunks = std::max<int64_t>(1, std::min<int64_t>({cols, 64, (1024 + rb - 1) / rb}));
+  const int64_t per = (cols + chunks - 1) / chunks;
+  DVec part = DVec::Empty(chunks * rows, F64);
+  EPS_DISPATCH(A.dt, hipLaunchKernelGGL(RowAbsSumPartKernel<T>,
+                                        dim3(static_cast<unsigned>(rb), static_cast<unsigned>(chunks)), dim3(kBlock), 0,
+                                        Runtime::Get().stream(), A.as<T>(), rows, cols, lda, per, part.as<double>()));
+  ColAbsSums(part, chunks, rows, chunks, rowsum_dev);
 }
 
 void ScaleByInvNorm(const DVec& y, const DVec& x, const double* normsq_dev) {
diff --git a/epsilon_amd/csrc/linear_map.cc b/epsilon_amd/csrc/linear_map.cc
--- a/epsilon_amd/csrc/linear_map.cc
+++ b/epsilon_amd/csrc/linear_map.cc
@@ -263,13 +263,28 @@
   return os.str();
 }
 std::shared_ptr<const LinearMapImpl> DenseMatrixImpl::Transpose() const {
-  return std::make_shared<DenseMatrixImpl>(data_, rows_, cols_, !trans_, scale_, id_, symmetric_);
+  auto t = std::make_shared<DenseMatrixImpl>(data_, rows_, cols_, !trans_, scale_, id_, symmetric_);
+  t->deferred_ = deferred_;
+  return t;
+}
+std::shared_ptr<const DenseMatrixImpl> DenseMatrixImpl::Rescaled(double scale) const {
+  auto r = std::make_shared<DenseMatrixImpl>(data_, rows_, cols_, trans_, scale, id_, symmetric_);
+  r->deferred_ = deferred_;
+  return r;
 }
 DVec DenseMatrixImpl::Materialize(bool force_copy) const {
-  if (!trans_ && scale_ == 1.0 && !force_copy) return data_;
-  DVec out = DVec::Empty(m() * n(), data_.dt);
-  k::MatCopy(trans_, m(), n(), scale_, data_, rows_, out);
+  if (!trans_ && scale_ == 1.0 && !force_copy) return data();
+  DVec out = DVec::Empty(m() * n(), dtype());
+  k::MatCopy(trans_, m(), n(), scale_, data(), rows_, out);
   return out;
+}
+
+const DVec& DeferredInverse::Entries() {
+  if (W.n == 0 && n > 0) {
+    W = DVec::Empty(n * n, X.dt);
+    k::SpdInverseFromFactor(X, n, W);
+  }
+  return W;
 }
 namespace {
 DVec SymmetricInverseByEig(const DVec& S, int64_t n) {
@@ -308,10 +323,10 @@
 std::shared_ptr<const LinearMapImpl> DenseMatrixImpl::Inverse() const {
   EPS_CHECK_MSG(m() == n(), "inverting non-square dense matrix");
   const int64_t nn = n();
-  if (nn == 0) return std::make_shared<DenseMatrixImpl>(data_, 0, 0, false, 1.0);
+  if (nn == 0) return std::make_shared<DenseMatrixImpl>(data(), 0, 0, false, 1.0);
   double d0;
   {
-    DVec first = data_.Slice(0, 1);
+    DVec first = data().Slice(0, 1);
     std::vector<double> h = first.ToHost();
     d0 = h[0] * scale_;
   }
@@ -321,25 +336,38 @@
   if (cache && id_) {
     key = HashDouble(HashCombine(HashCombine(id_, 0x1171), trans_ ? 2 : 1), scale_);
     if (auto hit = cache->Find(key)) {
-      auto again = std::make_shared<DenseMatrixImpl>(hit->data(), nn, nn, false, sign, key, true);
+      auto again = std::make_shared<DenseMatrixImpl>(hit->data_, nn, nn, false, sign, key, true);
+      again->deferred_ = hit->deferred_;
       again->packed_ = hit->packed_;
       again->applies_ = hit->applies_;
       return again;
     }
   }
-  DVec W = DVec::Empty(nn * nn, data_.dt);
-  k::MatCopy(trans_, nn, nn, sign * scale_, data_, rows_, W);
-  const bool keep_x = key != 0 && data_.dt == F32 && nn >= kWhitenMinRows && FusedWhitenEnabled();
+  DVec W = DVec::Empty(nn * nn, dtype());
+  k::MatCopy(trans_, nn, nn, sign * scale_, data(), rows_, W);
+  const bool keep_x = key != 0 && dtype() == F32 && nn >= kWhitenMinRows && FusedWhitenEnabled();
+  const bool defer = keep_x && !opt::Is0(opt::kLazyInverse);
   DVec X;
   try {
-    k::SpdInverseInPlace(W, nn, keep_x ? &X : nullptr);
+    if (defer) {
+      X = k::SpdFactorInverse(W, nn);
+      W = DVec();
+    } else {
+      k::SpdInverseInPlace(W, nn, keep_x ? &X : nullptr);
+    }
   } catch (const Error&) {
     (void)hipGetLastError();
-    k::MatCopy(trans_, nn, nn, sign * scale_, data_, rows_, W);
+    if (W.n == 0) W = DVec::Empty(nn * nn, dtype());
+    k::MatCopy(trans_, nn, nn, sign * scale_, data(), rows_, W);
     W = SymmetricInverseByEig(W, nn);
     X = DVec();
   }
   auto result = std::make_shared<DenseMatrixImpl>(W, nn, nn, false, sign, key, true);
+  if (defer && X.n > 0) {
+    result->deferred_ = std::make_shared<DeferredInverse>();
+    result->deferred_->n = nn;
+    result->deferred_->X = X;
+  }
   if (cache && key) cache->Put(key, result);
   if (cache && key && X.n > 0) {
     const uint64_t xkey = FactorInverseKey(key);
@@ -360,7 +388,7 @@
     return Inverse();
   double d0;
   {
-    std::vector<double> h = data_.Slice(0, 1).ToHost();
+    std::vector<double> h = data().Slice(0, 1).ToHost();
     d0 = h[0] * scale_;
   }
   const double sign = d0 < 0 ? -1.0 : 1.0;
@@ -375,12 +403,12 @@
   const int64_t per = (nn + G - 1) / G;
   const int64_t lo = std::min<int64_t>(nn, comm->rank() * per);
   const int64_t cnt = std::min<int64_t>(nn, lo + per) - lo;
-  DVec W = DVec::Empty(nn * nn, data_.dt);
-  k::MatCopy(trans_, nn, nn, sign * scale_, data_, rows_, W);
-  DVec mine = DVec::Zeros(nn * per, data_.dt);
+  DVec W = DVec::Empty(nn * nn, dtype());
+  k::MatCopy(trans_, nn, nn, sign * scale_, data(), rows_, W);
+  DVec mine = DVec::Zeros(nn * per, dtype());
   k::SpdInverseColumns(W, nn, lo, cnt, mine);
-  DVec full = DVec::Empty(nn * per * G, data_.dt);
-  comm->AllGather(mine.data(), full.data(), static_cast<size_t>(nn * per), data_.dt);
+  DVec full = DVec::Empty(nn * per * G, dtype());
+  comm->AllGather(mine.data(), full.data(), static_cast<size_t>(nn * per), dtype());
   DVec inv = full.Slice(0, nn * nn);
   k::SymmetrizeFromLower(inv, nn, nn);
   auto result = std::make_shared<DenseMatrixImpl>(inv, nn, nn, false, sign, key, true);
@@ -392,12 +420,13 @@
   if (o.type() != DENSE_MATRIX || o.m() != m() || o.n() != n()) return false;
   const auto& A = static_cast<const DenseMatrixImpl&>(o);
   if (A.trans_ != trans_ || A.scale_ != scale_) return false;
-  if (A.data_.data() == data_.data()) return true;
-  if (A.data_.dt != data_.dt) return false;
+  if (A.deferred_ != nullptr && A.deferred_ == deferred_) return true;
+  if (A.data().data() == data().data()) return true;
+  if (A.dtype() != dtype()) return false;
   Runtime& rt = Runtime::Get();
   rt.ResetSlots();
   int s = rt.NewSlot();
-  k::SumSqDiff(A.data_, data_, rt.SlotPtr(s), false);
+  k::SumSqDiff(A.data(), data(), rt.SlotPtr(s), false);
   rt.FetchSlots();
   return rt.SlotValue(s) == 0.0;
 }
@@ -408,12 +437,12 @@
     const int first = mode == opt::kSymvPackedFirst ? 1 : 3;
     if (!packed) packed_ = DVec();
     if (packed && packed_.n == 0 && ++applies_ >= first && !Runtime::Get().capturing())
-      packed_ = k::SymvPack(rows_, data_, rows_);
+      packed_ = k::SymvPack(rows_, data(), rows_);
     if (packed_.n > 0) k::SymvPacked(rows_, alpha * scale_, packed_, x, beta, y);
-    else k::Symv(rows_, alpha * scale_, data_, rows_, x, beta, y);
+    else k::Symv(rows_, alpha * scale_, data(), rows_, x, beta, y);
     return;
   }
-  k::Gemv(trans_, rows_, cols_, alpha * scale_, data_, rows_, x, beta, y);
+  k::Gemv(trans_, rows_, cols_, alpha * scale_, data(), rows_, x, beta, y);
 }
 std::vector<double> DenseMatrixImpl::AsDenseHost() const { return Materialize(false).ToHost(); }
 
@@ -662,8 +691,7 @@
       }
       case DENSE_MATRIX: {
         const auto& D = static_cast<const DenseMatrixImpl&>(R);
-        return std::make_shared<DenseMatrixImpl>(D.data(), D.rows(), D.cols(), D.trans(),
-                                                 S.alpha() * D.scale(), D.id(), D.symmetric());
+        return D.Rescaled(S.alpha() * D.scale());
       }
       case KRONECKER_PRODUCT:
         return MultiplyScalarKron(S, static_cast<const KroneckerProductImpl&>(R));
@@ -681,8 +709,7 @@
       }
       case DENSE_MATRIX: {
         const auto& D = static_cast<const DenseMatrixImpl&>(L);
-        return std::make_shared<DenseMatrixImpl>(D.data(), D.rows(), D.cols(), D.trans(),
-                                                 D.scale() * S.alpha(), D.id(), D.symmetric());
+        return D.Rescaled(D.scale() * S.alpha());
       }
       case KRONECKER_PRODUCT:
         return MultiplyScalarKron(S, static_cast<const KroneckerProductImpl&>(L));
@@ -917,10 +944,9 @@
 }
 
 namespace {
-double SpectralNormLowerBound(const LinearMapImpl& A, int steps) {
-  const int64_t n = A.n();
-  if (n == 0 || A.m() != n) return 0;
-  const DType dt = MapDType(A, CurrentDType());
+template <class ApplyFn>
+double PowerIterationNorm(int64_t n, DType dt, int steps, ApplyFn apply) {
+  if (n == 0) return 0;
   Runtime& rt = Runtime::Get();
   DVec x = DVec::Empty(n, dt), y = DVec::Empty(n, dt);
   k::FillHash(x, 0x5eedu);
@@ -929,13 +955,34 @@
   k::SumSq(x, rt.SlotPtr(slot), false);
   k::ScaleByInvNorm(x, x, rt.SlotPtr(slot));
   for (int it = 0; it < steps; ++it) {
-    A.Apply(1.0, x, 0.0, y);
+    apply(x, y);
     slot = rt.NewSlot();
     k::SumSq(y, rt.SlotPtr(slot), false);
     k::ScaleByInvNorm(x, y, rt.SlotPtr(slot));
   }
   rt.FetchSlots();
   return std::sqrt(rt.SlotValue(slot));
+}
+double SpectralNormLowerBound(const LinearMapImpl& A, int steps) {
+  if (A.m() != A.n()) return 0;
+  return PowerIterationNorm(A.n(), MapDType(A, CurrentDType()), steps,
+                            [&](const DVec& x, const DVec& y) { A.Apply(1.0, x, 0.0, y); });
+}
+double SpectralNormLowerBoundOfGram(const DVec& X, int64_t n, int steps) {
+  DVec t = DVec::Empty(n, X.dt);
+  return PowerIterationNorm(n, X.dt, steps, [&](const DVec& x, const DVec& y) {
+    k::Gemv(false, n, n, 1.0, X, n, x, 0.0, t);
+    k::Gemv(true, n, n, 1.0, X, n, t, 0.0, y);
+  });
+}
+double MaxOfDeviceDoubles(const std::shared_ptr<Buffer>& buf, int64_t n) {
+  std::vector<double> h(static_cast<size_t>(n));
+  EPS_HIP(hipMemcpyAsync(h.data(), buf->p, h.size() * sizeof(double), hipMemcpyDeviceToHost,
+                         Runtime::Get().stream()));
+  Runtime::Get().Sync();
+  double mx = 0;
+  for (double v : h) mx = std::max(mx, v);
+  return mx;
 }
 }
 
@@ -950,7 +997,24 @@
     }
     return mx > 0 ? mx / mn : 1.0;
   }
-  const double k1 = OneNorm(B.impl()) * OneNorm(Binv.impl());
+  const double b1 = OneNorm(B.impl());
+  if (Binv.impl().type() == DENSE_MATRIX) {
+    const auto& D = static_cast<const DenseMatrixImpl&>(Binv.impl());
+    if (D.deferred() != nullptr && !D.materialized()) {
+      const DeferredInverse& r = *D.deferred();
+      const double c = std::fabs(D.scale());
+      auto sums = Runtime::Get().Alloc(static_cast<size_t>(r.n) * sizeof(double));
+      k::ColAbsSums(r.X, r.n, r.n, r.n, static_cast<double*>(sums->p));
+      const double x1 = MaxOfDeviceDoubles(sums, r.n);
+      k::RowAbsSums(r.X, r.n, r.n, r.n, static_cast<double*>(sums->p));
+      const double xinf = MaxOfDeviceDoubles(sums, r.n);
+      const double ub = b1 * c * x1 * xinf;
+      if (!(ub > 1e3)) return ub;
+      const double k2f = 1.5 * SpectralNormLowerBound(B.impl(), 6) * c * SpectralNormLowerBoundOfGram(r.X, r.n, 6);
+      if (k2f <= 0.99e3) return k2f;
+    }
+  }
+  const double k1 = b1 * OneNorm(Binv.impl());
   if (!(k1 > 1e3)) return k1;
   const double k2 = 1.5 * SpectralNormLowerBound(B.impl(), 6) * SpectralNormLowerBound(Binv.impl(), 6);
   return std::min(k1, k2);
diff --git a/epsilon_amd/csrc/linear_map.h b/epsilon_amd/csrc/linear_map.h
--- a/epsilon_amd/csrc/linear_map.h
+++ b/epsilon_amd/csrc/linear_map.h
@@ -149,6 +149,14 @@
   DVec dev_;
 };
 
+struct DeferredInverse {
+  int64_t n = 0;
+  DVec X;
+  DVec W;
+  bool materialized() const { return W.n > 0; }
+  const DVec& Entries();
+};
+
 class DenseMatrixImpl final : public LinearMapImpl {
  public:
   DenseMatrixImpl(DVec data, int64_t rows, int64_t cols, bool trans, double scale,
@@ -165,18 +173,25 @@
   void Apply(double alpha, const DVec& x, double beta, const DVec& y) const override;
   std::vector<double> AsDenseHost() const override;
 
-  const DVec& data() const { return data_; }
+  const DVec& data() const {
+    if (deferred_ != nullptr && data_.n == 0) data_ = deferred_->Entries();
+    return data_;
+  }
   int64_t rows() const { return rows_; }
   int64_t cols() const { return cols_; }
   bool trans() const { return trans_; }
   double scale() const { return scale_; }
   uint64_t id() const { return id_; }
   bool symmetric() const { return symmetric_; }
-  DType dtype() const { return data_.dt; }
+  DType dtype() const { return deferred_ != nullptr ? deferred_->X.dt : data_.dt; }
   DVec Materialize(bool force_copy) const;
-
- private:
-  DVec data_;
+  std::shared_ptr<const DenseMatrixImpl> Rescaled(double scale) const;
+  const std::shared_ptr<DeferredInverse>& deferred() const { return deferred_; }
+  bool materialized() const { return deferred_ == nullptr || deferred_->materialized(); }
+
+ private:
+  mutable DVec data_;
+  std::shared_ptr<DeferredInverse> deferred_;
   int64_t rows_, cols_;
   bool trans_;
   double scale_;
diff --git a/epsilon_amd/csrc/options.cc b/epsilon_amd/csrc/options.cc
--- a/epsilon_amd/csrc/options.cc
+++ b/epsilon_amd/csrc/options.cc
@@ -40,6 +40,7 @@
     {kGraph, "EPSILON_HIP_GRAPH"},
     {kHostThreads, "EPSILON_HIP_HOST_THREADS"},
     {kInitTrace, "EPSILON_HIP_INIT_TRACE"},
+    {kLazyInverse, "EPSILON_HIP_LAZY_INVERSE", "lazy_inverse", {"0", "1"}, "1"},
     {kPeerWindowMemory, "EPSILON_HIP_PEER_WINDOW_MEMORY"},
     {kPinnedUpload, "EPSILON_HIP_PINNED_UPLOAD"},
     {kPipelineChecks, "EPSILON_HIP_PIPELINE_CHECKS"},
diff --git a/epsilon_amd/csrc/options.h b/epsilon_amd/csrc/options.h
--- a/epsilon_amd/csrc/options.h
+++ b/epsilon_amd/csrc/options.h
@@ -31,6 +31,7 @@
   kGraph,
   kHostThreads,
   kInitTrace,
+  kLazyInverse,
   kPeerWindowMemory,
   kPinnedUpload,
   kPipelineChecks,
diff --git a/epsilon_amd/csrc/prox.cc b/epsilon_amd/csrc/prox.cc
--- a/epsilon_amd/csrc/prox.cc
+++ b/epsilon_amd/csrc/prox.cc
@@ -530,8 +530,7 @@
     const auto& D = static_cast<const DenseMatrixImpl&>(K.B().impl());
     *cols = K.A().impl().n();
     if (*cols < 1) return nullptr;
-    return std::make_shared<DenseMatrixImpl>(D.data(), D.rows(), D.cols(), D.trans(),
-                                             D.scale() * GetScalar(K.A()), D.id(), D.symmetric());
+    return D.Rescaled(D.scale() * GetScalar(K.A()));
   }
 
  private:
```
